# zzuiekongning/MGDT-YOLO

Measured on AMD Instinct MI355X. Metric: images/sec @640x640 bs=32 per GPU, detection forward + NMS (whole job: 1 GPU(s)), higher is better.
Workload: dtype bf16; 1 GPU; mspa_c2f_gd_yolov8-n (MSPA-C2f + GD neck + Detect, nc=80) 640x640 inference, batch 32/GPU: forward + decode + NMS(conf 0.25, iou 0.7), hipGraph replay, 4 batches in flight (one captured graph per resident batch, replayed round-robin on 4 streams); global_batch=32, parallelism=replicas x1 (batch-sharded, no data-path collective), rccl_ranks=1, input=bfloat16 NCHW images, 8 different batches resident in HBM (600 MiB) cycled, detections_last_step=9600, weights=seeded random init (no checkpoints offline), batches_in_flight=4

## Files before the change

include/mgdt.h:

```cpp
#ifndef MGDT_H
#define MGDT_H
#include <stddef.h>
#include <stdint.h>

#ifdef __cplusplus
extern "C" {
#endif

typedef void* mgdt_stream;

typedef enum { MGDT_OK = 0, MGDT_BAD_SHAPE = -1, MGDT_BAD_DTYPE = -2, MGDT_LAUNCH_FAIL = -3, MGDT_BAD_ARG = -4,
               MGDT_WORKSPACE = -5 } mgdt_status;
typedef enum { MGDT_F32 = 0, MGDT_BF16 = 1, MGDT_U8 = 2  } mgdt_dtype;
typedef enum { MGDT_ACT_NONE = 0, MGDT_ACT_SILU = 1, MGDT_ACT_RELU = 2, MGDT_ACT_GELU = 3 } mgdt_act;

typedef struct {
  void* p;
  int32_t n, h, w, c;
  int64_t sn, sh, sw, sc;
} mgdt_view;

const char* mgdt_last_error(void);
const char* mgdt_version(void);

size_t mgdt_conv_packed_bytes(int cin, int cout, int k, int dtype);
int mgdt_conv_pack(const float* w_oihw, const float* conv_bias, const float* bn_gamma, const float* bn_beta,
                   const float* bn_mean, const float* bn_var, float bn_eps, int cin, int cout, int k, int dtype,
                   void* packed_out, float* bias_out, mgdt_stream s);
int mgdt_conv_pack_dgrad(const float* w_oihw, int cin, int cout, int k, int phase, int dtype, void* packed_out, float* bias_out, mgdt_stream s);
typedef struct mgdt_pack_desc {
  const float* w; const float* conv_bias; const float* bn_gamma; const float* bn_beta; const float* bn_mean; const float* bn_var;
  float bn_eps; int32_t cin, cout, k, dtype, mode;
  void* packed; float* bias_out;
} mgdt_pack_desc;
int mgdt_conv_pack_batch(const mgdt_pack_desc* descs, int n, mgdt_stream s);

int mgdt_conv2d_fwd(const mgdt_view* x, const mgdt_view* x2, const float* in_scale, const float* in_shift,
                    const void* packed_w, const float* bias, int k, int stride, int act, const mgdt_view* r1,
                    const mgdt_view* r2, const mgdt_view* y, int dtype, mgdt_stream s);
size_t mgdt_conv_packed_bytes_fp8(int cin, int cout, int k);
int mgdt_conv_pack_fp8(const float* w_oihw, const float* conv_bias, const float* bn_gamma, const float* bn_beta, const float* bn_mean,
                       const float* bn_var, float bn_eps, int cin, int cout, int k, float x_qscale, void* packed_out, float* bias_out,
                       float* oscale_out, mgdt_stream s);
int mgdt_conv2d_fp8_fwd(const mgdt_view* x, const mgdt_view* x2, const float* in_scale, const float* in_shift, const void* packed_w,
                        const float* bias, const float* oscale, float x_qscale, int k, int stride, int act, const mgdt_view* r1,
                        const mgdt_view* r2, const mgdt_view* y, mgdt_stream s);
int mgdt_conv2d_phase_fwd(const mgdt_view* x, const void* packed_w, const float* bias, int phase, const mgdt_view* r1, const mgdt_view* r2,
                          const mgdt_view* y, int dtype, mgdt_stream s);

size_t mgdt_cnx_mlp_packed_bytes(int c, int dtype);
int mgdt_cnx_mlp_pack(const float* w1, const float* b1, const float* w2, const float* b2, int c, void* packed, int dtype, mgdt_stream s);
size_t mgdt_cnx_mlp_workspace_bytes(int n, int h, int w, int c);
int mgdt_cnx_mlp_fwd(const mgdt_view* t, const mgdt_view* res, const void* packed, const float* gamma, const float* beta, void* ws,
                     const mgdt_view* y, int dtype, mgdt_stream s);

int mgdt_cnx_block_supported(int n, int h, int w, int c, int dtype);
size_t mgdt_cnx_block_workspace_bytes(int n, int h, int w, int c);
int mgdt_cnx_block_fwd(const mgdt_view* x, const float* dw_w49c, const float* dw_b, const float* ln_w, const float* ln_b, float eps, const void* packed,
                       const float* gamma, const float* beta, const void* tail_w, const float* tail_b, int tail_act, void* ws, size_t ws_bytes,
                       const mgdt_view* y, int dtype, mgdt_stream s);

size_t mgdt_stem2_packed_bytes(void);
int mgdt_stem2_pack(const float* w_folded, void* packed, mgdt_stream s);
int mgdt_stem2_fwd(const mgdt_view* x, int x_dtype, const void* packed0, const float* bias0, const void* packed1, const float* bias1,
                   const mgdt_view* y, mgdt_stream s);

int mgdt_detect_tail_supported(int c2, int c3, int nc, int reg_max, int dtype);
int mgdt_detect_tail_fwd(const mgdt_view* tb, const mgdt_view* tc, const void* wb, const float* bb, const void* wc, const float* bc, int nc,
                         float stride, int a_off, int a_total, const mgdt_view* feat, float* y, unsigned long long* best_keys,
                         const void* wb3, const float* bb3, mgdt_stream s);
int mgdt_detect_tail_aug_fwd(const mgdt_view* tb, const mgdt_view* tc, const void* wb, const float* bb, const void* wc, const float* bc, int nc,
                             float stride, int a_off, int a_total, const mgdt_view* feat, float* y, unsigned long long* best_keys,
                             const void* wb3, const float* bb3, float aug_scale, int aug_flip, float aug_img_w, mgdt_stream s);

int mgdt_scale_img_fwd(const mgdt_view* x, int x_dtype, int flip, int hs, int ws, float pad, const mgdt_view* y, int y_dtype, mgdt_stream s);

int mgdt_csp_block_supported(int mode, int cin, int cout, int wd, int nbtl, int h, int w, int dtype);
int mgdt_csp_block_tiles(int mode, int n, int cin, int cout, int wd, int nbtl, int h, int w, int* geom8);
int mgdt_csp_block_fwd(int mode, const mgdt_view* x, const void* front, const float* front_bias, const void* const* mid,
                       const float* const* mid_bias, int nbtl, int shortcut, const void* back, const float* back_bias, int wd, int act,
                       const mgdt_view* y, float* pool, int dtype, mgdt_stream s);

size_t mgdt_pw_chain_packed_bytes(int wd, int dtype);
int mgdt_pw_chain_pack(int idx, const float* w_oi, const float* conv_bias, const float* bn_gamma, const float* bn_beta, const float* bn_mean,
                       const float* bn_var, float bn_eps, int wd, int dtype, void* packed, mgdt_stream s);
int mgdt_pw_chain3_fwd(const mgdt_view* x, const void* packed, int wd, int act, const mgdt_view* y, int dtype, mgdt_stream s);

int mgdt_conv1x1_inject_supported(int cin, int cout, int h, int w, int hg, int wg, int dtype);
int mgdt_conv1x1_inject_fwd(const mgdt_view* x, const void* packed_w, const float* bias, const mgdt_view* ga, const mgdt_view* gf,
                            const mgdt_view* y, int dtype, mgdt_stream s);

int mgdt_conv1x1_inject_conv_supported(int cin, int cmid, int cout2, int h, int w, int hg, int wg, int dtype);
int mgdt_conv1x1_inject_conv_fwd(const mgdt_view* x, const void* packed_w, const float* bias, const mgdt_view* ga, const mgdt_view* gf,
                                 const mgdt_view* gsrc, const void* packed_wg, const float* bias_g, int cmid,
                                 const void* packed_w2, const float* bias2, int act2, const mgdt_view* y2, int dtype, mgdt_stream s);

size_t mgdt_groupnorm_workspace_bytes(int n, int c);
int mgdt_groupnorm_fwd(const mgdt_view* x, const float* gamma, const float* beta, int groups, float eps, int act, void* ws, const mgdt_view* y,
                       int dtype, mgdt_stream s);
int mgdt_tood_layer_attn_fwd(const float* sums, int n, int c, int hw, const float* w1, const float* b1, const float* w2, const float* b2, int hid,
                             int stacked, float* scale, mgdt_stream s);
int mgdt_dcnv2_fwd(const mgdt_view* x, const mgdt_view* offset_mask, const float* w_gemm, const float* bias, const mgdt_view* y, int dtype,
                   mgdt_stream s);
int mgdt_dcnv2_mfma_fwd(const mgdt_view* x, const mgdt_view* offset_mask, const void* packed_w, const mgdt_view* y, int dtype, mgdt_stream s);
int mgdt_pixel_gate_fwd(const mgdt_view* x, const mgdt_view* gate, const mgdt_view* y, int dtype, mgdt_stream s);

int mgdt_conv_pack_direct(const float* w_oihw, const float* conv_bias, const float* bn_gamma, const float* bn_beta,
                          const float* bn_mean, const float* bn_var, float bn_eps, int cin_g, int cout, int k,
                          float* w_out, float* bias_out, mgdt_stream s);
int mgdt_conv2d_direct_fwd(const mgdt_view* x, int x_dtype, const float* w_gemm, const float* bias, int k, int stride,
                           int groups, int act, const mgdt_view* y, int dtype, mgdt_stream s);

#define MGDT_SPR_SPLITS 16
int mgdt_spr_pool_fwd(const mgdt_view* x, float* pooled, int dtype, mgdt_stream s);
int mgdt_spr_attn_fwd(const float* pooled, const float* fc1_w, const float* fc1_b, const float* fc2_w,
                      const float* fc2_b, int n, int c, int groups, int h, int w, int softmax, float* attn, mgdt_stream s);
int mgdt_scale_channels_fwd(const mgdt_view* x, const float* attn, const mgdt_view* y, int dtype, mgdt_stream s);
int mgdt_spr_attn_scale_fwd(const float* pooled, int nsplit, int tiles_x, int tiles_y, const float* fc1_w, const float* fc1_b, const float* fc2_w, const float* fc2_b, int groups,
                            const mgdt_view* x, const mgdt_view* y, const mgdt_view* pool_a, const mgdt_view* pool_b, int dtype, mgdt_stream s);

int mgdt_sppf_pool_fwd(const mgdt_view* x, const mgdt_view* y1, const mgdt_view* y2, const mgdt_view* y3, int dtype,
                       mgdt_stream s);

int mgdt_adaptive_avgpool_fwd(const mgdt_view* x, const mgdt_view* y, int dtype, mgdt_stream s);
int mgdt_bilinear_fwd(const mgdt_view* x, const mgdt_view* y, int dtype, mgdt_stream s);
int mgdt_nearest_fwd(const mgdt_view* x, const mgdt_view* y, int dtype, mgdt_stream s);
int mgdt_copy_fwd(const mgdt_view* x, int x_dtype, const mgdt_view* y, int y_dtype, mgdt_stream s);
int mgdt_image_pad4_fwd(const mgdt_view* x, int x_dtype, const mgdt_view* y, int y_dtype, mgdt_stream s);

#define MGDT_GRN_SPLITS 8
int mgdt_dwconv7_ln_fwd(const mgdt_view* x, const float* dw_w, const float* dw_b, const float* ln_w, const float* ln_b,
                        float eps, const mgdt_view* y, int dtype, mgdt_stream s);
int mgdt_grn_stats_fwd(const mgdt_view* t, const float* gamma, float* ws, float* scale, int dtype, mgdt_stream s);

int mgdt_inject_fwd(const mgdt_view* local, const mgdt_view* ga, const mgdt_view* gf, const mgdt_view* y, int dtype,
                    mgdt_stream s);

int mgdt_detect_decode_fwd(const mgdt_view* feat, int reg_max, int nc, float stride, int a_off, int a_total, float* y,
                           int dtype, mgdt_stream s);
int mgdt_detect_decode_aug_fwd(const mgdt_view* feat, int reg_max, int nc, float stride, int a_off, int a_total, float* y,
                               unsigned long long* best_keys, float aug_scale, int aug_flip, float aug_img_w, int dtype, mgdt_stream s);

size_t mgdt_nms_workspace_bytes(int n, int nc, int a, int multi_label, int max_nms);
int mgdt_nms_fwd(const float* pred, int n, int nc, int a, float conf_thres, float iou_thres, const int32_t* classes,
                 int n_classes, int agnostic, int multi_label, int max_det, int max_nms, float max_wh, float* out,
                 int32_t* kept_anchor, int32_t* counts, const unsigned long long* best_keys, void* ws, size_t ws_bytes, mgdt_stream s);

int mgdt_val_match_fwd(const float* det, const int32_t* ndet, int n, int max_det, const float* labels, const int32_t* nlab, int max_lab,
                       const float* iouv, int n_iou, uint8_t* correct, mgdt_stream s);

size_t mgdt_detect_loss_workspace_bytes(int b, int a_total, int n_gt);
int mgdt_detect_loss_fwd(const mgdt_view* const* feats, const float* strides, int n_levels, int reg_max, int nc,
                         const float* gt, int n_gt, int call_count, float gain_box, float gain_cls, float gain_dfl,
                         float* out5, unsigned char* fg_out, int32_t* gt_idx_out, float* tscore_out, void* ws,
                         size_t ws_bytes, int dtype, mgdt_stream s);
int mgdt_detect_loss_fwd_dev(const mgdt_view* const* feats, const float* strides, int n_levels, int reg_max, int nc,
                             const float* gt, int n_gt, const int32_t* call_count_dev, float gain_box, float gain_cls, float gain_dfl,
                             float* out5, unsigned char* fg_out, int32_t* gt_idx_out, float* tscore_out, void* ws,
                             size_t ws_bytes, int dtype, mgdt_stream s);
int mgdt_detect_loss_bwd(const mgdt_view* const* feats, const mgdt_view* const* grads, const float* strides, int n_levels,
                         int reg_max, int nc, const float* gt, int n_gt, float gain_box, float gain_cls, float gain_dfl,
                         float gscale, const float* out5, void* ws, size_t ws_bytes, int dtype, mgdt_stream s);

size_t mgdt_reduce_workspace_bytes(int c);
int mgdt_bn_stats_fwd(const mgdt_view* y, float eps, float momentum, float* mean, float* rstd, float* running_mean,
                      float* running_var, void* ws, int dtype, mgdt_stream s);
int mgdt_bn_act_fwd(const mgdt_view* y, const float* mean, const float* rstd, const float* gamma, const float* beta, int act,
                    const mgdt_view* r1, const mgdt_view* r2, const mgdt_view* z, int dtype, mgdt_stream s);
int mgdt_bn_act_bwd(const mgdt_view* gz, const mgdt_view* y, const float* mean, const float* rstd, const float* gamma,
                    const float* beta, int act, float* dgamma, float* dbeta, const mgdt_view* dy, void* ws, int dtype, mgdt_stream s);
int mgdt_conv_dgrad(const mgdt_view* dy, const float* w_oihw, int k, int stride, const mgdt_view* dx, int accumulate, int dtype,
                    mgdt_stream s);
int mgdt_gconv_dgrad(const mgdt_view* dy, const float* w, int k, int stride, int groups, const mgdt_view* dx, int accumulate, int dtype,
                     mgdt_stream s);
size_t mgdt_gconv_wgrad_workspace_bytes(int cin, int cout, int k, int groups);
int mgdt_gconv_wgrad(const mgdt_view* x, const mgdt_view* dy, int k, int stride, int groups, float* dw, int accumulate, void* ws, int dtype,
                     mgdt_stream s);
size_t mgdt_conv_wgrad_workspace_bytes(int cin, int cout, int k);
int mgdt_conv_wgrad(const mgdt_view* x, const mgdt_view* x2, const mgdt_view* dy, int k, int stride, float* dw_oihw, float* dbias,
                    int accumulate, void* ws, int dtype, mgdt_stream s);
int mgdt_conv_wgrad_splits(int cin, int cout, int k);
typedef struct mgdt_wgrad_final_desc { const float* partial; float* dw; long n; int32_t nsplit; int32_t accumulate; } mgdt_wgrad_final_desc;
int mgdt_wgrad_final_batch(const mgdt_wgrad_final_desc* descs, int n, mgdt_stream s);
int mgdt_add_fwd(const mgdt_view* a, const mgdt_view* b, const mgdt_view* o, int dtype, mgdt_stream s);
int mgdt_maxpool5_bwd(const mgdt_view* x, const mgdt_view* gy, float* gx_f32, int dtype, mgdt_stream s);
int mgdt_nearest_bwd(const mgdt_view* gy, const mgdt_view* gx, int dtype, mgdt_stream s);

int mgdt_ew_binary(const mgdt_view* a, const mgdt_view* b, const mgdt_view* o, int mode, int dtype, mgdt_stream s);
int mgdt_channel_affine(const mgdt_view* x, const float* scale, const float* shift, const mgdt_view* y, int dtype, mgdt_stream s);
size_t mgdt_nc_reduce_workspace_bytes(int n, int c);
int mgdt_nc_reduce(const mgdt_view* a, const mgdt_view* b, float* out, void* ws, int dtype, mgdt_stream s);
int mgdt_adaptive_avgpool_bwd(const mgdt_view* gy, const mgdt_view* gx, int accumulate, int dtype, mgdt_stream s);
int mgdt_bilinear_bwd(const mgdt_view* gy, const mgdt_view* gx, int accumulate, int dtype, mgdt_stream s);
size_t mgdt_spr_bwd_workspace_bytes(int n, int c, int groups);
int mgdt_spr_bwd(const mgdt_view* gy, const float* pooled_partial, int splits, const float* attn, const float* dattn,
                 const float* fc1_w, const float* fc1_b, const float* fc2_w, const float* fc2_b, int groups,
                 const mgdt_view* gx, float* param_grads, void* ws, int dtype, mgdt_stream s);
int mgdt_dwconv7_ln_train_fwd(const mgdt_view* x, const float* dw_w, const float* dw_b, const float* ln_w, const float* ln_b,
                              float eps, const mgdt_view* y, const mgdt_view* u_out, int dtype, mgdt_stream s);
size_t mgdt_dwconv7_ln_bwd_workspace_bytes(int c);
int mgdt_dwconv7_ln_bwd(const mgdt_view* x, const mgdt_view* u, const mgdt_view* gy, const float* dw_w49c, const float* ln_w, float eps,
                        const mgdt_view* du_tmp, const mgdt_view* dx, int accumulate_dx, float* d_dw_w, float* d_dw_b,
                        float* d_ln_w, float* d_ln_b, void* ws, int dtype, mgdt_stream s);
int mgdt_grn_bwd(const mgdt_view* g, const mgdt_view* t, const float* S, const float* A, const float* B, const float* gamma,
                 const mgdt_view* dt, float* dgamma, float* dbeta, void* ws, int dtype, mgdt_stream s);

size_t mgdt_grad_norm_workspace_bytes(void);
int mgdt_grad_clip_coef(const float* g, long n, float max_norm, float* out2, void* ws, mgdt_stream s);
int mgdt_sgd_step(float* p, const float* g, float* buf, const float* wd, long n, float lr, float lr_bias, float momentum, int nesterov,
                  int first, const float* clip2, mgdt_stream s);
int mgdt_ema_update(float* ema, const float* p, long n, float decay, mgdt_stream s);
int mgdt_sgd_ema_step_dev(float* p, const float* g, float* buf, const float* wd, long n_param, float* ema, long n_total, const float* hyper4,
                          int nesterov, int first, const float* clip2, mgdt_stream s);

int mgdt_box_convert(const float* in, float* out, long n, int row, int mode, mgdt_stream s);
int mgdt_box_iou(const float* b1, int n, const float* b2, int m, float eps, float* out, mgdt_stream s);
int mgdt_bbox_iou(const float* b1, int stride1, const float* b2, int stride2, long n, int xywh, int mode, float eps, float* out, mgdt_stream s);
int mgdt_scale_boxes(float* boxes, long n, int row, float gain, float padx, float pady, float h0, float w0, mgdt_stream s);
int mgdt_letterbox_fwd(const void* src_hwc_bgr, int sh, int sw, long src_pitch, void* dst_chw_rgb, int dh, int dw, int new_h, int new_w, int top,
                       int left, mgdt_stream s);
size_t mgdt_ap_workspace_bytes(int n_det, int n_cls);
int mgdt_ap_per_class(const void* tp, const float* conf, const int32_t* seg, const int32_t* nlab, int n_det, int n_cls, int T, const double* x101,
                      const double* px, double eps, void* ws, double* ap, double* pcur, double* rcur, mgdt_stream s);

int mgdt_gn_affine(const float* Sy, const float* Syy, int n, int c, int hw, const float* gamma, const float* beta, int groups, float eps,
                   float* mean_ng, float* rstd_ng, float* A, float* B, mgdt_stream s);
int mgdt_nc_affine_act_bwd(const mgdt_view* g, const mgdt_view* y, const float* A, const float* B, int act, const mgdt_view* gu, int dtype, mgdt_stream s);
size_t mgdt_gn_bwd_workspace_bytes(int n, int c);
int mgdt_gn_bwd_coef(const float* S1, const float* S2, const float* mean_ng, const float* rstd_ng, const float* gamma, int n, int c, int hw, int groups,
                     float* P, float* Q, float* R, float* dgamma, float* dbeta, int accumulate, void* ws, mgdt_stream s);
int mgdt_nc_axpby(const mgdt_view* a, const float* sa, const mgdt_view* b, const float* sb, const float* shift, const mgdt_view* out, int dtype,
                  mgdt_stream s);
int mgdt_pixel_gate_bwd(const mgdt_view* g, const mgdt_view* x, const mgdt_view* logit, const mgdt_view* gx, const mgdt_view* glogit, int dtype, mgdt_stream s);
size_t mgdt_tood_layer_attn_bwd_workspace_bytes(int n, int c, int hid, int stacked);
int mgdt_tood_layer_attn_bwd(const float* sums, const float* dscale, int n, int c, int hw, const float* w1, const float* b1, const float* w2,
                             const float* b2, int hid, int stacked, float* dsums, float* dw1, float* db1, float* dw2, float* db2, int accumulate,
                             void* ws, mgdt_stream s);
int mgdt_dcn_im2col(const mgdt_view* x, const mgdt_view* om, const mgdt_view* col, int dtype, mgdt_stream s);
int mgdt_dcn_col2im_bwd(const mgdt_view* gcol, const mgdt_view* x, const mgdt_view* om, float* gx_f32, const mgdt_view* gom, int dtype, mgdt_stream s);

#ifdef __cplusplus
}
#endif
#endif
```

mgdt_yolo_amd/_lib.py:

```python
import ctypes as C
import os

_HERE = os.path.dirname(os.path.abspath(__file__))
LIB_PATH = os.environ.get('MGDT_LIB') or os.path.join(_HERE, 'csrc', 'libmgdt_hip.so')

F32, BF16 = 0, 1
ACT_NONE, ACT_SILU, ACT_RELU, ACT_GELU = 0, 1, 2, 3
SPR_SPLITS = 16
GRN_SPLITS = 8


class View(C.Structure):
    _fields_ = [('p', C.c_void_p), ('n', C.c_int32), ('h', C.c_int32), ('w', C.c_int32), ('c', C.c_int32),
                ('sn', C.c_int64), ('sh', C.c_int64), ('sw', C.c_int64), ('sc', C.c_int64)]


VP = C.POINTER(View)
_vp, _i, _f, _sz = C.c_void_p, C.c_int, C.c_float, C.c_size_t

class PackDesc(C.Structure):
    _fields_ = [('w', C.c_void_p), ('conv_bias', C.c_void_p), ('bn_gamma', C.c_void_p), ('bn_beta', C.c_void_p), ('bn_mean', C.c_void_p), ('bn_var', C.c_void_p),
                ('bn_eps', C.c_float), ('cin', C.c_int32), ('cout', C.c_int32), ('k', C.c_int32), ('dtype', C.c_int32), ('mode', C.c_int32),
                ('packed', C.c_void_p), ('bias_out', C.c_void_p)]


class WgradFinalDesc(C.Structure):
    _fields_ = [('partial', C.c_void_p), ('dw', C.c_void_p), ('n', C.c_long), ('nsplit', C.c_int32), ('accumulate', C.c_int32)]


PROTOTYPES = {
    'mgdt_last_error': (C.c_char_p, []),
    'mgdt_version': (C.c_char_p, []),
    'mgdt_conv_packed_bytes': (_sz, [_i, _i, _i, _i]),
    'mgdt_conv_pack': (_i, [_vp, _vp, _vp, _vp, _vp, _vp, _f, _i, _i, _i, _i, _vp, _vp, _vp]),
    'mgdt_conv2d_fwd': (_i, [VP, VP, _vp, _vp, _vp, _vp, _i, _i, _i, VP, VP, VP, _i, _vp]),
    'mgdt_conv_packed_bytes_fp8': (_sz, [_i, _i, _i]),
    'mgdt_conv_pack_fp8': (_i, [_vp, _vp, _vp, _vp, _vp, _vp, _f, _i, _i, _i, _f, _vp, _vp, _vp, _vp]),
    'mgdt_conv2d_fp8_fwd': (_i, [VP, VP, _vp, _vp, _vp, _vp, _vp, _f, _i, _i, _i, VP, VP, VP, _vp]),
    'mgdt_conv_pack_batch': (_i, [_vp, _i, _vp]),
    'mgdt_conv2d_phase_fwd': (_i, [VP, _vp, _vp, _i, VP, VP, VP, _i, _vp]),
    'mgdt_conv_wgrad_splits': (_i, [_i, _i, _i]),
    'mgdt_wgrad_final_batch': (_i, [_vp, _i, _vp]),
    'mgdt_conv_pack_dgrad': (_i, [_vp, _i, _i, _i, _i, _i, _vp, _vp, _vp]),
    'mgdt_conv_pack_direct': (_i, [_vp, _vp, _vp, _vp, _vp, _vp, _f, _i, _i, _i, _vp, _vp, _vp]),
    'mgdt_conv2d_direct_fwd': (_i, [VP, _i, _vp, _vp, _i, _i, _i, _i, VP, _i, _vp]),
    'mgdt_spr_pool_fwd': (_i, [VP, _vp, _i, _vp]),
    'mgdt_spr_attn_fwd': (_i, [_vp, _vp, _vp, _vp, _vp, _i, _i, _i, _i, _i, _i, _vp, _vp]),
    'mgdt_scale_channels_fwd': (_i, [VP, _vp, VP, _i, _vp]),
    'mgdt_sppf_pool_fwd': (_i, [VP, VP, VP, VP, _i, _vp]),
    'mgdt_adaptive_avgpool_fwd': (_i, [VP, VP, _i, _vp]),
    'mgdt_bilinear_fwd': (_i, [VP, VP, _i, _vp]),
    'mgdt_nearest_fwd': (_i, [VP, VP, _i, _vp]),
    'mgdt_copy_fwd': (_i, [VP, _i, VP, _i, _vp]),
    'mgdt_image_pad4_fwd': (_i, [VP, _i, VP, _i, _vp]),
    'mgdt_dwconv7_ln_fwd': (_i, [VP, _vp, _vp, _vp, _vp, _f, VP, _i, _vp]),
    'mgdt_cnx_mlp_packed_bytes': (_sz, [_i, _i]),
    'mgdt_cnx_mlp_pack': (_i, [_vp, _vp, _vp, _vp, _i, _vp, _i, _vp]),
    'mgdt_cnx_mlp_workspace_bytes': (_sz, [_i, _i, _i, _i]),
    'mgdt_cnx_mlp_fwd': (_i, [VP, VP, _vp, _vp, _vp, _vp, VP, _i, _vp]),
    'mgdt_cnx_block_supported': (_i, [_i, _i, _i, _i, _i]),
    'mgdt_cnx_block_workspace_bytes': (_sz, [_i, _i, _i, _i]),
    'mgdt_cnx_block_fwd': (_i, [VP, _vp, _vp, _vp, _vp, _f, _vp, _vp, _vp, _vp, _vp, _i, _vp, _sz, VP, _i, _vp]),
    'mgdt_pw_chain_packed_bytes': (_sz, [_i, _i]),
    'mgdt_pw_chain_pack': (_i, [_i, _vp, _vp, _vp, _vp, _vp, _vp, _f, _i, _i, _vp, _vp]),
    'mgdt_pw_chain3_fwd': (_i, [VP, _vp, _i, _i, VP, _i, _vp]),
    'mgdt_conv1x1_inject_supported': (_i, [_i, _i, _i, _i, _i, _i, _i]),
    'mgdt_conv1x1_inject_fwd': (_i, [VP, _vp, _vp, VP, VP, VP, _i, _vp]),
    'mgdt_conv1x1_inject_conv_supported': (_i, [_i, _i, _i, _i, _i, _i, _i, _i]),
    'mgdt_conv1x1_inject_conv_fwd': (_i, [VP, _vp, _vp, VP, VP, VP, _vp, _vp, _i, _vp, _vp, _i, VP, _i, _vp]),
    'mgdt_spr_attn_scale_fwd': (_i, [_vp, _i, _i, _i, _vp, _vp, _vp, _vp, _i, VP, VP, VP, VP, _i, _vp]),
    'mgdt_stem2_packed_bytes': (_sz, []),
    'mgdt_stem2_pack': (_i, [_vp, _vp, _vp]),
    'mgdt_stem2_fwd': (_i, [VP, _i, _vp, _vp, _vp, _vp, VP, _vp]),
    'mgdt_detect_tail_supported': (_i, [_i, _i, _i, _i, _i]),
    'mgdt_detect_tail_fwd': (_i, [VP, VP, _vp, _vp, _vp, _vp, _i, _f, _i, _i, VP, _vp, _vp, _vp, _vp, _vp]),
    'mgdt_detect_tail_aug_fwd': (_i, [VP, VP, _vp, _vp, _vp, _vp, _i, _f, _i, _i, VP, _vp, _vp, _vp, _vp, _f, _i, _f, _vp]),
    'mgdt_scale_img_fwd': (_i, [VP, _i, _i, _i, _i, _f, VP, _i, _vp]),
    'mgdt_csp_block_supported': (_i, [_i, _i, _i, _i, _i, _i, _i, _i]),
    'mgdt_csp_block_tiles': (_i, [_i, _i, _i, _i, _i, _i, _i, _i, _vp]),
    'mgdt_csp_block_fwd': (_i, [_i, VP, _vp, _vp, _vp, _vp, _i, _i, _vp, _vp, _i, _i, VP, _vp, _i, _vp]),
    'mgdt_groupnorm_workspace_bytes': (_sz, [_i, _i]),
    'mgdt_groupnorm_fwd': (_i, [VP, _vp, _vp, _i, _f, _i, _vp, VP, _i, _vp]),
    'mgdt_tood_layer_attn_fwd': (_i, [_vp, _i, _i, _i, _vp, _vp, _vp, _vp, _i, _i, _vp, _vp]),
    'mgdt_dcnv2_fwd': (_i, [VP, VP, _vp, _vp, VP, _i, _vp]),
    'mgdt_dcnv2_mfma_fwd': (_i, [VP, VP, _vp, VP, _i, _vp]),
    'mgdt_pixel_gate_fwd': (_i, [VP, VP, VP, _i, _vp]),
    'mgdt_gn_affine': (_i, [_vp, _vp, _i, _i, _i, _vp, _vp, _i, _f, _vp, _vp, _vp, _vp, _vp]),
    'mgdt_nc_affine_act_bwd': (_i, [VP, VP, _vp, _vp, _i, VP, _i, _vp]),
    'mgdt_gn_bwd_workspace_bytes': (_sz, [_i, _i]),
    'mgdt_gn_bwd_coef': (_i, [_vp, _vp, _vp, _vp, _vp, _i, _i, _i, _i, _vp, _vp, _vp, _vp, _vp, _i, _vp, _vp]),
    'mgdt_nc_axpby': (_i, [VP, _vp, VP, _vp, _vp, VP, _i, _vp]),
    'mgdt_pixel_gate_bwd': (_i, [VP, VP, VP, VP, VP, _i, _vp]),
    'mgdt_tood_layer_attn_bwd_workspace_bytes': (_sz, [_i, _i, _i, _i]),
    'mgdt_tood_layer_attn_bwd': (_i, [_vp, _vp, _i, _i, _i, _vp, _vp, _vp, _vp, _i, _i, _vp, _vp, _vp, _vp, _vp, _i, _vp, _vp]),
    'mgdt_dcn_im2col': (_i, [VP, VP, VP, _i, _vp]),
    'mgdt_dcn_col2im_bwd': (_i, [VP, VP, VP, _vp, VP, _i, _vp]),
    'mgdt_val_match_fwd': (_i, [_vp, _vp, _i, _i, _vp, _vp, _i, _vp, _i, _vp, _vp]),
    'mgdt_grn_stats_fwd': (_i, [VP, _vp, _vp, _vp, _i, _vp]),
    'mgdt_inject_fwd': (_i, [VP, VP, VP, VP, _i, _vp]),
    'mgdt_detect_decode_fwd': (_i, [VP, _i, _i, _f, _i, _i, _vp, _i, _vp]),
    'mgdt_detect_decode_aug_fwd': (_i, [VP, _i, _i, _f, _i, _i, _vp, _vp, _f, _i, _f, _i, _vp]),
    'mgdt_detect_loss_workspace_bytes': (_sz, [_i, _i, _i]),
    'mgdt_detect_loss_fwd': (_i, [_vp, _vp, _i, _i, _i, _vp, _i, _i, _f, _f, _f, _vp, _vp, _vp, _vp, _vp, _sz, _i, _vp]),
    'mgdt_detect_loss_fwd_dev': (_i, [_vp, _vp, _i, _i, _i, _vp, _i, _vp, _f, _f, _f, _vp, _vp, _vp, _vp, _vp, _sz, _i, _vp]),
    'mgdt_detect_loss_bwd': (_i, [_vp, _vp, _vp, _i, _i, _i, _vp, _i, _f, _f, _f, _f, _vp, _vp, _sz, _i, _vp]),
    'mgdt_reduce_workspace_bytes': (_sz, [_i]),
    'mgdt_bn_stats_fwd': (_i, [VP, _f, _f, _vp, _vp, _vp, _vp, _vp, _i, _vp]),
    'mgdt_bn_act_fwd': (_i, [VP, _vp, _vp, _vp, _vp, _i, VP, VP, VP, _i, _vp]),
    'mgdt_bn_act_bwd': (_i, [VP, VP, _vp, _vp, _vp, _vp, _i, _vp, _vp, VP, _vp, _i, _vp]),
    'mgdt_conv_dgrad': (_i, [VP, _vp, _i, _i, VP, _i, _i, _vp]),
    'mgdt_gconv_dgrad': (_i, [VP, _vp, _i, _i, _i, VP, _i, _i, _vp]),
    'mgdt_gconv_wgrad_workspace_bytes': (_sz, [_i, _i, _i, _i]),
    'mgdt_gconv_wgrad': (_i, [VP, VP, _i, _i, _i, _vp, _i, _vp, _i, _vp]),
    'mgdt_conv_wgrad_workspace_bytes': (_sz, [_i, _i, _i]),
    'mgdt_conv_wgrad': (_i, [VP, VP, VP, _i, _i, _vp, _vp, _i, _vp, _i, _vp]),
    'mgdt_add_fwd': (_i, [VP, VP, VP, _i, _vp]),
    'mgdt_maxpool5_bwd': (_i, [VP, VP, _vp, _i, _vp]),
    'mgdt_nearest_bwd': (_i, [VP, VP, _i, _vp]),
    'mgdt_ew_binary': (_i, [VP, VP, VP, _i, _i, _vp]),
    'mgdt_channel_affine': (_i, [VP, _vp, _vp, VP, _i, _vp]),
    'mgdt_nc_reduce_workspace_bytes': (_sz, [_i, _i]),
    'mgdt_nc_reduce': (_i, [VP, VP, _vp, _vp, _i, _vp]),
    'mgdt_adaptive_avgpool_bwd': (_i, [VP, VP, _i, _i, _vp]),
    'mgdt_bilinear_bwd': (_i, [VP, VP, _i, _i, _vp]),
    'mgdt_spr_bwd_workspace_bytes': (_sz, [_i, _i, _i]),
    'mgdt_spr_bwd': (_i, [VP, _vp, _i, _vp, _vp, _vp, _vp, _vp, _vp, _i, VP, _vp, _vp, _i, _vp]),
    'mgdt_dwconv7_ln_train_fwd': (_i, [VP, _vp, _vp, _vp, _vp, _f, VP, VP, _i, _vp]),
    'mgdt_dwconv7_ln_bwd_workspace_bytes': (_sz, [_i]),
    'mgdt_dwconv7_ln_bwd': (_i, [VP, VP, VP, _vp, _vp, _f, VP, VP, _i, _vp, _vp, _vp, _vp, _vp, _i, _vp]),
    'mgdt_grn_bwd': (_i, [VP, VP, _vp, _vp, _vp, _vp, VP, _vp, _vp, _vp, _i, _vp]),
    'mgdt_grad_norm_workspace_bytes': (_sz, []),
    'mgdt_grad_clip_coef': (_i, [_vp, C.c_long, _f, _vp, _vp, _vp]),
    'mgdt_sgd_step': (_i, [_vp, _vp, _vp, _vp, C.c_long, _f, _f, _f, _i, _i, _vp, _vp]),
    'mgdt_ema_update': (_i, [_vp, _vp, C.c_long, _f, _vp]),
    'mgdt_sgd_ema_step_dev': (_i, [_vp, _vp, _vp, _vp, C.c_long, _vp, C.c_long, _vp, _i, _i, _vp, _vp]),
    'mgdt_box_convert': (_i, [_vp, _vp, C.c_long, _i, _i, _vp]),
    'mgdt_box_iou': (_i, [_vp, _i, _vp, _i, _f, _vp, _vp]),
    'mgdt_bbox_iou': (_i, [_vp, _i, _vp, _i, C.c_long, _i, _i, _f, _vp, _vp]),
    'mgdt_scale_boxes': (_i, [_vp, C.c_long, _i, _f, _f, _f, _f, _f, _vp]),
    'mgdt_letterbox_fwd': (_i, [_vp, _i, _i, C.c_long, _vp, _i, _i, _i, _i, _i, _i, _vp]),
    'mgdt_ap_workspace_bytes': (_sz, [_i, _i]),
    'mgdt_ap_per_class': (_i, [_vp, _vp, _vp, _vp, _i, _i, _i, _vp, _vp, C.c_double, _vp, _vp, _vp, _vp, _vp]),
    'mgdt_nms_workspace_bytes': (_sz, [_i, _i, _i, _i, _i]),
    'mgdt_nms_fwd': (_i, [_vp, _i, _i, _i, _f, _f, _vp, _i, _i, _i, _i, _i, _f, _vp, _vp, _vp, _vp, _vp, _sz, _vp]),
}

_lib = None


def lib():
    global _lib
    if _lib is None:
        if not os.path.exists(LIB_PATH):
            raise RuntimeError(f'{LIB_PATH} is missing: build it with `python -c "import __graft_entry__ as g; g.build()"` '
                               '(mgdt_yolo_amd has no CPU or PyTorch fallback)')
        import torch
        l = C.CDLL(LIB_PATH)
        for name, (res, args) in PROTOTYPES.items():
            fn = getattr(l, name)
            fn.restype, fn.argtypes = res, args
        _lib = l
    return _lib


def check(status, what=''):
    if status != 0:
        raise RuntimeError(f'{what or "mgdt"} failed ({status}): {lib().mgdt_last_error().decode()}')
```

mgdt_yolo_amd/csrc/conv3x3_lds.hip:

```cpp
#include <type_traits>
#include <vector>

#include "common.h"

#define C3_OOB ((int)0x80000000)
#define C3_TW 16
#define C3_RW 18
#define C3_MAXI 14

struct C3Args {
  const char* x; int xsn, xsh, xsw; uint32_t x_bytes;
  char* y; int ysn, ysh, ysw; uint32_t y_bytes;
  const char* wpk; const float* bias;
  int N, H, W, Ho, Wo, Cin, Cout, CP, nchunks, NTtot, ncg, tiles_x, tiles_per_img, ntiles, XP, act;
  FastDiv fd_tpi, fd_tx, fd_cp;
  const float* oscale; float xq;
  unsigned long long* dbg;
};

template <int ACT> __device__ __forceinline__ float c3_act(float v) {
  if (ACT == MGDT_ACT_SILU) return v * fast_sigmoid(v);
  if (ACT == MGDT_ACT_RELU) return fmaxf(v, 0.f);
  return v;
}

template <int NBW, int ACT, int NCH, int MT, bool Q8 = false, int S = 1, int WS = 1>
__global__ __launch_bounds__(256 * WS, 1) void conv3x3_lds_kernel(const C3Args a) {
  constexpr int NTHR = 256 * WS, NBH = (NBW + WS - 1) / WS;
  constexpr int RW = 15 * S + 3, TH = 4 * MT, RH = (TH - 1) * S + 3, RPX = RH * RW;
  constexpr int MAXI = ((S == 1 ? C3_MAXI : 18) + WS - 1) / WS;
  constexpr int WB = Q8 ? 512 : 1024, PB = Q8 ? 8 : 16;
  extern __shared__ __attribute__((aligned(16))) char c3_lds[];
  int* tab = (int*)c3_lds;
  char* wl = c3_lds + (((size_t)a.nchunks * 16 + 15) & ~(size_t)15);
  char* xs = wl + (size_t)a.nchunks * NBW * WB;
  const int tid = threadIdx.x, lane = tid & 63, r = lane & 15, g = lane >> 4;
  const int wave_all = __builtin_amdgcn_readfirstlane(tid >> 6);
  const int wave = wave_all & 3, wcol = wave_all >> 2;
  const int cg = blockIdx.x % a.ncg, w0 = blockIdx.x / a.ncg, wstep = gridDim.x / a.ncg;
  const int nb0 = cg * NBW;
  const __amdgpu_buffer_rsrc_t xrs = __builtin_amdgcn_make_buffer_rsrc((void*)a.x, 0, a.x_bytes, 0x00020000);
  const __amdgpu_buffer_rsrc_t yrs = __builtin_amdgcn_make_buffer_rsrc((void*)a.y, 0, a.y_bytes, 0x00020000);

  for (int p = tid; p < a.nchunks * 4; p += NTHR) {
    const int tap = (int)fdiv((uint32_t)p, a.fd_cp), cp = p - tap * a.CP;
    tab[p] = tap < 9 ? ((tap / 3) * RW + (tap % 3)) * a.XP + cp * PB : 0;
  }
  constexpr int WV = WB / 16;
  {
    const int total = a.nchunks * NBW * WV;
    for (int i0 = tid; i0 < total; i0 += 8 * NTHR) {
      uint4 t[8];
#pragma unroll
      for (int u = 0; u < 8; ++u) {
        const int i = min(i0 + u * NTHR, total - 1);
        const int kc = i / (NBW * WV), rem = i - kc * NBW * WV, bw = rem / WV, ln = rem % WV;
        const bool ok = nb0 + bw < a.NTtot;
        t[u] = ok ? *(const uint4*)(a.wpk + ((size_t)(kc * a.NTtot + nb0 + bw) * WV + ln) * 16) : make_uint4(0u, 0u, 0u, 0u);
      }
#pragma unroll
      for (int u = 0; u < 8; ++u)
        if (i0 + u * NTHR < total) *(uint4*)(wl + (size_t)(i0 + u * NTHR) * 16) = t[u];
    }
  }
  const int nbw0 = nb0 + wcol * NBH;
  f32x4 bias[NBH], osc[Q8 ? NBH : 1];
#pragma unroll
  for (int bw = 0; bw < NBH; ++bw) {
    bias[bw] = nbw0 + bw < a.NTtot ? *(const f32x4*)(a.bias + (nbw0 + bw) * 16 + 4 * g) : f32x4{0.f, 0.f, 0.f, 0.f};
    if constexpr (Q8) {
      osc[bw] = nbw0 + bw < a.NTtot ? *(const f32x4*)(a.oscale + (nbw0 + bw) * 16 + 4 * g) : f32x4{1.f, 1.f, 1.f, 1.f};
      bias[bw] = bias[bw] / osc[bw];
    }
  }

  const int nitems = RPX * a.CP;
  uint4 stage[MAXI];
  auto issue = [&](int t) {
    const int n = (int)fdiv((uint32_t)t, a.fd_tpi), rt = t - n * a.tiles_per_img;
    const int tyi = (int)fdiv((uint32_t)rt, a.fd_tx), txi = rt - tyi * a.tiles_x;
    const int iy0 = tyi * TH * S - 1, ix0 = txi * C3_TW * S - 1;
#pragma unroll
    for (int u = 0; u < MAXI; ++u) {
      const int it = tid + u * NTHR;
      const int pix = (int)fdiv((uint32_t)it, a.fd_cp), c8 = it - pix * a.CP;
      const int py = pix / RW, px = pix - py * RW;
      const int iy = iy0 + py, ix = ix0 + px;
      const bool ok = it < nitems && (unsigned)iy < (unsigned)a.H && (unsigned)ix < (unsigned)a.W;
      stage[u] = __builtin_bit_cast(uint4, __builtin_amdgcn_raw_buffer_load_b128(xrs, ok ? (uint32_t)(n * a.xsn + iy * a.xsh + ix * a.xsw + c8 * 16) : (uint32_t)C3_OOB, 0, 0));
    }
  };
  auto commit = [&]() {
#pragma unroll
    for (int u = 0; u < MAXI; ++u) {
      const int it = tid + u * NTHR;
      if (it < nitems) {
        const int pix = (int)fdiv((uint32_t)it, a.fd_cp), c8 = it - pix * a.CP;
        if constexpr (Q8) *(long*)(xs + pix * a.XP + c8 * 8) = quant8(__builtin_bit_cast(bf16x8, stage[u]), a.xq);
        else *(uint4*)(xs + pix * a.XP + c8 * 16) = stage[u];
      }
    }
  };

  const char* const wlane = wl + lane * PB;
  int bbase[MT];
#pragma unroll
  for (int m = 0; m < MT; ++m) bbase[m] = ((wave * MT + m) * S * RW + r * S) * a.XP;

  __builtin_amdgcn_s_waitcnt(0x0F70);
  unsigned long long T0 = 0, Tc = 0, Tm = 0, Te = 0, tl = 0, ntl = 0;
  if (a.dbg) { T0 = __builtin_amdgcn_s_memrealtime(); tl = T0; }
  int t = w0;
  if (t < a.ntiles) issue(t);
  while (t < a.ntiles) {
    __syncthreads();
    commit();
    __syncthreads();
    if (a.dbg) { const unsigned long long n_ = __builtin_amdgcn_s_memrealtime(); Tc += n_ - tl; tl = n_; }
    const int tn = t + wstep;
    if (tn < a.ntiles) issue(tn);

    f32x4 acc[NBH][MT];
#pragma unroll
    for (int bw = 0; bw < NBH; ++bw)
#pragma unroll
      for (int m = 0; m < MT; ++m) acc[bw][m] = bias[bw];
    typedef typename std::conditional<Q8, long, bf16x8>::type frag_t;
    frag_t A[2][NBH], B[2][MT];
    auto load_frags = [&](int kc, int buf) {
      const int off = tab[kc * 4 + g];
#pragma unroll
      for (int bw = 0; bw < NBH; ++bw) A[buf][bw] = *(const frag_t*)(wlane + (size_t)(kc * NBW + wcol * NBH + bw) * WB);
#pragma unroll
      for (int m = 0; m < MT; ++m) B[buf][m] = *(const frag_t*)(xs + bbase[m] + off);
    };
    auto mm = [&](frag_t w, frag_t p, f32x4 c) __attribute__((always_inline)) {
      if constexpr (Q8) return mma_q8(w, p, c);
      else return __builtin_amdgcn_mfma_f32_16x16x32_bf16(w, p, c, 0, 0, 0);
    };
    load_frags(0, 0);
    if (NCH > 0) {
#pragma unroll
      for (int kc = 0; kc < NCH; ++kc) {
        if (kc + 1 < NCH) load_frags(kc + 1, (kc + 1) & 1);
#pragma unroll
        for (int bw = 0; bw < NBH; ++bw)
#pragma unroll
          for (int m = 0; m < MT; ++m) acc[bw][m] = mm(A[kc & 1][bw], B[kc & 1][m], acc[bw][m]);
      }
    } else {
      for (int kc = 0; kc < a.nchunks; kc += 2) {
        if (kc + 1 < a.nchunks) load_frags(kc + 1, 1);
#pragma unroll
        for (int bw = 0; bw < NBH; ++bw)
#pragma unroll
          for (int m = 0; m < MT; ++m) acc[bw][m] = mm(A[0][bw], B[0][m], acc[bw][m]);
        if (kc + 1 < a.nchunks) {
          if (kc + 2 < a.nchunks) load_frags(kc + 2, 0);
#pragma unroll
          for (int bw = 0; bw < NBH; ++bw)
#pragma unroll
            for (int m = 0; m < MT; ++m) acc[bw][m] = mm(A[1][bw], B[1][m], acc[bw][m]);
        }
      }
    }

    if (a.dbg) { const unsigned long long n_ = __builtin_amdgcn_s_memrealtime(); Tm += n_ - tl; tl = n_; }
    {
      const int n = (int)fdiv((uint32_t)t, a.fd_tpi), rt = t - n * a.tiles_per_img;
      const int tyi = (int)fdiv((uint32_t)rt, a.fd_tx), txi = rt - tyi * a.tiles_x;
#pragma unroll
      for (int m = 0; m < MT; ++m) {
        const int oy = tyi * TH + wave * MT + m, ox = txi * C3_TW + r;
        const bool pin = oy < a.Ho && ox < a.Wo;
        const int po = n * a.ysn + oy * a.ysh + ox * a.ysw;
#pragma unroll
        for (int bw = 0; bw < NBH; ++bw) {
          const int co = (nbw0 + bw) * 16 + 4 * g;
          bf16x4 o;
#pragma unroll
          for (int j = 0; j < 4; ++j) o[j] = (bf16)c3_act<ACT>(Q8 ? acc[bw][m][j] * osc[Q8 ? bw : 0][j] : acc[bw][m][j]);
          __builtin_amdgcn_raw_buffer_store_b64(__builtin_bit_cast(__attribute__((__vector_size__(2 * sizeof(unsigned int)))) unsigned int, o), yrs,
                                                (pin && co < a.Cout) ? (uint32_t)(po + co * 2) : (uint32_t)C3_OOB, 0, 0);
        }
      }
    }
    if (a.dbg) { const unsigned long long n_ = __builtin_amdgcn_s_memrealtime(); Te += n_ - tl; tl = n_; ++ntl; }
    t = tn;
  }
  if (a.dbg && tid == 0) { unsigned long long* d = a.dbg + (size_t)blockIdx.x * 6; d[0] = T0; d[1] = tl; d[2] = Tc; d[3] = Tm; d[4] = Te; d[5] = ntl; }
}

bool mgdt_conv3x3_lds_launch(const mgdt_view* x, const mgdt_view* y, const void* packed_w, const float* bias, int act, int CP, int nchunks, int NTtot, hipStream_t st,
                             const float* q8_oscale, float q8_xq, int stride) {
  const bool q8 = q8_oscale != nullptr;
  static const int mode = getenv("MGDT_CONV3_LDS") ? atoi(getenv("MGDT_CONV3_LDS")) : 1;
  if (!mode) return false;
  static const bool ws2 = !(getenv("MGDT_C3_WAVES8") && atoi(getenv("MGDT_C3_WAVES8")) == 0);
  const bool wide = mode >= 3 || ws2;
  const int Cin = x->c, Cout = y->c;
  if (stride == 2 && (q8_oscale || Cin > 64 || NTtot % 4 || (nchunks != 9 && !(nchunks == 18 && wide)))) return false;
  if (Cin % 8 || Cin < 32 || Cin > 80 || Cout % 4 || Cout < 32 || (act != MGDT_ACT_SILU && act != MGDT_ACT_NONE && act != MGDT_ACT_RELU)) return false;
  const long M = (long)x->n * x->h * x->w;
  if (M < 16 * 1024 || x->h < 16 || x->w < 16) return false;
  const long extx = ((long)(x->n - 1) * x->sn + (long)(x->h - 1) * x->sh + (long)(x->w - 1) * x->sw + x->c) * 2;
  const long exty = ((long)(y->n - 1) * y->sn + (long)(y->h - 1) * y->sh + (long)(y->w - 1) * y->sw + y->c) * 2;
  if (extx >= 0x7fffffffL || exty >= 0x7fffffffL) return false;
  C3Args a;
  memset(&a, 0, sizeof(a));
  a.x = (const char*)x->p; a.xsn = (int)(x->sn * 2); a.xsh = (int)(x->sh * 2); a.xsw = (int)(x->sw * 2); a.x_bytes = (uint32_t)extx;
  a.y = (char*)y->p; a.ysn = (int)(y->sn * 2); a.ysh = (int)(y->sh * 2); a.ysw = (int)(y->sw * 2); a.y_bytes = (uint32_t)exty;
  a.wpk = (const char*)packed_w; a.bias = bias;
  a.N = x->n; a.H = x->h; a.W = x->w; a.Ho = y->h; a.Wo = y->w; a.Cin = Cin; a.Cout = Cout; a.CP = CP; a.nchunks = nchunks; a.NTtot = NTtot; a.act = act;
  a.XP = q8 ? Cin + 16 : Cin * 2 + 16;
  a.oscale = q8_oscale; a.xq = q8_xq;
  const int NBW = stride == 2 ? 4 : NTtot;
  if (NBW != 2 && NBW != 3 && NBW != 4 && NBW != 5 && NBW != 6) return false;
  a.ncg = NTtot / NBW;
  const size_t fixed = (((size_t)nchunks * 16 + 15) & ~(size_t)15) + (size_t)nchunks * NBW * (q8 ? 512 : 1024);
  auto region = [&](int mt) { return stride == 2 ? (size_t)(8 * mt + 1) * 33 * a.XP : (size_t)(4 * mt + 2) * C3_RW * a.XP; };
  int MT = stride == 2 ? 2 : 4;
  if (stride == 1 && fixed + region(MT) > 160 * 1024) MT = NBW == 5 && !q8 && wide && fixed + region(3) <= 160 * 1024 ? 3 : 2;
  const size_t lds = fixed + region(MT);
  if (lds > 160 * 1024) return false;
  if (NBW == 5 && !q8 && MT == 2 && mode < 2) return false;
  if (stride == 1 && (q8 ? MT != 4 : ((NBW == 5 && MT == 4) || (NBW != 5 && MT != 4)))) return false;
  const int TH = 4 * MT;
  a.tiles_x = cdiv(y->w, C3_TW);
  a.tiles_per_img = a.tiles_x * cdiv(y->h, TH);
  a.ntiles = x->n * a.tiles_per_img;
  if ((stride == 2 ? (2 * TH + 1) * 33 * CP > 256 * 18 : (TH + 2) * C3_RW * CP > 256 * C3_MAXI)) return false;
  a.fd_tpi = make_fastdiv((uint32_t)a.tiles_per_img); a.fd_tx = make_fastdiv((uint32_t)a.tiles_x); a.fd_cp = make_fastdiv((uint32_t)CP);
  int nwg = 256 / a.ncg * a.ncg;
  nwg = (int)std::min<long>(nwg, (long)a.ntiles * a.ncg);
  nwg = nwg / a.ncg * a.ncg;
  if (nwg < a.ncg) return false;
 #define C3_LAUNCH_Q8(NB, ACTV)                                                                                      \
  {                                                                                                                  \
    static std::atomic<bool> qattr{false}, qattr18{false}, qattr23{false};                                            \
    if (nchunks == 18) {                                                                                             \
      if (!qattr18) { (void)hipFuncSetAttribute((const void*)conv3x3_lds_kernel<NB, ACTV, 18, 4, true>, hipFuncAttributeMaxDynamicSharedMemorySize, 160 * 1024); qattr18 = true; } \
      conv3x3_lds_kernel<NB, ACTV, 18, 4, true><<<nwg, 256, lds, st>>>(a);                                           \
    } else if (nchunks == 23) {                                                                                      \
      if (!qattr23) { (void)hipFuncSetAttribute((const void*)conv3x3_lds_kernel<NB, ACTV, 23, 4, true>, hipFuncAttributeMaxDynamicSharedMemorySize, 160 * 1024); qattr23 = true; } \
      conv3x3_lds_kernel<NB, ACTV, 23, 4, true><<<nwg, 256, lds, st>>>(a);                                           \
    } else {                                                                                                         \
      if (!qattr) { (void)hipFuncSetAttribute((const void*)conv3x3_lds_kernel<NB, ACTV, 0, 4, true>, hipFuncAttributeMaxDynamicSharedMemorySize, 160 * 1024); qattr = true; } \
      conv3x3_lds_kernel<NB, ACTV, 0, 4, true><<<nwg, 256, lds, st>>>(a);                                            \
    }                                                                                                                \
  }
#define C3_ACT_Q8(NB) \
  if (act == MGDT_ACT_SILU) C3_LAUNCH_Q8(NB, MGDT_ACT_SILU) else if (act == MGDT_ACT_RELU) C3_LAUNCH_Q8(NB, MGDT_ACT_RELU) else C3_LAUNCH_Q8(NB, MGDT_ACT_NONE)
#define C3_LAUNCH(NB, ACTV, MTV, WSV)                                                                                     \
  {                                                                                                                  \
    static std::atomic<bool> attr{false}, attr18{false}, attr23{false};                                                                        \
    if (nchunks == 18) {                                                                                             \
      if (!attr18) { (void)hipFuncSetAttribute((const void*)conv3x3_lds_kernel<NB, ACTV, 18, MTV, false, 1, WSV>, hipFuncAttributeMaxDynamicSharedMemorySize, 160 * 1024); attr18 = true; } \
      conv3x3_lds_kernel<NB, ACTV, 18, MTV, false, 1, WSV><<<nwg, 256 * WSV, lds, st>>>(a);                                                    \
    } else if (nchunks == 23) {                                                                                      \
      if (!attr23) { (void)hipFuncSetAttribute((const void*)conv3x3_lds_kernel<NB, ACTV, 23, MTV, false, 1, WSV>, hipFuncAttributeMaxDynamicSharedMemorySize, 160 * 1024); attr23 = true; } \
      conv3x3_lds_kernel<NB, ACTV, 23, MTV, false, 1, WSV><<<nwg, 256 * WSV, lds, st>>>(a);                                               \
    } else {                                                                                                         \
      if (!attr) { (void)hipFuncSetAttribute((const void*)conv3x3_lds_kernel<NB, ACTV, 0, MTV, false, 1, WSV>, hipFuncAttributeMaxDynamicSharedMemorySize, 160 * 1024); attr = true; } \
      conv3x3_lds_kernel<NB, ACTV, 0, MTV, false, 1, WSV><<<nwg, 256 * WSV, lds, st>>>(a);                                                     \
    }                                                                                                                \
  }
#define C3_ACT(NB, MTV, WSV) \
  if (act == MGDT_ACT_SILU) C3_LAUNCH(NB, MGDT_ACT_SILU, MTV, WSV) else if (act == MGDT_ACT_RELU) C3_LAUNCH(NB, MGDT_ACT_RELU, MTV, WSV) else C3_LAUNCH(NB, MGDT_ACT_NONE, MTV, WSV)
  static unsigned long long* dbgbuf = nullptr;
  if (getenv("MGDT_C3_DBG") && !dbgbuf) (void)hipMalloc((void**)&dbgbuf, 256 * 6 * 8);
  a.dbg = dbgbuf;
#define C3_LAUNCH_S2(ACTV, NCHV)                                                                                      \
  {                                                                                                                  \
    static std::atomic<bool> sattr{false}, sattr8{false};                                                            \
    if (ws2) {                                                                                                       \
      if (!sattr8) { (void)hipFuncSetAttribute((const void*)conv3x3_lds_kernel<4, ACTV, NCHV, 2, false, 2, 2>, hipFuncAttributeMaxDynamicSharedMemorySize, 160 * 1024); sattr8 = true; } \
      conv3x3_lds_kernel<4, ACTV, NCHV, 2, false, 2, 2><<<nwg, 512, lds, st>>>(a);                                   \
    } else {                                                                                                         \
      if (!sattr) { (void)hipFuncSetAttribute((const void*)conv3x3_lds_kernel<4, ACTV, NCHV, 2, false, 2>, hipFuncAttributeMaxDynamicSharedMemorySize, 160 * 1024); sattr = true; } \
      conv3x3_lds_kernel<4, ACTV, NCHV, 2, false, 2><<<nwg, 256, lds, st>>>(a);                                      \
    }                                                                                                                \
  }
#define C3_ACT_S2(NCHV) \
  if (act == MGDT_ACT_SILU) C3_LAUNCH_S2(MGDT_ACT_SILU, NCHV) else if (act == MGDT_ACT_RELU) C3_LAUNCH_S2(MGDT_ACT_RELU, NCHV) else C3_LAUNCH_S2(MGDT_ACT_NONE, NCHV)
  if (stride == 2) {
    if (nchunks == 9) { C3_ACT_S2(9) } else { C3_ACT_S2(18) }
  } else if (q8) {
    if (NBW == 6) { C3_ACT_Q8(6) } else if (NBW == 5) { C3_ACT_Q8(5) } else if (NBW == 4) { C3_ACT_Q8(4) } else if (NBW == 3) { C3_ACT_Q8(3) } else { C3_ACT_Q8(2) }
  } else if (ws2 && (NBW == 6 || NBW == 4 || (NBW == 5 && MT == 3))) {
    if (NBW == 6) { C3_ACT(6, 4, 2) } else if (NBW == 4) { C3_ACT(4, 4, 2) } else { C3_ACT(5, 3, 2) }
  } else if (NBW == 6) { C3_ACT(6, 4, 1) } else if (NBW == 5 && MT == 3) { C3_ACT(5, 3, 1) } else if (NBW == 5) { C3_ACT(5, 2, 1) } else if (NBW == 4) { C3_ACT(4, 4, 1) } else if (NBW == 3) { C3_ACT(3, 4, 1) } else { C3_ACT(2, 4, 1) }
#undef C3_ACT
#undef C3_ACT_Q8
#undef C3_ACT_S2
#undef C3_LAUNCH_S2
#undef C3_LAUNCH_Q8
#undef C3_LAUNCH
  if (dbgbuf) {
    std::vector<unsigned long long> h(256 * 6);
    (void)hipStreamSynchronize(st);
    (void)hipMemcpy(h.data(), dbgbuf, h.size() * 8, hipMemcpyDeviceToHost);
    unsigned long long t0 = ~0ull, t1 = 0; double c = 0, m = 0, e = 0, nt = 0;
    for (int i = 0; i < nwg; ++i) { t0 = std::min(t0, h[i * 6]); t1 = std::max(t1, h[i * 6 + 1]); c += h[i * 6 + 2]; m += h[i * 6 + 3]; e += h[i * 6 + 4]; nt += h[i * 6 + 5]; }
    fprintf(stderr, "conv3x3_lds cin %d cout %d %dx%d: %d wgs, %d tiles, span %.1f us; per tile (us): wait+commit %.2f mfma %.2f epilogue %.2f\n", Cin, Cout, x->h, x->w, nwg,
            a.ntiles, (t1 - t0) * 0.01, c / nt * 0.01, m / nt * 0.01, e / nt * 0.01);
  }
  return true;
}
```

mgdt_yolo_amd/csrc/conv_igemm.hip:

```cpp
#include "conv_igemm_kernel.h"

struct FoldArgs { const float *cb, *g, *b, *mu, *var; float eps; int cout_real, cpad; float* bias_out; };
template <typename T>
__global__ void pack_kernel(const float* __restrict__ w, const float* __restrict__ scale, int Cin, int Cout, int KS,
                            int CP, int nchunks, int NTtot, T* __restrict__ out, int dgrad = 0, FoldArgs fa = FoldArgs{}) {
  constexpr int PE = Piece<T>::PE;
  long total = (long)nchunks * NTtot * 64 * PE;
  if (fa.bias_out && blockIdx.x == 0)
    for (int c = threadIdx.x; c < fa.cpad; c += blockDim.x) {
      float bo = 0.f;
      if (c < fa.cout_real) {
        if (fa.g) {
          const float s = fa.g[c] / sqrtf(fa.eps + fa.var[c]);
          bo = fa.b[c] - fa.g[c] * fa.mu[c] / sqrtf(fa.var[c] + fa.eps);
          if (fa.cb) bo += s * fa.cb[c];
        } else if (fa.cb) {
          bo = fa.cb[c];
        }
      }
      fa.bias_out[c] = bo;
    }
  for (long i = blockIdx.x * (long)blockDim.x + threadIdx.x; i < total; i += (long)gridDim.x * blockDim.x) {
    int j = (int)(i % PE);
    long t = i / PE;
// ... 130 lines not shown
      const float amax = red[0] * fabsf(fold);
      ws = amax > 0.f ? amax / 448.f : 1.f;
    }
    wscale[c] = ws;
    oscale[c] = ws / xq;
    fa.bias_out[c] = bo;
  }
}
__global__ void pack_q8_kernel(const float* __restrict__ w, FoldArgs fa, const float* __restrict__ wscale, int Cin, int Cout, int KS, int CP, int nchunks,
                               int NTtot, long* __restrict__ out) {
  typedef __attribute__((ext_vector_type(2))) int i32x2;
  const long total = (long)nchunks * NTtot * 64;
  for (long t = blockIdx.x * (long)blockDim.x + threadIdx.x; t < total; t += (long)gridDim.x * blockDim.x) {
    const int lane = (int)(t % 64);
    const int nb = (int)((t / 64) % NTtot), kc = (int)(t / 64 / NTtot);
    const int r = lane & 15, g = lane >> 4;
    const int p = kc * 4 + g, tap = p / CP, cp = p % CP, cout = nb * 16 + r;
    float v[8];
#pragma unroll
    for (int j = 0; j < 8; ++j) {
      const int cin = cp * 8 + j;
      float q = 0.f;
      if (tap < KS * KS && cin < Cin && cout < Cout) {
        q = w[(((long)cout * Cin + cin) * KS + tap / KS) * KS + tap % KS];
        if (fa.g) q *= fa.g[cout] / sqrtf(fa.eps + fa.var[cout]);
        q = __builtin_amdgcn_fmed3f(q / wscale[cout], -448.f, 448.f);
      }
      v[j] = q;
    }
    i32x2 o = {0, 0};
    o[0] = __builtin_amdgcn_cvt_pk_fp8_f32(v[0], v[1], o[0], false);
    o[0] = __builtin_amdgcn_cvt_pk_fp8_f32(v[2], v[3], o[0], true);
    o[1] = __builtin_amdgcn_cvt_pk_fp8_f32(v[4], v[5], o[1], false);
    o[1] = __builtin_amdgcn_cvt_pk_fp8_f32(v[6], v[7], o[1], true);
    out[t] = __builtin_bit_cast(long, o);
  }
}

extern "C" size_t mgdt_conv_packed_bytes_fp8(int cin, int cout, int k) {
  int CP, nchunks, NTtot;
  conv_geometry(cin, cout, k, MGDT_BF16, &CP, &nchunks, &NTtot);
  return (size_t)nchunks * NTtot * 512 + (size_t)NTtot * 16 * sizeof(float);
}

extern "C" int mgdt_conv_pack_fp8(const float* w, const float* cb, const float* g, const float* b, const float* mu, const float* var, float eps,
                                  int cin, int cout, int k, float x_qscale, void* packed, float* bias_out, float* oscale_out, mgdt_stream s) {
  if (!w || !packed || !bias_out || !oscale_out) MGDT_FAIL(MGDT_BAD_ARG, "conv_pack_fp8: null pointer");
  if ((g != nullptr) != (b != nullptr) || (g != nullptr) != (mu != nullptr) || (g != nullptr) != (var != nullptr))
    MGDT_FAIL(MGDT_BAD_ARG, "conv_pack_fp8: BN arguments must be all present or all NULL");
  if (!(x_qscale > 0.f) || !(x_qscale < 3.0e38f)) MGDT_FAIL(MGDT_BAD_ARG, "conv_pack_fp8: x_qscale must be a positive finite number");
  if (cin % 8 || cout % 4 || (k != 1 && k != 3)) MGDT_FAIL(MGDT_BAD_SHAPE, "conv_pack_fp8: cin=%d must be a multiple of 8, cout=%d of 4, k=%d 1 or 3", cin, cout, k);
  int CP, nchunks, NTtot;
  conv_geometry(cin, cout, k, MGDT_BF16, &CP, &nchunks, &NTtot);
  hipStream_t st = (hipStream_t)s;
  float* wscale = (float*)((char*)packed + (size_t)nchunks * NTtot * 512);
  const int cpad = NTtot * 16;
  const FoldArgs fa{cb, g, b, mu, var, eps, cout, cpad, bias_out};
  q8_wscale_kernel<<<cpad, 256, 0, st>>>(w, fa, cin * k * k, x_qscale, wscale, oscale_out);
  const long total = (long)nchunks * NTtot * 64;
  pack_q8_kernel<<<(int)std::min<long>((total + 255) / 256, 4096), 256, 0, st>>>(w, fa, wscale, cin, cout, k, CP, nchunks, NTtot, (long*)packed);
  MGDT_CHECK_LAUNCH("conv_pack_fp8");
  return MGDT_OK;
}

struct PackJob { const float* w; FoldArgs fa; int Cin, Cout, KS, CP, nchunks, NTtot, dgrad; void* out; };
#define PACK_BATCH 16
struct PackJobs { PackJob j[PACK_BATCH]; };
template <typename T>
__global__ void pack_batch_kernel(const PackJobs jobs) {
  const PackJob& J = jobs.j[blockIdx.y];
  constexpr int PE = Piece<T>::PE;
  const long total = (long)J.nchunks * J.NTtot * 64 * PE;
  const FoldArgs fa = J.fa;
  if (fa.bias_out && blockIdx.x == 0)
    for (int c = threadIdx.x; c < fa.cpad; c += blockDim.x) {
      float bo = 0.f;
      if (c < fa.cout_real) {
        if (fa.g) {
          const float s = fa.g[c] / sqrtf(fa.eps + fa.var[c]);
          bo = fa.b[c] - fa.g[c] * fa.mu[c] / sqrtf(fa.var[c] + fa.eps);
          if (fa.cb) bo += s * fa.cb[c];
        } else if (fa.cb) {
          bo = fa.cb[c];
        }
      }
      fa.bias_out[c] = bo;
    }
  const int Cin = J.Cin, Cout = J.Cout, KS = J.KS, CP = J.CP, NTtot = J.NTtot, dgrad = J.dgrad;
  const float* __restrict__ w = J.w;
  T* __restrict__ out = (T*)J.out;
  for (long i = blockIdx.x * (long)blockDim.x + threadIdx.x; i < total; i += (long)gridDim.x * blockDim.x) {
    int j = (int)(i % PE);
    long t = i / PE;
    int lane = (int)(t % 64);
    t /= 64;
    int nb = (int)(t % NTtot);
    int kc = (int)(t / NTtot);
    int r = lane & 15, g = lane >> 4;
    int p = kc * 4 + g;
    int tap = p / CP, cp = p % CP;
    if (dgrad >= 2) {
      const int nc_ = 1 + ((dgrad - 2) & 1), nr_ = 1 + ((dgrad - 2) >> 1);
      tap = tap < nr_ * nc_ ? (1 + tap / nc_) * 3 + (1 + tap % nc_) : 99;
    }
    int cin = cp * PE + j, cout = nb * 16 + r;
    float v = 0.f;
    if (tap < KS * KS && cin < Cin && cout < Cout) {
      if (dgrad == 1) v = w[(((long)cin * Cout + cout) * KS + (KS - 1 - tap / KS)) * KS + (KS - 1 - tap % KS)];
      else if (dgrad >= 2) {
        const int py = (dgrad - 2) >> 1, px = (dgrad - 2) & 1;
        const int ky = py + 1 - 2 * (tap / KS - 1), kx = px + 1 - 2 * (tap % KS - 1);
        v = ((unsigned)ky < 3u && (unsigned)kx < 3u) ? w[(((long)cin * Cout + cout) * 3 + ky) * 3 + kx] : 0.f;
      }
      else v = w[(((long)cout * Cin + cin) * KS + tap / KS) * KS + tap % KS];
      if (fa.g) v *= fa.g[cout] / sqrtf(fa.eps + fa.var[cout]);
    }
    out[i] = (T)v;
  }
}

extern "C" int mgdt_conv_pack_batch(const mgdt_pack_desc* d, int n, mgdt_stream s) {
  if (!d || n < 0) MGDT_FAIL(MGDT_BAD_ARG, "conv_pack_batch: null descriptor array");
  hipStream_t st = (hipStream_t)s;
  for (int dtype : {MGDT_F32, MGDT_BF16}) {
    PackJobs jobs;
    int m = 0;
    auto flush = [&]() {
      if (!m) return;
      for (int q = m; q < PACK_BATCH; ++q) { jobs.j[q] = jobs.j[0]; jobs.j[q].nchunks = 0; jobs.j[q].fa.bias_out = nullptr; }
      if (dtype == MGDT_F32) pack_batch_kernel<float><<<dim3(32, m), 256, 0, st>>>(jobs);
      else pack_batch_kernel<bf16><<<dim3(32, m), 256, 0, st>>>(jobs);
      m = 0;
    };
    for (int i = 0; i < n; ++i) {
      const mgdt_pack_desc& e = d[i];
      if (e.dtype != dtype) continue;
      if (!e.w || !e.packed || !e.bias_out) MGDT_FAIL(MGDT_BAD_ARG, "conv_pack_batch: descriptor %d has a null pointer", i);
      if (e.mode < 0 || e.mode > 5 || (e.mode >= 2 && e.k != 3)) MGDT_FAIL(MGDT_BAD_SHAPE, "conv_pack_batch: descriptor %d mode %d", i, e.mode);
      PackJob& J = jobs.j[m++];
      const int gi = e.mode == 0 ? e.cin : e.cout, go = e.mode == 0 ? e.cout : e.cin;
      conv_geometry(gi, go, e.k, dtype, &J.CP, &J.nchunks, &J.NTtot, e.mode >= 2 ? phase_ntaps(e.mode) : 0);
      J.w = e.w; J.Cin = gi; J.Cout = go; J.KS = e.k; J.dgrad = e.mode; J.out = e.packed;
      J.fa = e.mode == 0 ? FoldArgs{e.conv_bias, e.bn_gamma, e.bn_beta, e.bn_mean, e.bn_var, e.bn_eps, go, J.NTtot * 16, e.bias_out}
                         : FoldArgs{nullptr, nullptr, nullptr, nullptr, nullptr, 0.f, go, J.NTtot * 16, e.bias_out};
      if (m == PACK_BATCH) flush();
    }
    flush();
  }
  MGDT_CHECK_LAUNCH("conv_pack_batch");
  return MGDT_OK;
}

bool mgdt_conv3x3_lds_launch(const mgdt_view* x, const mgdt_view* y, const void* packed_w, const float* bias, int act, int CP, int nchunks, int NTtot, hipStream_t st,
                             const float* q8_oscale, float q8_xq, int stride);

template <typename T, int NT, int MT, bool Q8>
int launch_igemm(const ConvArgs& a, int gx, int gy, int threads, size_t lds, hipStream_t st);

template <typename T>
static int dispatch_igemm(const ConvArgs& a, int NT, int MT, int gx, int gy, int threads, size_t lds, hipStream_t st) {
#define CASE(nt, mt) \
  if (NT == nt && MT == mt) return launch_igemm<T, nt, mt, false>(a, gx, gy, threads, lds, st);
  CASE(1, 2) CASE(1, 4) CASE(2, 2) CASE(3, 2) CASE(4, 2) CASE(5, 2) CASE(6, 2) CASE(8, 2)
#undef CASE
  MGDT_FAIL(MGDT_BAD_SHAPE, "conv2d: no kernel for NT=%d MT=%d", NT, MT);
}

static int dispatch_igemm_q8(const ConvArgs& a, int NT, int gx, int gy, int threads, size_t lds, hipStream_t st) {
#define CASE(nt) \
  if (NT == nt) return launch_igemm<bf16, nt, 2, true>(a, gx, gy, threads, lds, st);
  CASE(1) CASE(2) CASE(3) CASE(4) CASE(5) CASE(6) CASE(8)
#undef CASE
  MGDT_FAIL(MGDT_BAD_SHAPE, "conv2d_fp8: no kernel for NT=%d", NT);
}

static int conv2d_fwd_impl(const mgdt_view* x, const mgdt_view* x2, const float* in_scale, const float* in_shift,
                           const void* packed_w, const float* bias, int k, int stride, int act, const mgdt_view* r1,
                           const mgdt_view* r2, const mgdt_view* y, int dtype, int tapmode, mgdt_stream s,
                           const float* q8_oscale = nullptr, float q8_xq = 1.f);
extern "C" int mgdt_conv2d_fwd(const mgdt_view* x, const mgdt_view* x2, const float* in_scale, const float* in_shift,
                               const void* packed_w, const float* bias, int k, int stride, int act, const mgdt_view* r1,
                               const mgdt_view* r2, const mgdt_view* y, int dtype, mgdt_stream s) {
  return conv2d_fwd_impl(x, x2, in_scale, in_shift, packed_w, bias, k, stride, act, r1, r2, y, dtype, 0, s);
}
extern "C" int mgdt_conv2d_phase_fwd(const mgdt_view* x, const void* packed_w, const float* bias, int phase, const mgdt_view* r1, const mgdt_view* r2,
                                     const mgdt_view* y, int dtype, mgdt_stream s) {
  if (phase < 0 || phase > 3) MGDT_FAIL(MGDT_BAD_ARG, "conv2d_phase: phase %d", phase);
  return conv2d_fwd_impl(x, nullptr, nullptr, nullptr, packed_w, bias, 3, 1, MGDT_ACT_NONE, r1, r2, y, dtype, 2 + phase, s);
}
extern "C" int mgdt_conv2d_fp8_fwd(const mgdt_view* x, const mgdt_view* x2, const float* in_scale, const float* in_shift,
                                   const void* packed_w, const float* bias, const float* oscale, float x_qscale, int k, int stride, int act,
                                   const mgdt_view* r1, const mgdt_view* r2, const mgdt_view* y, mgdt_stream s) {
  if (!oscale) MGDT_FAIL(MGDT_BAD_ARG, "conv2d_fp8: null oscale");
  if (!(x_qscale > 0.f) || !(x_qscale < 3.0e38f)) MGDT_FAIL(MGDT_BAD_ARG, "conv2d_fp8: x_qscale must be a positive finite number");
  return conv2d_fwd_impl(x, x2, in_scale, in_shift, packed_w, bias, k, stride, act, r1, r2, y, MGDT_BF16, 0, s, oscale, x_qscale);
}
static int conv2d_fwd_impl(const mgdt_view* x, const mgdt_view* x2, const float* in_scale, const float* in_shift,
                           const void* packed_w, const float* bias, int k, int stride, int act, const mgdt_view* r1,
                           const mgdt_view* r2, const mgdt_view* y, int dtype, int tapmode, mgdt_stream s,
                           const float* q8_oscale, float q8_xq) {
  const bool q8 = q8_oscale != nullptr;
  const int WB = q8 ? 512 : 1024;
  if (!view_ok(x) || !view_ok(y) || !packed_w || !bias) MGDT_FAIL(MGDT_BAD_ARG, "conv2d: null/empty view or weights");
  if (dtype != MGDT_F32 && dtype != MGDT_BF16) MGDT_FAIL(MGDT_BAD_DTYPE, "conv2d: dtype %d", dtype);
  if ((k != 1 && k != 3) || (stride != 1 && stride != 2)) MGDT_FAIL(MGDT_BAD_SHAPE, "conv2d: k=%d stride=%d unsupported", k, stride);
  const int pe = piece_elems(dtype);
  const int pad = k / 2;
  const int Ho = (x->h + 2 * pad - k) / stride + 1, Wo = (x->w + 2 * pad - k) / stride + 1;
  if (y->n != x->n || y->h != Ho || y->w != Wo) MGDT_FAIL(MGDT_BAD_SHAPE, "conv2d: y is %dx%dx%d, expected %dx%dx%d", y->n, y->h, y->w, x->n, Ho, Wo);
  if (x->c % pe || y->c % 4) MGDT_FAIL(MGDT_BAD_SHAPE, "conv2d: cin=%d must be a multiple of %d and cout=%d of 4", x->c, pe, y->c);
  auto aligned = [&](const mgdt_view* v, int q) {
    return v->sc == 1 && v->sw % q == 0 && v->sh % q == 0 && v->sn % q == 0 && ((uintptr_t)v->p % (q * dtype_size(dtype))) == 0;
  };
  if (!aligned(x, pe) || !aligned(y, 4)) MGDT_FAIL(MGDT_BAD_SHAPE, "conv2d: x/y must be NHWC views (sc==1) with 16-byte aligned pieces");
  if (x2 && x2->p && (x2->n != x->n || x2->h != x->h || x2->w != x->w || x2->c != x->c || !aligned(x2, pe)))
    MGDT_FAIL(MGDT_BAD_SHAPE, "conv2d: x2 must match x");
  for (const mgdt_view* rr : {r1, r2})
    if (rr && rr->p && (rr->n != y->n || rr->h != Ho || rr->w != Wo || rr->c != y->c || !aligned(rr, 4)))
      MGDT_FAIL(MGDT_BAD_SHAPE, "conv2d: residual must match y");

  ConvArgs a;
  memset(&a, 0, sizeof(a));
  const long sz = (long)dtype_size(dtype);
  auto extent = [&](const mgdt_view* v) { return ((long)(v->n - 1) * v->sn + (long)(v->h - 1) * v->sh + (long)(v->w - 1) * v->sw + v->c) * sz; };
  bool fits = true;
  auto bind = [&](const mgdt_view* v, const char** p, int* sn, int* sh, int* sw, uint32_t* bytes) {
    if (!v || !v->p) return;
    if (extent(v) >= 0x7fffffffL || v->sh * sz >= (1L << 23) || v->sw * sz >= (1L << 23)) { fits = false; return; }
    *p = (const char*)v->p; *sn = (int)(v->sn * sz); *sh = (int)(v->sh * sz); *sw = (int)(v->sw * sz); *bytes = (uint32_t)extent(v);
  };
  const char* yp = nullptr;
  bind(x, &a.x, &a.xsn, &a.xsh, &a.xsw, &a.x_bytes);
  bind(x2, &a.x2, &a.x2sn, &a.x2sh, &a.x2sw, &a.x2_bytes);
  bind(y, &yp, &a.ysn, &a.ysh, &a.ysw, &a.y_bytes);
  bind(r1, &a.r1, &a.r1sn, &a.r1sh, &a.r1sw, &a.r1_bytes);
  bind(r2, &a.r2, &a.r2sn, &a.r2sh, &a.r2sw, &a.r2_bytes);
  if (!fits) MGDT_FAIL(MGDT_BAD_SHAPE, "conv2d: a view spans >= 2 GiB or has a row stride >= 8 MiB");
  a.y = (char*)yp;
  a.in_scale = in_scale; a.in_shift = in_shift;
  a.wpk = (const char*)packed_w; a.bias = bias;
  a.oscale = q8_oscale; a.xq = q8_xq;
  a.N = x->n; a.H = x->h; a.W = x->w; a.Cin = x->c; a.Ho = Ho; a.Wo = Wo; a.Cout = y->c;
  a.KS = k; a.stride = stride; a.pad = pad; a.act = act;
  a.ntaps = tapmode >= 2 ? phase_ntaps(tapmode) : k * k;
  a.taplist = phase_taplist(tapmode, k);
  conv_geometry(a.Cin, a.Cout, k, dtype, &a.CP, &a.nchunks, &a.NTtot, tapmode >= 2 ? a.ntaps : 0);
  long M = (long)a.N * Ho * Wo;
  if (M > 0x7fffffffL - (1 << 20)) MGDT_FAIL(MGDT_BAD_SHAPE, "conv2d: problem too large");
  a.M = (int)M; a.HoWo = Ho * Wo;
  a.fd_howo = make_fastdiv((uint32_t)a.HoWo); a.fd_wo = make_fastdiv((uint32_t)Wo);
  if (tapmode == 0 && dtype == MGDT_BF16 && k == 3 && !(x2 && x2->p) && !in_scale && !in_shift && !(r1 && r1->p) && !(r2 && r2->p) &&
      mgdt_conv3x3_lds_launch(x, y, packed_w, bias, act, a.CP, a.nchunks, a.NTtot, (hipStream_t)s, q8_oscale, q8_xq, stride)) {
    MGDT_CHECK_LAUNCH("conv2d(3x3 lds)");
    return MGDT_OK;
  }

  int LDS_PANEL_KIB = 144;
  { const char* e = getenv("MGDT_CONV_PANEL_KIB"); if (e) LDS_PANEL_KIB = atoi(e); }
  int NT = 1;
  for (int c : {8, 6, 5, 4, 3, 2, 1})
    if (a.NTtot % c == 0 && (long)a.nchunks * c * WB <= LDS_PANEL_KIB * 1024L) { NT = c; break; }
  int MT = 2;
  if (!q8 && NT == 1 && a.NTtot == 1) { const char* e = getenv("MGDT_CONV_MT1"); MT = e && atoi(e) == 4 ? 4 : 2; }
  int waves = 8;
  auto wgs = [&](int nt, int wv) { return (long)cdiv(M, 16 * wv * MT) * (a.NTtot / nt); };
  {
    const char* e = getenv("MGDT_CONV_MINWG");
    const int minwg = e ? atoi(e) : 128;
    while (wgs(NT, waves) < minwg && NT > 1 && NT % 2 == 0) NT /= 2;
  }
  {
    static const bool tail_split = getenv("MGDT_CONV_TAIL_SPLIT") != nullptr;
    const long w0 = wgs(NT, waves);
    if (tail_split && w0 > 768 && w0 <= 960 && NT % 2 == 0) NT /= 2;
  }
  {
    const char* e;
    if ((e = getenv("MGDT_CONV_WAVES"))) waves = std::min(8, std::max(1, atoi(e)));
  }
  a.numTiles = cdiv(M, 16 * waves * MT);
  a.T8 = cdiv(a.numTiles, 8);
  a.tab_bytes = (a.nchunks + 3) / 4 * 4 * 4 * 16;
  size_t panel = (size_t)a.nchunks * NT * WB;
  if (panel <= (size_t)LDS_PANEL_KIB * 1024) { a.seg_chunks = a.nchunks; a.nseg = 1; }
  else { a.seg_chunks = 64; a.nseg = cdiv(a.nchunks, a.seg_chunks); }
  size_t lds = a.tab_bytes + (size_t)(q8 ? 2 : 1) * NT * 16 * sizeof(float) + (size_t)a.seg_chunks * NT * WB;
  int gcap = waves == 8 ? 256 : 1024;
  { const char* e = getenv("MGDT_CONV_GCAP"); if (e) gcap = atoi(e); }
  if (lds > 160 * 1024) MGDT_FAIL(MGDT_BAD_SHAPE, "conv2d: %zu bytes of LDS for NT=%d, %d chunks", lds, NT, a.seg_chunks);
  int gx = std::min(8 * a.T8, gcap), gy = a.NTtot / NT;
  hipStream_t st = (hipStream_t)s;
  if (q8) return dispatch_igemm_q8(a, NT, gx, gy, waves * 64, lds, st);
  if (dtype == MGDT_F32) return dispatch_igemm<float>(a, NT, MT, gx, gy, waves * 64, lds, st);
  return dispatch_igemm<bf16>(a, NT, MT, gx, gy, waves * 64, lds, st);
}
```

mgdt_yolo_amd/csrc/pointwise.hip:

```cpp
#include <algorithm>
#include <vector>

#include <type_traits>
#include "common.h"

#define SPR_SPLITS 16

static inline int grid_for(long work, int block = 256, int cap = 8192) { return (int)std::min<long>((work + block - 1) / block, cap); }

struct PixIdx { FastDiv fq, fw, fh; int Q, W, H; };
static inline PixIdx make_pixidx(int H, int W, int Q) { return PixIdx{make_fastdiv((uint32_t)Q), make_fastdiv((uint32_t)W), make_fastdiv((uint32_t)H), Q, W, H}; }
__device__ __forceinline__ void decode_idx(uint32_t i, const PixIdx& d, int& n, int& h, int& w, int& q) {
  uint32_t t = fdiv(i, d.fq);
  q = (int)(i - t * d.Q);
  uint32_t t2 = fdiv(t, d.fw);
  w = (int)(t - t2 * d.W);
  uint32_t t3 = fdiv(t2, d.fh);
  h = (int)(t2 - t3 * d.H);
  n = (int)t3;
}
template <typename T, int V> __device__ __forceinline__ void ldv(const T* p, float (&v)[V]) {
#pragma unroll
  for (int k = 0; k < V; k += 4) {
    f32x4 t = load4<T>(p + k);
// ... 261 lines not shown
  const int c0 = (int)((long)blockIdx.x * NC / gridDim.x), c1 = (int)((long)(blockIdx.x + 1) * NC / gridDim.x);
  for (int j = threadIdx.x; j < (c1 - c0) * Q; j += 256) {
    const int cl = j / Q, q = j - cl * Q, cell = c0 + cl, cy = cell / Wc, cx = cell - cy * Wc;
    float a[V];
#pragma unroll
    for (int k = 0; k < V; ++k) a[k] = att[q * V + k];
    float v[FM * FM][V];
#pragma unroll
    for (int e = 0; e < FM * FM; ++e) ldv<T, V>(x + n * xsn + (long)(cy * FM + e / FM) * xsh + (long)(cx * FM + e % FM) * xsw + q * V, v[e]);
    float accb[V], accs[4][V];
#pragma unroll
    for (int k = 0; k < V; ++k) { accb[k] = 0.f; accs[0][k] = accs[1][k] = accs[2][k] = accs[3][k] = 0.f; }
#pragma unroll
    for (int e = 0; e < FM * FM; ++e) {
      const int yy = e / FM, xx = e % FM;
#pragma unroll
      for (int k = 0; k < V; ++k) v[e][k] = (float)(T)(v[e][k] * a[k]);
      stv<T, V>(y + n * ysn + (long)(cy * FM + yy) * ysh + (long)(cx * FM + xx) * ysw + q * V, v[e]);
#pragma unroll
      for (int k = 0; k < V; ++k) {
        accb[k] += v[e][k];
        if (FM == 4) accs[(yy >> 1) * 2 + (xx >> 1)][k] += v[e][k];
      }
    }
    if (big.F) {
      const float inv = 1.f / (float)(FM * FM);
#pragma unroll
      for (int k = 0; k < V; ++k) accb[k] *= inv;
      stv<T, V>((T*)big.y + n * big.sn + cy * big.sh + cx * big.sw + q * V, accb);
    }
    if (FM == 4 && small.F) {
#pragma unroll
      for (int sc = 0; sc < 4; ++sc) {
#pragma unroll
        for (int k = 0; k < V; ++k) accs[sc][k] *= 0.25f;
        stv<T, V>((T*)small.y + n * small.sn + (long)(cy * 2 + (sc >> 1)) * small.sh + (long)(cx * 2 + (sc & 1)) * small.sw + q * V, accs[sc]);
      }
    }
  }
}

__device__ __forceinline__ void spr_prologue_fast(const float* __restrict__ partial, const float* __restrict__ w1, const float* __restrict__ b1,
                                                  const float* __restrict__ w2, const float* __restrict__ b2, int C, int G, int n, int nsplit, int tiles_x,
                                                  int tiles_y, FastDiv fd_gst, FastDiv fd_tx, FastDiv fd_l4, const float* cnt, float* sm, float* red, float* att, unsigned long long* TS, int& nt) {
#define SPR_STAMP() do { if (TS) TS[nt++] = __builtin_amdgcn_s_memrealtime(); } while (0)
  const int tid = threadIdx.x, cw = C / G, hid = cw / 4, L = 5 * cw, L4 = L / 4, r1 = L + 4, r2 = hid + 1;
  float* pvec = sm;
  float* hbuf = sm + C * 5;
  float* obuf = hbuf + G * hid;
  float* w1s = att + C + ((4 - ((C * 7 + G * hid) & 3)) & 3);
  float* w2s = w1s + hid * r1;
  float* b1s = w2s + cw * r2;
  float* b2s = b1s + hid;
  constexpr int PB = 16, WB = 6;
  const int ph = 256 / C, c = tid % C, sp0 = tid / C;
  const float* pc = partial + (long)n * nsplit * C + c;
  float pv[PB];
#pragma unroll
  for (int u = 0; u < PB; ++u) { const int sp = sp0 + u * ph; pv[u] = (sp0 < ph && sp < nsplit) ? pc[(long)sp * C] : 0.f; }
  const int nw4 = hid * L4;
  float4 wv[WB];
#pragma unroll
  for (int u = 0; u < WB; ++u) { const int i4 = tid + u * 256; wv[u] = i4 < nw4 ? ((const float4*)w1)[i4] : make_float4(0.f, 0.f, 0.f, 0.f); }
  const float w2v = tid < cw * hid ? w2[tid] : 0.f;
  const float b1v = tid < hid ? b1[tid] : 0.f, b2v = tid < cw ? b2[tid] : 0.f;
  SPR_STAMP();
#pragma unroll
  for (int u = 0; u < WB; ++u) {
    const int i4 = tid + u * 256;
    if (i4 < nw4) { const int row = (int)fdiv((uint32_t)i4, fd_l4); *(float4*)(w1s + row * r1 + (i4 - row * L4) * 4) = wv[u]; }
  }
  for (int i4 = tid + WB * 256; i4 < nw4; i4 += 256) { const int row = (int)fdiv((uint32_t)i4, fd_l4); *(float4*)(w1s + row * r1 + (i4 - row * L4) * 4) = ((const float4*)w1)[i4]; }
  if (tid < cw * hid) w2s[(tid / hid) * r2 + tid % hid] = w2v;
  for (int i = tid + 256; i < cw * hid; i += 256) w2s[(i / hid) * r2 + i % hid] = w2[i];
  if (tid < hid) b1s[tid] = b1v;
  if (tid < cw) b2s[tid] = b2v;
  for (int i = tid + 256; i < cw; i += 256) b2s[i] = b2[i];
  __builtin_amdgcn_s_waitcnt(0x0F70); SPR_STAMP();
  float acc[5] = {0.f, 0.f, 0.f, 0.f, 0.f};
  auto add = [&](float v, int sp) __attribute__((always_inline)) {
    const int tile = (int)fdiv((uint32_t)sp, fd_gst), ty = (int)fdiv((uint32_t)tile, fd_tx), tx = tile - ty * tiles_x;
    const int bin = (2 * ty >= tiles_y ? 2 : 0) + (2 * tx >= tiles_x ? 1 : 0);
    acc[0] += v;
    acc[1] += bin == 0 ? v : 0.f;
    acc[2] += bin == 1 ? v : 0.f;
    acc[3] += bin == 2 ? v : 0.f;
    acc[4] += bin == 3 ? v : 0.f;
  };
#pragma unroll
  for (int u = 0; u < PB; ++u) add(pv[u], sp0 + u * ph);
  if (sp0 < ph) {
    for (int sp = sp0 + PB * ph; sp < nsplit; sp += PB * ph) {
#pragma unroll
      for (int u = 0; u < PB; ++u) pv[u] = sp + u * ph < nsplit ? pc[(long)(sp + u * ph) * C] : 0.f;
#pragma unroll
      for (int u = 0; u < PB; ++u) add(pv[u], sp + u * ph);
    }
  }
#pragma unroll
  for (int k = 0; k < 5; ++k) red[k * 256 + tid] = acc[k];
  __syncthreads();
  for (int o = tid; o < C * 5; o += 256) {
    const int cc = o % C, k = o / C, gi = cc / cw, ci = cc - gi * cw;
    float sum = 0.f;
    for (int p = 0; p < ph; ++p) sum += red[k * 256 + p * C + cc];
    pvec[gi * L + (k == 0 ? ci : cw + 4 * ci + (k - 1))] = sum / cnt[k];
  }
  __syncthreads();
  SPR_STAMP();
  const int nout = G * hid;
  int tpo = 64;
  while (tpo > 1 && (256 / tpo < nout || tpo > L4)) tpo >>= 1;
  const int opp = 256 / tpo;
  for (int base = 0; base < nout; base += opp) {
    const int o = base + tid / tpo, p = tid % tpo;
    float a0 = 0.f, a1 = 0.f;
    if (o < nout) {
      const int gi = o / hid, hj = o - gi * hid;
      const float4* wr = (const float4*)(w1s + hj * r1);
      const float4* pg = (const float4*)(pvec + gi * L);
      int i = p;
      for (; i + tpo < L4; i += 2 * tpo) {
        const float4 wa = wr[i], xa = pg[i], wb = wr[i + tpo], xb = pg[i + tpo];
        a0 = fmaf(wa.w, xa.w, fmaf(wa.z, xa.z, fmaf(wa.y, xa.y, fmaf(wa.x, xa.x, a0))));
        a1 = fmaf(wb.w, xb.w, fmaf(wb.z, xb.z, fmaf(wb.y, xb.y, fmaf(wb.x, xb.x, a1))));
      }
      if (i < L4) { const float4 wa = wr[i], xa = pg[i]; a0 = fmaf(wa.w, xa.w, fmaf(wa.z, xa.z, fmaf(wa.y, xa.y, fmaf(wa.x, xa.x, a0)))); }
    }
    float s = a0 + a1;
    for (int m = tpo >> 1; m >= 1; m >>= 1) s += __shfl_xor(s, m, 64);
    if (o < nout && p == 0) hbuf[o] = fmaxf(s + b1s[o % hid], 0.f);
  }
  __syncthreads();
  SPR_STAMP();
  for (int o = tid; o < C; o += 256) {
    const int gi = o / cw, ci = o - gi * cw;
    float s = b2s[ci];
#pragma unroll 4
    for (int hj = 0; hj < hid; ++hj) s = fmaf(w2s[ci * r2 + hj], hbuf[gi * hid + hj], s);
    obuf[o] = 1.f / (1.f + expf(-s));
  }
  __syncthreads();
  SPR_STAMP();
  for (int ci = tid; ci < cw; ci += 256) {
    float mx = -INFINITY;
    for (int gi = 0; gi < G; ++gi) mx = fmaxf(mx, obuf[gi * cw + ci]);
    float den = 0.f;
    for (int gi = 0; gi < G; ++gi) { const float e = expf(obuf[gi * cw + ci] - mx); att[gi * cw + ci] = e; den += e; }
    for (int gi = 0; gi < G; ++gi) att[gi * cw + ci] /= den;
  }
  __syncthreads();
}

template <typename T, int V>
__global__ __launch_bounds__(256) void spr_attn_scale_kernel(const float* __restrict__ partial, const float* __restrict__ w1, const float* __restrict__ b1,
                                                             const float* __restrict__ w2, const float* __restrict__ b2, int C, int G, int H, int W,
                                                             const T* __restrict__ x, long xsn, long xsh, long xsw, T* __restrict__ y, long ysn, long ysh,
                                                             long ysw, FastDiv fd_q, FastDiv fd_w, int nsplit, int tiles_x, int tiles_y, SprPool pa, SprPool pb, FastDiv fd_gst,
                                                             FastDiv fd_tx, FastDiv fd_l4, int fast, unsigned long long* dbg) {
  extern __shared__ float sm[];
  unsigned long long TS[10]; int nt = 0;
  auto stamp = [&]() __attribute__((always_inline)) { if (dbg) TS[nt++] = __builtin_amdgcn_s_memrealtime(); };
  stamp();
  const int n = blockIdx.y, cw = C / G, hid = cw / 4;
  float* pooled = sm;
  float* hbuf = sm + C * 5;
  float* obuf = hbuf + G * hid;
  float* att = obuf + C;
  const int hs1 = bin_start(1, H, 2), he0 = bin_end(0, H, 2), ws1 = bin_start(1, W, 2), we0 = bin_end(0, W, 2);
  const float cnt[5] = {(float)H * W, (float)he0 * we0, (float)he0 * (W - ws1), (float)(H - hs1) * we0, (float)(H - hs1) * (W - ws1)};
  __shared__ float red[5 * 256];
  if (fast) {
    spr_prologue_fast(partial, w1, b1, w2, b2, C, G, n, nsplit, tiles_x, tiles_y, fd_gst, fd_tx, fd_l4, cnt, sm, red, att, dbg ? TS : nullptr, nt);
  } else {
    if (tiles_x > 0) {
      const int gst = nsplit / (tiles_x * tiles_y);
      for (int c0 = 0; c0 < C; c0 += 256) {
        const int lanes_c = min(C - c0, 256);
        const int ph = 256 / lanes_c;
        const int c = c0 + threadIdx.x % lanes_c, sp0 = threadIdx.x / lanes_c;
        float acc[5] = {0.f, 0.f, 0.f, 0.f, 0.f};
        if (sp0 < ph) {
          for (int sp = sp0; sp < nsplit; sp += ph) {
            const float v = partial[((long)n * nsplit + sp) * C + c];
            const int tile = sp / gst, ty = tile / tiles_x, tx = tile - ty * tiles_x;
            const int bin = (2 * ty >= tiles_y ? 2 : 0) + (2 * tx >= tiles_x ? 1 : 0);
            acc[0] += v;
            acc[1] += bin == 0 ? v : 0.f;
            acc[2] += bin == 1 ? v : 0.f;
            acc[3] += bin == 2 ? v : 0.f;
            acc[4] += bin == 3 ? v : 0.f;
          }
        }
#pragma unroll
        for (int k = 0; k < 5; ++k) red[k * 256 + threadIdx.x] = acc[k];
        __syncthreads();
        for (int o = threadIdx.x; o < lanes_c * 5; o += 256) {
          const int cc = o % lanes_c, k = o / lanes_c;
          float sum = 0.f;
          for (int p = 0; p < ph; ++p) sum += red[k * 256 + p * lanes_c + cc];
          pooled[(c0 + cc) * 5 + k] = sum / cnt[k];
        }
        __syncthreads();
      }
    } else {
      for (int i = threadIdx.x; i < C * 5; i += 256) {
        float sum = 0.f;
        for (int sp = 0; sp < nsplit; ++sp) sum += partial[((long)n * nsplit + sp) * C * 5 + i];
        pooled[i] = sum / cnt[i % 5];
      }
      __syncthreads();
    }
    for (int o = threadIdx.x; o < G * hid; o += 256) {
      int gi = o / hid, hj = o % hid;
      const float* wr = w1 + (long)hj * 5 * cw;
      float acc = b1[hj];
      for (int c = 0; c < cw; ++c) acc = fmaf(wr[c], pooled[(gi * cw + c) * 5 + 0], acc);
      for (int c = 0; c < cw; ++c)
        for (int bn = 0; bn < 4; ++bn) acc = fmaf(wr[cw + c * 4 + bn], pooled[(gi * cw + c) * 5 + 1 + bn], acc);
      hbuf[o] = fmaxf(acc, 0.f);
    }
    __syncthreads();
    for (int o = threadIdx.x; o < C; o += 256) {
      int gi = o / cw, c = o % cw;
      float acc = b2[c];
      for (int hj = 0; hj < hid; ++hj) acc = fmaf(w2[(long)c * hid + hj], hbuf[gi * hid + hj], acc);
      obuf[o] = 1.f / (1.f + expf(-acc));
    }
    __syncthreads();
    for (int c = threadIdx.x; c < cw; c += 256) {
      float mx = -INFINITY;
      for (int gi = 0; gi < G; ++gi) mx = fmaxf(mx, obuf[gi * cw + c]);
      float den = 0.f;
      for (int gi = 0; gi < G; ++gi) den += expf(obuf[gi * cw + c] - mx);
      for (int gi = 0; gi < G; ++gi) att[gi * cw + c] = expf(obuf[gi * cw + c] - mx) / den;
    }
    __syncthreads();
  }
  stamp();
  auto fin = [&]() __attribute__((always_inline)) { if (dbg) { __builtin_amdgcn_s_waitcnt(0); stamp(); if (threadIdx.x == 0) for (int k = 0; k < 8; ++k) dbg[((size_t)blockIdx.y * gridDim.x + blockIdx.x) * 8 + k] = TS[k]; } };
  {
    const int fa = pa.F, fb = pb.F, fm = max(fa, fb);
    const bool cells = fm > 0 && (fm == 2 || fm == 4) && (fa == 0 || fa == fm || (fm == 4 && fa == 2)) && (fb == 0 || fb == fm || (fm == 4 && fb == 2)) && !(fa == fb);
    if (cells) {
      const SprPool none = {nullptr, 0, 0, 0, 0};
      const SprPool big = fa == fm ? pa : (fb == fm ? pb : none), small = (fa && fa < fm) ? pa : ((fb && fb < fm) ? pb : none);
      if (fm == 4) spr_scale_cells<T, V, 4>(x, xsn, xsh, xsw, y, ysn, ysh, ysw, att, n, H, W, C, big, small);
      else spr_scale_cells<T, V, 2>(x, xsn, xsh, xsw, y, ysn, ysh, ysw, att, n, H, W, C, big, small);
      fin();
      return;
    }
  }
  const int Q = C / V, HW = H * W;
  const int p0 = (int)((long)blockIdx.x * HW / gridDim.x), p1 = (int)((long)(blockIdx.x + 1) * HW / gridDim.x);
  const uint32_t total = (uint32_t)(p1 - p0) * Q;
  auto one = [&](uint32_t i, long& xo, long& yo, int& qv) __attribute__((always_inline)) {
    const int pl = (int)fdiv(i, fd_q), q = (int)i - pl * Q;
    const int p = p0 + pl, h = (int)fdiv((uint32_t)p, fd_w), w = p - h * W;
    xo = n * xsn + h * xsh + w * xsw + q * V; yo = n * ysn + h * ysh + w * ysw + q * V; qv = q * V;
  };
  uint32_t i = threadIdx.x;
  for (; i + 3 * 256 < total; i += 4 * 256) {
    float v[4][V];
    long yo[4];
    int qv[4];
#pragma unroll
    for (int u = 0; u < 4; ++u) { long xo; one(i + u * 256, xo, yo[u], qv[u]); ldv<T, V>(x + xo, v[u]); }
#pragma unroll
    for (int u = 0; u < 4; ++u) {
#pragma unroll
      for (int k = 0; k < V; ++k) v[u][k] *= att[qv[u] + k];
      stv<T, V>(y + yo[u], v[u]);
    }
  }
  for (; i < total; i += 256) {
    long xo, yo; int qv; float v[V];
    one(i, xo, yo, qv);
    ldv<T, V>(x + xo, v);
#pragma unroll
    for (int k = 0; k < V; ++k) v[k] *= att[qv + k];
    stv<T, V>(y + yo, v);
  }
  const SprPool pools[2] = {pa, pb};
#pragma unroll
  for (int pi = 0; pi < 2; ++pi) {
    const SprPool P = pools[pi];
    if (P.F == 0) continue;
    const int F = P.F, Ho = H / F, Wo = W / F, HWo = Ho * Wo;
    const int q0 = (int)((long)blockIdx.x * HWo / gridDim.x), q1 = (int)((long)(blockIdx.x + 1) * HWo / gridDim.x);
    const float inv = 1.f / (float)(F * F);
    for (int j = threadIdx.x; j < (q1 - q0) * Q; j += 256) {
      const int pl = j / Q, q = j - pl * Q, po = q0 + pl, oy = po / Wo, ox = po - oy * Wo;
      float a[V], acc[V];
#pragma unroll
      for (int k = 0; k < V; ++k) { a[k] = att[q * V + k]; acc[k] = 0.f; }
      for (int yy = 0; yy < F; ++yy)
        for (int xx = 0; xx < F; ++xx) {
          float v[V];
          ldv<T, V>(x + n * xsn + (long)(oy * F + yy) * xsh + (long)(ox * F + xx) * xsw + q * V, v);
#pragma unroll
          for (int k = 0; k < V; ++k) acc[k] += (float)(T)(v[k] * a[k]);
        }
#pragma unroll
      for (int k = 0; k < V; ++k) acc[k] *= inv;
      stv<T, V>((T*)P.y + n * P.sn + oy * P.sh + ox * P.sw + q * V, acc);
    }
  }
  fin();
}

extern "C" int mgdt_spr_attn_scale_fwd(const float* pooled, int nsplit, int tiles_x, int tiles_y, const float* fc1_w, const float* fc1_b, const float* fc2_w, const float* fc2_b, int groups,
                                       const mgdt_view* x, const mgdt_view* y, const mgdt_view* pool_a, const mgdt_view* pool_b, int dtype, mgdt_stream s) {
  if (nsplit <= 0) nsplit = SPR_SPLITS;
  if (tiles_x > 0 && (tiles_y <= 0 || nsplit % (tiles_x * tiles_y) || tiles_x % 2 || tiles_y % 2 || x->h % 2 || x->w % 2))
    MGDT_FAIL(MGDT_BAD_SHAPE, "spr_attn_scale: per-tile sums need an even tile grid over an even map (nsplit=%d tiles %dx%d)", nsplit, tiles_y, tiles_x);
  if (!pooled || !fc1_w || !fc1_b || !fc2_w || !fc2_b || !view_ok(x) || !view_ok(y)) MGDT_FAIL(MGDT_BAD_ARG, "spr_attn_scale: null/empty argument");
  const int c = x->c;
  if (groups < 1 || c % groups || (c / groups) % 4 || c > 4096) MGDT_FAIL(MGDT_BAD_SHAPE, "spr_attn_scale: c=%d groups=%d", c, groups);
  if (!vec4_ok(x, dtype) || !vec4_ok(y, dtype) || x->n != y->n || x->h != y->h || x->w != y->w || y->c != c)
    MGDT_FAIL(MGDT_BAD_SHAPE, "spr_attn_scale: views must be matching NHWC, c%%4==0");
  const int cw = c / groups, hid = cw / 4;
  size_t lds = (size_t)(c * 5 + groups * hid + 2 * c) * sizeof(float);
  const size_t wbytes = ((size_t)hid * (5 * cw + 4) + (size_t)cw * (hid + 1) + hid + cw + 4) * sizeof(float);
  const int fast = tiles_x > 0 && c <= 256 && lds + wbytes <= 48 * 1024 && ((uintptr_t)fc1_w & 15) == 0;
  if (fast) lds += wbytes;
  SprPool pl[2] = {{nullptr, 0, 0, 0, 0}, {nullptr, 0, 0, 0, 0}};
  bool pool8 = true;
  const mgdt_view* pv[2] = {pool_a, pool_b};
  for (int i = 0; i < 2; ++i) {
    const mgdt_view* p = pv[i];
    if (!p || !p->p) continue;
    if (!view_ok(p) || !vec4_ok(p, dtype) || p->n != x->n || p->c != c || p->h < 1 || x->h % p->h || x->w % p->w || x->h / p->h != x->w / p->w)
      MGDT_FAIL(MGDT_BAD_SHAPE, "spr_attn_scale: a pooled output must be an NHWC view of the same n, c whose size divides the map by one factor");
    pl[i].y = p->p; pl[i].sn = p->sn; pl[i].sh = p->sh; pl[i].sw = p->sw; pl[i].F = x->h / p->h;
    pool8 = pool8 && vecN_ok(p, dtype, 8);
  }
  static unsigned long long* dbgbuf = nullptr;
  if (getenv("MGDT_SPR_DBG") && !dbgbuf) (void)hipMalloc((void**)&dbgbuf, 4096 * 8 * 8);
  int gK = 0;
  MGDT_DISPATCH_TV(dtype, vecN_ok(x, dtype, 8) && vecN_ok(y, dtype, 8) && pool8, {
    const long vecs = (long)x->h * x->w * (c / V);
    static const long per_wg = getenv("MGDT_SPR_VECS") ? atol(getenv("MGDT_SPR_VECS")) : 2048;
    static const long kmax = getenv("MGDT_SPR_KMAX") ? atol(getenv("MGDT_SPR_KMAX")) : 12;
    const int K = (int)std::max<long>(1, std::min<long>(kmax, vecs / per_wg));
    spr_attn_scale_kernel<T, V><<<dim3(K, x->n), 256, lds, (hipStream_t)s>>>(pooled, fc1_w, fc1_b, fc2_w, fc2_b, c, groups, x->h, x->w, (const T*)x->p, x->sn,
                                                                              x->sh, x->sw, (T*)y->p, y->sn, y->sh, y->sw, make_fastdiv((uint32_t)(c / V)),
                                                                              make_fastdiv((uint32_t)x->w), nsplit, tiles_x, tiles_y, pl[0], pl[1],
                                                                              make_fastdiv((uint32_t)(tiles_x > 0 ? nsplit / (tiles_x * tiles_y) : 1)),
                                                                              make_fastdiv((uint32_t)std::max(tiles_x, 1)), make_fastdiv((uint32_t)(5 * cw / 4)), fast, dbgbuf);
    gK = K;
  });
  MGDT_CHECK_LAUNCH("spr_attn_scale_fwd");
  if (dbgbuf && gK * x->n <= 4096) {
    (void)hipStreamSynchronize((hipStream_t)s);
    std::vector<unsigned long long> h((size_t)gK * x->n * 8);
    (void)hipMemcpy(h.data(), dbgbuf, h.size() * 8, hipMemcpyDeviceToHost);
    unsigned long long t0 = ~0ull, t1 = 0; double ph[7] = {0, 0, 0, 0, 0, 0, 0};
    const int ns = fast ? 8 : 3;
    for (int i = 0; i < gK * x->n; ++i) { t0 = std::min(t0, h[i * 8]); t1 = std::max(t1, h[i * 8 + ns - 1]); for (int k = 0; k + 1 < ns; ++k) ph[k] += (double)(h[i * 8 + k + 1] - h[i * 8 + k]); }
    fprintf(stderr, "spr_attn_scale c %d %dx%d: %d wgs, span %.1f us; mean per wg (us):", c, x->h, x->w, gK * x->n, (t1 - t0) * 0.01);
    for (int k = 0; k + 1 < ns; ++k) fprintf(stderr, " %.2f", ph[k] * 0.01 / (gK * x->n));
    fprintf(stderr, fast ? "  (issue | loads land | sums | fc1 | fc2 | softmax | scale)\n" : "  (prologue | scale)\n");
  }
  return MGDT_OK;
}

template <typename T, int V>
__global__ void scale_channels_kernel(const T* __restrict__ x, long xsn, long xsh, long xsw, const float* __restrict__ attn,
                                      T* __restrict__ y, long ysn, long ysh, long ysw, uint32_t total, int C, PixIdx d) {
  for (uint32_t i = blockIdx.x * blockDim.x + threadIdx.x; i < total; i += gridDim.x * blockDim.x) {
    int n, h, w, q;
    decode_idx(i, d, n, h, w, q);
    float v[V], a[V];
    ldv<T, V>(x + n * xsn + h * xsh + w * xsw + q * V, v);
    ldv<float, V>(attn + (long)n * C + q * V, a);
#pragma unroll
    for (int k = 0; k < V; ++k) v[k] *= a[k];
    stv<T, V>(y + n * ysn + h * ysh + w * ysw + q * V, v);
  }
}

extern "C" int mgdt_scale_channels_fwd(const mgdt_view* x, const float* attn, const mgdt_view* y, int dtype, mgdt_stream s) {
  if (!view_ok(x) || !view_ok(y) || !attn) MGDT_FAIL(MGDT_BAD_ARG, "scale_channels: null/empty argument");
  if (!vec4_ok(x, dtype) || !vec4_ok(y, dtype) || x->n != y->n || x->h != y->h || x->w != y->w || x->c != y->c)
    MGDT_FAIL(MGDT_BAD_SHAPE, "scale_channels: views must be matching NHWC, c%%4==0");
  long tot = (long)x->n * x->h * x->w * x->c;
  if (tot >= 0x7fffffffL) MGDT_FAIL(MGDT_BAD_SHAPE, "scale_channels: too large");
  MGDT_DISPATCH_TV(dtype, vecN_ok(x, dtype, 8) && vecN_ok(y, dtype, 8), {
    PixIdx d = make_pixidx(x->h, x->w, x->c / V);
    uint32_t total = (uint32_t)(tot / V);
    scale_channels_kernel<T, V><<<grid_for(total), 256, 0, (hipStream_t)s>>>((const T*)x->p, x->sn, x->sh, x->sw, attn, (T*)y->p, y->sn, y->sh, y->sw, total, x->c, d);
  });
  MGDT_CHECK_LAUNCH("scale_channels_fwd");
  return MGDT_OK;
}

__device__ __forceinline__ float pool_max(float a, float b) { return __builtin_elementwise_maximum(a, b); }

template <typename T, int SPPF_CG>
__global__ __launch_bounds__(256) void sppf_pool_kernel(const T* __restrict__ x, long xsn, long xsh, long xsw, T* __restrict__ y1, long s1n,
                                                        long s1h, long s1w, T* __restrict__ y2, long s2n, long s2h, long s2w,
                                                        T* __restrict__ y3, long s3n, long s3h, long s3w, int H, int W) {
  extern __shared__ float sm[];
  const int n = blockIdx.x, c0 = blockIdx.y * SPPF_CG, HW = H * W, WP = W + 4, PP = (H + 4) * WP;
  float* A = sm;
  float* Bf = sm + PP * SPPF_CG;
  constexpr int QN = SPPF_CG / 4;
  const f32x4 ninf = {-INFINITY, -INFINITY, -INFINITY, -INFINITY};
  for (int i = threadIdx.x; i < PP * QN; i += 256) {
    const int pp = i / QN, qq = (i % QN) * 4;
    const int hh = pp / WP - 2, ww = pp % WP - 2;
    const bool in = (unsigned)hh < (unsigned)H && (unsigned)ww < (unsigned)W;
    *(f32x4*)(A + pp * SPPF_CG + qq) = in ? load4<T>(x + n * xsn + hh * xsh + ww * xsw + c0 + qq) : ninf;
    *(f32x4*)(Bf + pp * SPPF_CG + qq) = ninf;
  }
  __syncthreads();
  T* outs[3] = {y1, y2, y3};
  const long on[3] = {s1n, s2n, s3n}, oh[3] = {s1h, s2h, s3h}, ow[3] = {s1w, s2w, s3w};
  for (int pass = 0; pass < 3; ++pass) {
    for (int i = threadIdx.x; i < HW * SPPF_CG; i += 256) {
      const int c = i % SPPF_CG, p = i / SPPF_CG, h = p / W, w = p - h * W;
      const int o = ((h + 2) * WP + w + 2) * SPPF_CG + c;
      const float a0 = A[o - 2 * SPPF_CG], a1 = A[o - SPPF_CG], a2 = A[o], a3 = A[o + SPPF_CG], a4 = A[o + 2 * SPPF_CG];
      Bf[o] = pool_max(pool_max(pool_max(a0, a1), pool_max(a2, a3)), a4);
    }
    __syncthreads();
    for (int i = threadIdx.x; i < HW * SPPF_CG; i += 256) {
      const int c = i % SPPF_CG, p = i / SPPF_CG, h = p / W, w = p - h * W;
      const int o = ((h + 2) * WP + w + 2) * SPPF_CG + c, rs = WP * SPPF_CG;
      const float b0 = Bf[o - 2 * rs], b1 = Bf[o - rs], b2 = Bf[o], b3 = Bf[o + rs], b4 = Bf[o + 2 * rs];
      A[o] = pool_max(pool_max(pool_max(b0, b1), pool_max(b2, b3)), b4);
    }
    __syncthreads();
    for (int i = threadIdx.x; i < HW * QN; i += 256) {
      const int p = i / QN, qq = (i % QN) * 4, h = p / W, w = p - h * W;
      store4<T>(outs[pass] + n * on[pass] + h * oh[pass] + w * ow[pass] + c0 + qq, *(const f32x4*)(A + ((h + 2) * WP + w + 2) * SPPF_CG + qq));
    }
  }
}

template <typename T, int V>
__global__ __launch_bounds__(256) void sppf_pool3_kernel(const T* __restrict__ x, long xsn, long xsh, long xsw, T* __restrict__ y1, long s1n, long s1h, long s1w,
                                                         T* __restrict__ y2, long s2n, long s2h, long s2w, T* __restrict__ y3, long s3n, long s3h, long s3w, int H, int W) {
  extern __shared__ __attribute__((aligned(16))) char sm3[];
  const int n = blockIdx.x, c0 = blockIdx.y * V, WP = W + 12, HP = H + 12;
  T* X = (T*)sm3;
  T* R = X + (size_t)H * WP * V;
  float ninf[V];
#pragma unroll
  for (int k = 0; k < V; ++k) ninf[k] = -INFINITY;
  for (int i = threadIdx.x; i < H * WP; i += 256) {
    const int h = i / WP, wp = i - h * WP, w = wp - 6;
    float v[V];
    if ((unsigned)w < (unsigned)W) ldv<T, V>(x + n * xsn + h * xsh + w * xsw + c0, v);
    else {
#pragma unroll
      for (int k = 0; k < V; ++k) v[k] = -INFINITY;
    }
    stv<T, V>(X + (size_t)i * V, v);
  }
  for (int i = threadIdx.x; i < 3 * 12 * W; i += 256) {
    const int pl = i / (12 * W), rem = i - pl * 12 * W, hr = rem / W, w = rem - hr * W;
    const int hp = hr < 6 ? hr : H + hr;
    stv<T, V>(R + ((size_t)(pl * HP + hp) * W + w) * V, ninf);
  }
  __syncthreads();
  for (int i = threadIdx.x; i < H * W; i += 256) {
    const int h = i / W, w = i - h * W;
    const T* row = X + ((size_t)h * WP + w) * V;
    float t[13][V];
#pragma unroll
    for (int j = 0; j < 13; ++j) ldv<T, V>(row + (size_t)j * V, t[j]);
    float m5[V], m9[V], m13[V];
#pragma unroll
    for (int k = 0; k < V; ++k) {
      m5[k] = pool_max(pool_max(pool_max(t[4][k], t[5][k]), pool_max(t[6][k], t[7][k])), t[8][k]);
      m9[k] = pool_max(pool_max(m5[k], pool_max(t[2][k], t[3][k])), pool_max(t[9][k], t[10][k]));
      m13[k] = pool_max(pool_max(m9[k], pool_max(t[0][k], t[1][k])), pool_max(t[11][k], t[12][k]));
    }
    stv<T, V>(R + ((size_t)(0 * HP + h + 6) * W + w) * V, m5);
    stv<T, V>(R + ((size_t)(1 * HP + h + 6) * W + w) * V, m9);
    stv<T, V>(R + ((size_t)(2 * HP + h + 6) * W + w) * V, m13);
  }
  __syncthreads();
  for (int i = threadIdx.x; i < H * W; i += 256) {
    const int h = i / W, w = i - h * W;
    float o[V], t[V];
#pragma unroll
    for (int k = 0; k < V; ++k) o[k] = -INFINITY;
#pragma unroll
    for (int j = 4; j <= 8; ++j) {
      ldv<T, V>(R + ((size_t)(0 * HP + h + j) * W + w) * V, t);
#pragma unroll
      for (int k = 0; k < V; ++k) o[k] = pool_max(o[k], t[k]);
    }
    stv<T, V>(y1 + n * s1n + h * s1h + w * s1w + c0, o);
#pragma unroll
    for (int k = 0; k < V; ++k) o[k] = -INFINITY;
#pragma unroll
    for (int j = 2; j <= 10; ++j) {
      ldv<T, V>(R + ((size_t)(1 * HP + h + j) * W + w) * V, t);
#pragma unroll
      for (int k = 0; k < V; ++k) o[k] = pool_max(o[k], t[k]);
    }
    stv<T, V>(y2 + n * s2n + h * s2h + w * s2w + c0, o);
#pragma unroll
    for (int k = 0; k < V; ++k) o[k] = -INFINITY;
#pragma unroll
    for (int j = 0; j <= 12; ++j) {
      ldv<T, V>(R + ((size_t)(2 * HP + h + j) * W + w) * V, t);
#pragma unroll
      for (int k = 0; k < V; ++k) o[k] = pool_max(o[k], t[k]);
    }
    stv<T, V>(y3 + n * s3n + h * s3h + w * s3w + c0, o);
  }
}
// ... 762 lines not shown
```

mgdt_yolo_amd/nn/modules/block.py:

```python
import torch
import torch.nn as nn

from ... import ops
from .conv import Conv, HipModule, act_code
from .convnextv2 import ConvNeXtV2_Block
from .spr_module import SPRModule

__all__ = ('DFL', 'SPPF', 'C2f', 'MSPA_C2f', 'Bottleneck', 'SimFusion_4in', 'SimFusion_3in', 'IFM', 'h_sigmoid',
           'InjectionMultiSum_Auto_pool', 'Upsample')


def _plain_block(first, last, bottlenecks):
    def conv_ok(c, k):
        return (isinstance(c, Conv) and c.plain_affine() and c.conv.kernel_size == (k, k) and c.conv.stride == (1, 1) and c.conv.groups == 1
                and act_code(c.act) == a0)
    try:
        a0 = act_code(first.act)
    except RuntimeError:
        return False
    if a0 != ops.ACT_SILU:
        return False
    if not (conv_ok(first, 1) and conv_ok(last, 1)) or len(bottlenecks) == 0:
        return False
    return all(isinstance(m, Bottleneck) and conv_ok(m.cv1, 3) and conv_ok(m.cv2, 3) and m.add == bottlenecks[0].add
               and m.cv1.conv.in_channels == m.cv1.conv.out_channels == m.cv2.conv.out_channels for m in bottlenecks)


class DFL(nn.Module):

    def __init__(self, c1=16):
        super().__init__()
        self.conv = nn.Conv2d(c1, 1, 1, bias=False).requires_grad_(False)
        self.conv.weight.data[:] = torch.arange(c1, dtype=torch.float).view(1, c1, 1, 1)
        self.c1 = c1


class Bottleneck(HipModule):

    def __init__(self, c1, c2, shortcut=True, g=1, k=(3, 3), e=0.5):
        super().__init__()
        c_ = int(c2 * e)
        k0 = k[0][0] if isinstance(k[0], (tuple, list)) else k[0]
        k1 = k[1][0] if isinstance(k[1], (tuple, list)) else k[1]
        self.cv1 = Conv(c1, c_, k0, 1)
        self.cv2 = Conv(c_, c2, k1, 1, g=g)
        self.add = shortcut and c1 == c2

    def run(self, x, out=None, x2=None):
        if self.training and hasattr(self.cv1, 'bn'):
            t = self.cv1.train_fwd(x, x2=x2)
            return self.cv2.train_fwd(t, out=out, r1=x if self.add else None, r2=x2 if self.add else None)
        t = self.cv1.run(x, x2=x2)
        return self.cv2.run(t, out=out, r1=x if self.add else None, r2=x2 if self.add else None)

    def backward(self, gz, acc_into=None):
        gmid = self.cv2.backward(gz)
        return self.cv1.backward(gmid, dx_out=acc_into, acc=acc_into is not None, r2=gz if self.add else None)

    def forward(self, x):
        return self.run(x)


class C2f(HipModule):

    def __init__(self, c1, c2, n=1, shortcut=False, g=1, e=0.5):
        super().__init__()
        self.c = int(c2 * e)
        self.cv1 = Conv(c1, 2 * self.c, 1, 1)
        self.cv2 = Conv((2 + n) * self.c, c2, 1)
        self.m = nn.ModuleList(Bottleneck(self.c, self.c, shortcut, g, k=((3, 3), (3, 3)), e=1.0) for _ in range(n))

    def forward(self, x, head=None):
        if head is not None:
            x_l = head[1][0]
            dt0 = self.cv1.out_dtype(x_l)
            ok = (not (self.training and hasattr(self.cv1, 'bn')) and _plain_block(self.cv1, self.cv2, self.m) and ops.csp_block_supported(
                ops.CSP_C2F, ops.new_act(x_l.shape[0], 2 * self.c, x_l.shape[2], x_l.shape[3], dt0, x_l.device), self.cv2.conv.out_channels, self.c, len(self.m), dt0))
            y01 = head[0].forward_into_conv(head[1], self.cv1) if ok else None
            if y01 is None:
                x = head[0](head[1])
            else:
                mids = [pk for m in self.m for pk in (m.cv1.packed(y01.dtype, False), m.cv2.packed(y01.dtype, False))]
                return ops.csp_block(ops.CSP_C2F, y01, None, None, mids, self.m[0].add, self.cv2.packed(y01.dtype, False), self.c, act_code(self.cv1.act),
                                     self.cv2.conv.out_channels, False)[0]
        b, _, h, w = x.shape
        c, n = self.c, len(self.m)
        train = self.training and hasattr(self.cv1, 'bn')
        dt = self.cv1.out_dtype(x)
        if not train and x.dtype == dt and _plain_block(self.cv1, self.cv2, self.m):
            y01 = ops.new_act(b, 2 * c, h, w, dt, x.device)
            if ops.csp_block_supported(ops.CSP_C2F, y01, self.cv2.conv.out_channels, c, n, dt):
                self.cv1.run(x, out=y01)
                mids = [pk for m in self.m for pk in (m.cv1.packed(dt, False), m.cv2.packed(dt, False))]
                return ops.csp_block(ops.CSP_C2F, y01, None, None, mids, self.m[0].add, self.cv2.packed(dt, False), c, act_code(self.cv1.act),
                                     self.cv2.conv.out_channels, False)[0]
        cat = ops.new_act(b, (2 + n) * c, h, w, dt, x.device)
        (self.cv1.train_fwd if train else self.cv1.run)(x, out=cat[:, :2 * c])
        for j, m in enumerate(self.m):
            m.run(cat[:, (1 + j) * c:(2 + j) * c], out=cat[:, (2 + j) * c:(3 + j) * c])
        return (self.cv2.train_fwd if train else self.cv2.run)(cat)

    forward_split = forward

    def backward(self, g):
        c, n = self.c, len(self.m)
        gcat = self.cv2.backward(g)
        for j in reversed(range(n)):
            self.m[j].backward(gcat[:, (2 + j) * c:(3 + j) * c], acc_into=gcat[:, (1 + j) * c:(2 + j) * c])
        return self.cv1.backward(gcat[:, :2 * c])


class MSPA_C2f(HipModule):

    def __init__(self, inplanes, outplanes, n=1, shortcut=False, g=1, e=0.5, scale=4, stride=1, stype='normal'):
        super().__init__()
        self.nums = scale
        self.inwidth = inplanes // self.nums
        self.outwidth = outplanes // self.nums
        self.stride = stride
        assert stype in ['stage', 'normal'], 'One of these is suppported (stage or normal)'
        self.stype = stype
        self.convs = nn.ModuleList([])
        self.btnk_nums = n
        for i in range(self.nums):
            if self.stride == 1 and i != self.nums - 1:
                self.convs.append(Conv(self.inwidth, self.inwidth, 1, 1))
            else:
                self.convs.append(Conv(inplanes + self.outwidth * (n - 1), outplanes, 1, 1))
        self.bottleneck = nn.ModuleList(Bottleneck(self.inwidth, self.inwidth, shortcut, g, k=((3, 3), (3, 3)), e=1.0) for _ in range(n))
        self.attention = SPRModule(self.outwidth)
        self.softmax = nn.Softmax(dim=1)

    def forward(self, x, deliver=None):
        if self.stride != 1:
            raise RuntimeError('MSPA_C2f: only stride=1 is wired by parse_model and built here')
        d_out = deliver.get('out') if deliver else None
        d_pools = deliver.get('pools', ()) if deliver else ()
        b, _, h, w = x.shape
        wd, s, n = self.inwidth, self.nums, self.btnk_nums
        train = self.training and hasattr(self.convs[0], 'bn')
        run = (lambda m: m.train_fwd) if train else (lambda m: m.run)
        dt = self.convs[0].out_dtype(x)
        at = self.attention
        if (not train and s == 4 and self.inwidth == self.outwidth and self._chain_ok() and _plain_block(self.convs[0], self.convs[3], self.bottleneck)
                and ops.csp_block_supported(ops.CSP_MSPA, x, self.convs[3].conv.out_channels, wd, n, dt)):
            mids = [pk for m in self.bottleneck for pk in (m.cv1.packed(dt, False), m.cv2.packed(dt, False))]
            out, pool, slots, tiles = ops.csp_block(ops.CSP_MSPA, x, self._packed_chain(dt).blob, None, mids, self.bottleneck[0].add,
                                                    self.convs[3].packed(dt, False), wd, act_code(self.convs[0].act), self.convs[3].conv.out_channels, True)
            return ops.spr_attention_scale(out, at.fc1.weight, at.fc1.bias, at.fc2.weight, at.fc2.bias, s, out=d_out, part=pool, nsplit=slots, tiles=tiles, pools=d_pools)
        cat = ops.new_act(b, (s - 1 + n) * wd, h, w, dt, x.device)
        if not train and s == 4 and ops.pw_chain_supported(wd, cat.dtype) and x.dtype == cat.dtype and self._chain_ok():
            ops.pw_chain3(x[:, :3 * wd], self._packed_chain(cat.dtype), act_code(self.convs[0].act), cat[:, :3 * wd])
        else:
            run(self.convs[0])(x[:, :wd], out=cat[:, :wd])
            for i in range(1, s - 1):
                run(self.convs[i])(cat[:, (i - 1) * wd:i * wd], x2=x[:, i * wd:(i + 1) * wd], out=cat[:, i * wd:(i + 1) * wd])
        src, pending = cat[:, (s - 2) * wd:(s - 1) * wd], x[:, (s - 1) * wd:s * wd]
        for j, m in enumerate(self.bottleneck):
            dst = cat[:, (s - 1 + j) * wd:(s + j) * wd]
            m.run(src, out=dst, x2=pending)
            src, pending = dst, None
        out = run(self.convs[s - 1])(cat)
        if train:
            attn, part = ops.spr_attention_train(out, at.fc1.weight, at.fc1.bias, at.fc2.weight, at.fc2.bias, s)
            self._save_ctx((out, attn, part, x.shape))
        else:
            return ops.spr_attention_scale(out, at.fc1.weight, at.fc1.bias, at.fc2.weight, at.fc2.bias, s, out=d_out, pools=d_pools)
        return ops.scale_channels(out, attn)

    def _chain_ok(self):
        cs = list(self.convs)[:3]
        return all(c.plain_affine() and c.conv.kernel_size == (1, 1) and c.conv.groups == 1 and c.conv.in_channels == self.inwidth
                   and c.conv.out_channels == self.inwidth and act_code(c.act) == act_code(cs[0].act) for c in cs)

    def _packed_chain(self, dtype):
        cs = list(self.convs)[:3]
        tens = [t for c in cs for t in c.affine_tensors()]
        return self._cached(('chain', dtype), tens, lambda: ops.PackedPwChain([(c.conv.weight, c.conv.bias, c.bn_tuple()) for c in cs], dtype))

    def backward(self, g):
        out, attn, part, xshape = self._ctx.pop()
        wd, s, n = self.inwidth, self.nums, self.btnk_nums
        at = self.attention
        dattn = ops.nc_reduce(g, out)
        prms = (at.fc1.weight, at.fc1.bias, at.fc2.weight, at.fc2.bias)
        gb = [ops.grad_buf(p) for p in prms]
        chained = all(t.is_contiguous() and t.dtype == torch.float32 for t in gb) and all(
            a.untyped_storage().data_ptr() == b.untyped_storage().data_ptr() and a.storage_offset() + a.numel() == b.storage_offset() for a, b in zip(gb, gb[1:]))
        pg_out = gb[0].new_empty(0).set_(gb[0].untyped_storage(), gb[0].storage_offset(), (sum(t.numel() for t in gb),)) if chained else None
        gout, pg = ops.spr_bwd(g, part, attn, dattn, at.fc1.weight, at.fc1.bias, at.fc2.weight, at.fc2.bias, s, out=pg_out)
        if not chained:
            o = 0
            for prm, t in zip(prms, gb):
                t.copy_(pg[o:o + t.numel()].view_as(prm))
                o += t.numel()
        gcat = self.convs[s - 1].backward(gout)
        gx = ops.new_act(xshape[0], xshape[1], xshape[2], xshape[3], g.dtype, g.device)
        sl = lambda t, i: t[:, i * wd:(i + 1) * wd]
        for j in reversed(range(n)):
            if j > 0:
                self.bottleneck[j].backward(sl(gcat, s - 1 + j), acc_into=sl(gcat, s - 2 + j))
                continue
            gin = self.bottleneck[j].backward(sl(gcat, s - 1 + j))
            dst = sl(gcat, s - 2 + j)
            ops.add(dst, gin, out=dst)
            ops.copy(gin, sl(gx, s - 1))
        for i in reversed(range(1, s - 1)):
            gi = self.convs[i].backward(sl(gcat, i), dx_out=sl(gx, i))
            dst = sl(gcat, i - 1)
            ops.add(dst, gi, out=dst)
        self.convs[0].backward(sl(gcat, 0), dx_out=sl(gx, 0))
        return gx


class SPPF(HipModule):

    def __init__(self, c1, c2, k=5):
        super().__init__()
        if k != 5:
            raise RuntimeError('SPPF: k=5 is what the YAMLs use and what the fused pooling kernel implements')
        c_ = c1 // 2
        self.cv1 = Conv(c1, c_, 1, 1)
        self.cv2 = Conv(c_ * 4, c2, 1, 1)
        self.m = nn.MaxPool2d(kernel_size=k, stride=1, padding=k // 2)

    def forward(self, x):
        b, _, h, w = x.shape
        c_ = self.cv1.conv.out_channels
        train = self.training and hasattr(self.cv1, 'bn')
        cat = ops.new_act(b, 4 * c_, h, w, self.cv1.out_dtype(x), x.device)
        (self.cv1.train_fwd if train else self.cv1.run)(x, out=cat[:, :c_])
        ops.sppf_pools(cat[:, :c_], cat[:, c_:2 * c_], cat[:, 2 * c_:3 * c_], cat[:, 3 * c_:])
        if train:
            self._cat = cat if ops.ctx_enabled() else None
        return (self.cv2.train_fwd if train else self.cv2.run)(cat)

    def backward(self, g):
        c_ = self.cv1.conv.out_channels
        cat, self._cat = self._cat, None
        gcat = self.cv2.backward(g)
        sl = lambda t, i: t[:, i * c_:(i + 1) * c_]
        g2 = ops.add(sl(gcat, 2), ops.maxpool5_bwd(sl(cat, 2), sl(gcat, 3)))
        g1 = ops.add(sl(gcat, 1), ops.maxpool5_bwd(sl(cat, 1), g2))
        g0 = ops.add(sl(gcat, 0), ops.maxpool5_bwd(sl(cat, 0), g1))
        return self.cv1.backward(g0)


class Upsample(nn.Module):

    def __init__(self, size=None, scale_factor=None, mode='nearest'):
        super().__init__()
        if mode != 'nearest' or size is not None:
            raise RuntimeError("Upsample: only (None, scale_factor, 'nearest') is on the detection path")
        self.scale_factor, self.mode, self.size = scale_factor, mode, size

    def forward(self, x):
        b, c, h, w = x.shape
        out = ops.new_act(b, c, int(h * self.scale_factor), int(w * self.scale_factor), x.dtype, x.device)
        return ops.nearest(x, out)

    def backward(self, g):
        b, c, h, w = g.shape
        return ops.nearest_bwd(g, ops.new_act(b, c, int(h / self.scale_factor), int(w / self.scale_factor), g.dtype, g.device))


class SimFusion_4in(nn.Module):

    def forward(self, x, pre=None):
        x_l, x_m, x_s, x_n = x
        b, c, h, w = x_s.shape
        cs = [x_l.shape[1], x_m.shape[1], c, x_n.shape[1]]
        self._shapes = [t.shape for t in x]
        out, done = None, ()
        if pre is not None and pre.get('out') is not None and tuple(pre['out'].shape) == (b, sum(cs), h, w) and pre['out'].dtype == x_s.dtype:
            out, done = pre['out'], pre['done']
        if out is None:
            out = ops.new_act(b, sum(cs), h, w, x_s.dtype, x_s.device)
        o = 0
        if 0 not in done:
            ops.adaptive_avgpool(x_l, out[:, o:o + cs[0]])
        o += cs[0]
        if 1 not in done:
            ops.adaptive_avgpool(x_m, out[:, o:o + cs[1]])
        o += cs[1]
        if not (2 in done and x_s.data_ptr() == out[:, o:o + cs[2]].data_ptr()):
            ops.copy(x_s, out[:, o:o + cs[2]])
        o += cs[2]
        ops.bilinear(x_n, out[:, o:o + cs[3]])
        return out

    def backward(self, g):
        sh = self._shapes
        mk = lambda i: ops.new_act(sh[i][0], sh[i][1], sh[i][2], sh[i][3], g.dtype, g.device)
        c0, c1, c2 = sh[0][1], sh[0][1] + sh[1][1], sh[0][1] + sh[1][1] + sh[2][1]
        return [ops.adaptive_avgpool_bwd(g[:, :c0], mk(0)), ops.adaptive_avgpool_bwd(g[:, c0:c1], mk(1)), g[:, c1:c2],
                ops.bilinear_bwd(g[:, c2:], mk(3))]


class SimFusion_3in(HipModule):

    def __init__(self, in_channel_list, out_channels):
        super().__init__()
        self.cv1 = Conv(in_channel_list[0], out_channels, act=nn.ReLU()) if in_channel_list[0] != out_channels else nn.Identity()
        self.cv2 = Conv(in_channel_list[1], out_channels, act=nn.ReLU()) if in_channel_list[1] != out_channels else nn.Identity()
        self.cv3 = Conv(in_channel_list[2], out_channels, act=nn.ReLU()) if in_channel_list[2] != out_channels else nn.Identity()
        self.cv_fuse = Conv(out_channels * 3, out_channels, act=nn.ReLU())

    def forward(self, x, pre=None):
        b, _, h, w = x[1].shape
        oc = self.cv_fuse.conv.out_channels
        dt, dev = x[1].dtype, x[1].device
        self._shapes = [t.shape for t in x]
        cat, done, pooled0 = None, (), None
        if pre is not None and pre.get('out') is not None and tuple(pre['out'].shape) == (b, 3 * oc, h, w) and pre['out'].dtype == dt:
            cat, done, pooled0 = pre['out'], pre['done'], pre.get('pooled0')
        if cat is None:
            cat = ops.new_act(b, 3 * oc, h, w, dt, dev)
        if isinstance(self.cv1, nn.Identity):
            if 0 not in done:
                ops.adaptive_avgpool(x[0], cat[:, :oc])
        else:
            if pooled0 is None or tuple(pooled0.shape) != (b, x[0].shape[1], h, w):
                pooled0 = ops.adaptive_avgpool(x[0], ops.new_act(b, x[0].shape[1], h, w, dt, dev))
            (self.cv1.train_fwd if (self.training and hasattr(self.cv1, 'bn')) else self.cv1.run)(pooled0, out=cat[:, :oc])
        if isinstance(self.cv2, nn.Identity):
            if not (1 in done and x[1].data_ptr() == cat[:, oc:2 * oc].data_ptr()):
                ops.copy(x[1], cat[:, oc:2 * oc])
        else:
            (self.cv2.train_fwd if (self.training and hasattr(self.cv2, 'bn')) else self.cv2.run)(x[1], out=cat[:, oc:2 * oc])
        if isinstance(self.cv3, nn.Identity):
            ops.bilinear(x[2], cat[:, 2 * oc:])
        else:
            (self.cv3.train_fwd if (self.training and hasattr(self.cv3, 'bn')) else self.cv3.run)(
                ops.bilinear(x[2], ops.new_act(b, x[2].shape[1], h, w, dt, dev)), out=cat[:, 2 * oc:])
        return self.cv_fuse(cat)

    def backward(self, g):
        oc = self.cv_fuse.conv.out_channels
        sh = self._shapes
        mk = lambda i: ops.new_act(sh[i][0], sh[i][1], sh[i][2], sh[i][3], g.dtype, g.device)
        gcat = self.cv_fuse.backward(g)
        g0 = gcat[:, :oc] if isinstance(self.cv1, nn.Identity) else self.cv1.backward(gcat[:, :oc])
        g1 = gcat[:, oc:2 * oc] if isinstance(self.cv2, nn.Identity) else self.cv2.backward(gcat[:, oc:2 * oc])
        g2 = gcat[:, 2 * oc:] if isinstance(self.cv3, nn.Identity) else self.cv3.backward(gcat[:, 2 * oc:])
        return [ops.adaptive_avgpool_bwd(g0, mk(0)), g1, ops.bilinear_bwd(g2, mk(2))]


class IFM(nn.Module):

    def __init__(self, inc, ouc, embed_dim_p=96, fuse_block_num=3) -> None:
        super().__init__()
        self.conv = nn.Sequential(Conv(inc, embed_dim_p), *[ConvNeXtV2_Block(embed_dim_p) for _ in range(fuse_block_num)],
                                  Conv(embed_dim_p, sum(ouc)))

    def forward(self, x):
        mods = list(self.conv)
        if (not self.training and len(mods) >= 2 and isinstance(mods[-2], ConvNeXtV2_Block) and not mods[-2]._forward_hooks and not self.conv._forward_hooks):
            for m in mods[:-2]:
                x = m(x)
            r = mods[-2](x, tail=mods[-1])
            return r[0] if isinstance(r, tuple) else mods[-1](r)
        return self.conv(x)

    def backward(self, g):
        for m in reversed(list(self.conv)):
            g = m.backward(g)
        return g


class h_sigmoid(nn.Module):

    def __init__(self, inplace=True):
        super().__init__()
        self.relu = nn.ReLU6(inplace=inplace)


class InjectionMultiSum_Auto_pool(HipModule):

    def __init__(self, inp: int, oup: int, global_inp: list, flag: int) -> None:
        super().__init__()
        self.global_inp = global_inp
        self.flag = flag
        self.local_embedding = Conv(inp, oup, 1, act=False)
        self.global_embedding = Conv(global_inp[self.flag], oup, 1, act=False)
        self.global_act = Conv(global_inp[self.flag], oup, 1, act=False)
        self.act = h_sigmoid()

    def _merged_global(self, g, xq=None):
        a, b = self.global_act, self.global_embedding
        ok = all(m.plain_affine() and act_code(m.act) == ops.ACT_NONE and m.conv.kernel_size == (1, 1) and m.conv.groups == 1 for m in (a, b))
        dt = a.out_dtype(g)
        fused = not hasattr(a, 'bn')
        if (not ok or fused != (not hasattr(b, 'bn')) or (not fused and a.bn.eps != b.bn.eps) or a.conv.out_channels % 8
                or not ops.conv_can_mfma(g, a.conv.in_channels, a.conv.out_channels + b.conv.out_channels, 1, 1, 1, dt)):
            return None
        tens = [t for m in (a, b) for t in m.affine_tensors()]
        cat = lambda fn: torch.cat([fn(a).detach().float(), fn(b).detach().float()])
        zb = lambda m: m.conv.bias if m.conv.bias is not None else torch.zeros(m.conv.out_channels, device=m.conv.weight.device)
        bn = lambda: None if fused else (cat(lambda m: m.bn.weight), cat(lambda m: m.bn.bias), cat(lambda m: m.bn.running_mean), cat(lambda m: m.bn.running_var), a.bn.eps)
        cb = lambda: cat(zb) if fused else None
        if xq is not None:
            return self._cached(('gaf', 'fp8', float(xq)), tens, lambda: ops.PackedConvFp8(cat(lambda m: m.conv.weight), cb(), bn(), 1, xq))
        return self._cached(('gaf', dt), tens, lambda: ops.PackedConv(cat(lambda m: m.conv.weight), cb(), bn(), 1, dt))

    def forward_into_conv(self, x, conv):
        x_l, x_g = x
        le = self.local_embedding
        if self.training or not isinstance(conv, Conv) or not conv.plain_affine() or not le.plain_affine():
            return None
        if ops.Q8_CALIB is not None or self.__dict__.get('_q8') or conv.__dict__.get('_q8') or le.__dict__.get('_q8'):
            return None
        dt = le.out_dtype(x_l)
        c0 = sum(self.global_inp[:self.flag])
        g = x_g[:, c0:c0 + self.global_inp[self.flag]]
        pk2g = self._merged_global(g)
        if (pk2g is None or dt != torch.bfloat16 or act_code(le.act) != ops.ACT_NONE or le.conv.kernel_size != (1, 1)
                or le.conv.groups != 1 or conv.conv.kernel_size != (1, 1) or conv.conv.stride != (1, 1) or conv.conv.groups != 1
                or conv.conv.in_channels != le.conv.out_channels):
            return None
        oc = self.global_act.conv.out_channels
        b, _, h, w = x_l.shape
        gh, gw = g.shape[2], g.shape[3]
        probe = ops.new_act(1, oc, gh, gw, dt, x_l.device)
        if not ops.conv1x1_inject_conv_supported(x_l, oc, conv.conv.out_channels, probe, dt):
            return None
        in_launch = g.shape[1] == 32 and oc == 256 and ops.FUSED_INJECT_GCONV
        if not in_launch:
            gaf = ops.conv2d(g, pk2g, 1, ops.ACT_NONE)
            ga, gf = gaf[:, :oc], gaf[:, oc:]
            if ga.stride() != gf.stride():
                return None
        pk2 = conv._cached(('acc_order', dt), conv.affine_tensors(), lambda: ops.PackedConv(
            conv.conv.weight.detach()[:, ops.acc_order_index(conv.conv.in_channels, conv.conv.weight.device)], conv.conv.bias, conv.bn_tuple(), 1, dt))
        out = ops.new_act(b, conv.conv.out_channels, h, w, dt, x_l.device)
        if in_launch:
            return ops.conv1x1_inject_conv(x_l, le.packed(dt, direct=False), None, None, pk2, act_code(conv.act), out, gsrc=g, pkg=pk2g)
        return ops.conv1x1_inject_conv(x_l, le.packed(dt, direct=False), ga, gf, pk2, act_code(conv.act), out)

    def forward(self, x):
        x_l, x_g = x
        c0 = sum(self.global_inp[:self.flag])
        g = x_g[:, c0:c0 + self.global_inp[self.flag]]
        train = self.training and hasattr(self.local_embedding, 'bn')
        f = (lambda m: m.train_fwd) if train else (lambda m: m.run)
        pk2 = None if train else self._merged_global(g)
        if pk2 is not None:
            xq = self.q8_site(('gaf',), g) if pk2.dtype == torch.bfloat16 else None
            gaf = ops.conv2d(g, pk2, 1, ops.ACT_NONE) if xq is None else ops.conv2d_fp8(g, self._merged_global(g, xq), 1, ops.ACT_NONE)
            oc = self.global_act.conv.out_channels
            ga, gf = gaf[:, :oc], gaf[:, oc:]
        else:
            ga = f(self.global_act)(g)
            gf = f(self.global_embedding)(g)
        le = self.local_embedding
        dt = le.out_dtype(x_l)
        if (not train and le.plain_affine() and act_code(le.act) == ops.ACT_NONE and le.conv.kernel_size == (1, 1) and le.conv.groups == 1
                and ops.conv1x1_inject_supported(x_l, le.conv.out_channels, ga, dt) and ga.stride() == gf.stride()):
            return ops.conv1x1_inject(x_l, le.packed(dt, direct=False), ga, gf)
        local = f(le)(x_l)
        if train:
            self._save_ctx((local, ga, x_g.shape, c0))
        return ops.inject(local, ga, gf)

    def backward(self, g):
        local, ga, gshape, c0 = self._ctx.pop()
        b, c, h, w = local.shape
        use_pool = h < ga.shape[2]
        small = lambda: ops.new_act(ga.shape[0], ga.shape[1], ga.shape[2], ga.shape[3], g.dtype, g.device)
# ... 19 lines not shown
```

mgdt_yolo_amd/nn/tasks.py:

```python
import ast
import contextlib
import math
import re
from copy import deepcopy
from pathlib import Path

import torch
import torch.nn as nn

from .. import ops
from ..yolo.utils.torch_utils import fuse_conv_and_bn, initialize_weights, intersect_dicts, make_divisible
from .modules import (C2f, IFM, MSPA_C2f, SPPF, Bottleneck, Concat, Conv, Detect, DWConv, InjectionMultiSum_Auto_pool,
                      SimFusion_3in, SimFusion_4in, TOODHead, Upsample)

REGISTRY = {c.__name__: c for c in (Conv, DWConv, Concat, Bottleneck, C2f, MSPA_C2f, SPPF, SimFusion_4in, SimFusion_3in, IFM,
                                    InjectionMultiSum_Auto_pool, Detect, TOODHead)}
REGISTRY['nn.Upsample'] = Upsample


class _TrainForwardFn(torch.autograd.Function):

    @staticmethod
    def forward(ctx, model, x, anchor):
        with ops.force_ctx():
            feats = model._predict_once(x)
        ctx.model = model
        ctx.n = len(feats)
        return tuple(feats)

    @staticmethod
    def backward(ctx, *gfeats):
        model = ctx.model
        gfeats = [g if g.is_contiguous(memory_format=torch.channels_last) else g.contiguous(memory_format=torch.channels_last) for g in gfeats]
        acc = model._accumulate_snapshot() if getattr(model, 'grad_accumulate', False) else None
        model.backward(gfeats)
        if acc is not None:
            model._accumulate_restore(acc)
        return None, None, None


class BaseModel(nn.Module):

    def forward(self, x, *args, **kwargs):
        if isinstance(x, dict):
            return self.loss(x, *args, **kwargs)
        return self.predict(x, *args, **kwargs)

    def predict(self, x, profile=False, visualize=False, augment=False):
        if profile or visualize:
            raise RuntimeError('profile / visualize are host-side tooling outside the hot path')
        if augment:
            if self.training or not hasattr(self, '_predict_augment'):
                raise RuntimeError('augment=True is an inference call form: put the detection model in eval() (augmented training is not built)')
            return self._predict_augment(x)
        if self.training and torch.is_grad_enabled() and any(p.requires_grad for p in self.model[0].parameters()):
            if not hasattr(self, '_anchor'):
                self._anchor = torch.zeros((), device=x.device, requires_grad=True)
            return list(_TrainForwardFn.apply(self, x, self._anchor))
        return self._predict_once(x)

    def _predict_once(self, x, profile=False, visualize=False):
        if not x.is_cuda:
            raise RuntimeError('mgdt_yolo_amd runs on MI355X (HIP) only: move the model and the input to cuda (no CPU fallback)')
        if self.training:
            for m in self.modules():
                m.__dict__.pop('_ctx', None)
        y = []
        layers = self.model
        if not self.training and self._stem_fusable(x):
            m0, m1 = self.model[0], self.model[1]
            pk0 = m0._cached(('stem2',), m0.affine_tensors(), lambda: ops.PackedStem2(m0.conv.weight, m0.folded_bn_like()))
            x = ops.stem2(x, pk0, m1.packed(torch.bfloat16, direct=False))
            y = [None, x if 1 in self.save else None]
            layers = list(self.model)[2:]
        plan = self._neck_plan(x) if not self.training else None
        bufs = {}
        head = None
        side = self._side_branch() if not self.training else None
        first = layers[0].i
        y += [None] * (len(self.model) - len(y))
        prev = {first - 1: x}

        def run(m):
            nonlocal head
            src = lambda j: prev[m.i - 1] if j == -1 else y[m.i + j if j < 0 else j]
            xin = src(m.f) if isinstance(m.f, int) else [src(j) for j in m.f]
            if head is not None:
                out, head = m(None, head=head), None
            elif self._injection_feeds_next(m):
                head, out = (m, xin), None
            elif plan is not None and m.i in plan['producers']:
                out = m(xin, deliver=self._neck_deliveries(plan, m, xin, bufs))
            elif plan is not None and m.i in plan['consumers']:
                out = m(xin, pre=bufs.get(m.i))
            else:
                out = m(xin)
            prev.pop(m.i - 1, None)
            prev[m.i] = out
            y[m.i] = out if m.i in self.save else None

        if side is None or side[2] < first:
            for m in layers:
                run(m)
            return prev[len(self.model) - 1]
        s0, s1, dep = side
        main, other = torch.cuda.current_stream(), ops.side_stream(x.device)
        for m in layers:
            if s0 <= m.i <= s1:
                continue
            if m.i == s1 + 1:
                main.wait_stream(other)
            run(m)
            if m.i == dep:
                other.wait_stream(main)
                with torch.cuda.stream(other):
                    for k in range(s0, s1 + 1):
                        run(self.model[k])
        if s1 + 1 >= len(self.model):
            main.wait_stream(other)
        return prev[len(self.model) - 1]

    def _side_branch(self):
        if not ops.SIDE_STREAM:
            return None
        if '_side_branch_cache' not in self.__dict__:
            absf = lambda m: [m.i + f if f < 0 else f for f in ([m.f] if isinstance(m.f, int) else m.f)]
            best = None
            n = len(self.model)
            for s0 in range(2, n - 1):
                deps, s1 = set(), s0 - 1
                for k in range(s0, n - 1):
                    ext = {j for j in absf(self.model[k]) if j < s0}
                    if ext and max(ext) >= s0 - 1:
                        break
                    deps |= ext
                    s1 = k
                if s1 < s0 or not deps:
                    continue
                dep = max(deps)
                if best is None or (s0 - 1 - dep, s1 - s0) > (best[0] - 1 - best[2], best[1] - best[0]):
                    best = (s0, s1, dep)
            self.__dict__['_side_branch_cache'] = best
        best = self.__dict__['_side_branch_cache']
        if best is None or any(self.model[k]._forward_hooks for k in range(best[2] + 1, best[1] + 1)):
            return None
        return best

    def _injection_feeds_next(self, m):
        if (self.training or not ops.FUSED_INJECT_CONV or getattr(self, 'compute_dtype', None) != torch.bfloat16 or not isinstance(m, InjectionMultiSum_Auto_pool)
                or m.i in self.save or m.i + 1 >= len(self.model)):
            return False
        nxt = self.model[m.i + 1]
        return isinstance(nxt, C2f) and nxt.f == -1 and not m._forward_hooks and not nxt._forward_hooks and len(nxt.m) >= 1

    def _neck_plan(self, x):
        if not ops.FUSED_NECK or getattr(self, 'compute_dtype', None) != torch.bfloat16 or not hasattr(self, '_reductions'):
            return None
        plan = self.__dict__.get('_neck_plan_cache')
        if plan is None:
            prod, cons = {}, set()
            absf = lambda m: [m.i + f if f < 0 else f for f in ([m.f] if isinstance(m.f, int) else m.f)]
            for m in self.model:
                if isinstance(m, SimFusion_4in):
                    src = absf(m)
                    kinds = ('pool', 'pool', 'main')
                elif isinstance(m, SimFusion_3in):
                    src = absf(m)
                    kinds = ('pool', 'main' if isinstance(m.cv2, nn.Identity) else None)
                else:
                    continue
                for slot, kind in enumerate(kinds):
                    j = src[slot]
                    if kind is None or not isinstance(self.model[j], MSPA_C2f):
                        continue
                    if kind == 'main' and any(k == 'main' for k, _, _ in prod.get(j, [])):
                        continue
                    prod.setdefault(j, []).append((kind, m.i, slot))
                    cons.add(m.i)
            plan = self.__dict__['_neck_plan_cache'] = {'producers': prod, 'consumers': cons} if prod else False
        if not plan:
            return None
        if any(self.model[i]._forward_hooks for i in list(plan['producers']) + list(plan['consumers'])):
            return None
        return plan

    def _neck_deliveries(self, plan, m, x, bufs):
        b, c, h, w = x.shape
        out, pools = None, []
        red = self._reductions
        absf = lambda mm: [mm.i + f if f < 0 else f for f in ([mm.f] if isinstance(mm.f, int) else mm.f)]
        for kind, ci, slot in plan['producers'][m.i]:
            cm = self.model[ci]
            src = absf(cm)
            tgt = src[2] if isinstance(cm, SimFusion_4in) else src[1]
            if red[tgt] % red[m.i]:
                continue
            F = int(red[tgt] // red[m.i])
            if F < 1 or h % F or w % F or (kind == 'main' and F != 1) or (kind == 'pool' and F == 1):
                continue
            th, tw = h // F, w // F
            if isinstance(cm, SimFusion_4in):
                cs = [self.model[j].c2 for j in src]
                total, off = sum(cs), sum(cs[:slot])
            else:
                oc = cm.cv_fuse.conv.out_channels
                total, off = 3 * oc, slot * oc
            st = bufs.setdefault(ci, {'out': None, 'done': set()})
            if st['out'] is None:
                st['out'] = ops.new_act(b, total, th, tw, x.dtype, x.device)
            if tuple(st['out'].shape) != (b, total, th, tw):
                continue
            if isinstance(cm, SimFusion_3in) and slot == 0 and not isinstance(cm.cv1, nn.Identity):
                st['pooled0'] = ops.new_act(b, c, th, tw, x.dtype, x.device)
                pools.append(st['pooled0'])
                continue
            view = st['out'][:, off:off + c]
            if kind == 'pool':
                pools.append(view)
            else:
                out = view
            st['done'].add(slot)
        return {'out': out, 'pools': pools[:2]} if (out is not None or pools) else None

    def _stem_fusable(self, x):
        if not ops.FUSED_STEM or getattr(self, 'compute_dtype', None) != torch.bfloat16 or len(self.model) < 3 or 0 in self.save:
            return False
        if x.dtype not in (torch.bfloat16, torch.float32, torch.uint8) or x.dim() != 4 or x.shape[1] != 3:
            return False
        m0, m1 = self.model[0], self.model[1]
        for m, (ci, co) in ((m0, (3, 16)), (m1, (16, 32))):
            if not (isinstance(m, Conv) and not isinstance(m, DWConv) and m.plain_affine() and isinstance(m.act, nn.SiLU) and m.f == -1 and not m._forward_hooks
                    and m.conv.kernel_size == (3, 3) and m.conv.stride == (2, 2) and m.conv.padding == (1, 1) and m.conv.groups == 1
                    and m.conv.in_channels == ci and m.conv.out_channels == co):
                return False
        return True

    def backward(self, head_grads, layer_done=None):
        with ops.defer_wgrad():
            self._backward_layers(head_grads, layer_done)

    def _backward_layers(self, head_grads, layer_done):
        n = len(self.model)
        pend = {n - 1: head_grads}
        for m in reversed(list(self.model)):
            g = pend.pop(m.i, None)
            if g is None:
                if layer_done is not None:
                    layer_done(m.i)
                continue
            if not hasattr(m, 'backward'):
                raise NotImplementedError(f'{type(m).__name__}.backward is not built yet (training path of this module: next)')
            first = m.i == 0
            gin = m.backward(g, need_dx=False) if (first and isinstance(m, Conv)) else m.backward(g)
            srcs = [m.f] if isinstance(m.f, int) else list(m.f)
            gins = [gin] if isinstance(m.f, int) else list(gin)
            for f, gi in zip(srcs, gins):
                if gi is None:
                    continue
                j = m.i - 1 if f == -1 else (f if f >= 0 else m.i + f)
                if j < 0:
                    continue
                if j in pend:
                    dst = pend[j] if (pend[j].is_contiguous(memory_format=torch.channels_last) and pend[j].shape == gi.shape) else None
                    pend[j] = ops.add(pend[j], gi, out=dst) if dst is not None else ops.add(pend[j], gi)
                else:
                    pend[j] = gi
            if layer_done is not None:
                layer_done(m.i)

    def _accumulate_snapshot(self):
        fs = getattr(self, '_flat_state', None)
        if fs is not None:
            return fs.grad.clone()
        return [(p, p.grad.clone()) for p in self.parameters() if p.requires_grad and p.grad is not None]

    def _accumulate_restore(self, snap):
        if torch.is_tensor(snap):
            self._flat_state.grad.add_(snap)
            return
        for p, g in snap:
            p.grad.add_(g)

    def fuse(self, verbose=True):
        if not self.is_fused():
            for m in self.model.modules():
                if isinstance(m, (Conv, DWConv)) and hasattr(m, 'bn'):
                    m.conv = fuse_conv_and_bn(m.conv, m.bn)
                    delattr(m, 'bn')
                    m.forward = m.forward_fuse
                    m.__dict__.pop('_pk', None)
        return self

    def is_fused(self, thresh=10):
        bn = tuple(v for k, v in nn.__dict__.items() if 'Norm' in k)
        return sum(isinstance(v, bn) for v in self.modules()) < thresh

    def info(self, detailed=False, verbose=True, imgsz=640):
        n_p = sum(x.numel() for x in self.parameters())
        n_l = len(list(self.modules()))
        if verbose:
            print(f'{Path(self.yaml.get("yaml_file", "model")).stem} summary: {n_l} layers, {n_p} parameters')
        return n_l, n_p

    def _apply(self, fn):
        self = super()._apply(fn)
        m = self.model[-1]
        if isinstance(m, Detect):
            m.stride = fn(m.stride)
            m.anchors = fn(m.anchors)
            m.strides = fn(m.strides)
        return self

    def load(self, weights, verbose=True):
        model = weights['model'] if isinstance(weights, dict) and 'model' in weights else weights
        csd = {k: v.float() for k, v in (model.state_dict() if isinstance(model, nn.Module) else model).items()}
        csd = intersect_dicts(csd, self.state_dict())
        self.load_state_dict(csd, strict=False)
        if verbose:
            print(f'Transferred {len(csd)}/{len(self.model.state_dict())} items from pretrained weights')

    def loss(self, batch, preds=None):
        if not hasattr(self, 'criterion'):
            self.criterion = self.init_criterion()
        preds = self.forward(batch['img']) if preds is None else preds
        return self.criterion(preds, batch)

    def init_criterion(self):
        raise NotImplementedError('compute_loss() needs to be implemented by task heads')

    def half(self):
        return self.set_compute_dtype(torch.bfloat16)

    def float(self):
        return self.set_compute_dtype(torch.float32)

    def quantize_fp8(self, calib, headroom=2.0, exclude=(), percentile=None):
        import math
        self.set_compute_dtype(torch.bfloat16)
        was_training = self.training
        self.eval()
        self.dequantize_fp8()
        stats = {}
        ops.Q8_CALIB, ops.Q8_CALIB_PCT = stats, percentile
        try:
            with torch.no_grad():
                for xb in (calib if isinstance(calib, (list, tuple)) else [calib]):
                    self._predict_once(xb)
        finally:
            ops.Q8_CALIB, ops.Q8_CALIB_PCT = None, None
            self.train(was_training)
        names = {m: n for n, m in self.named_modules()}
        table = {}
        for (m, key), amax in stats.items():
            if any(e in names.get(m, '?') + '.' for e in exclude):
                continue
            q = 1.0 if not (amax > 0.0 and math.isfinite(amax)) else 2.0 ** math.floor(math.log2(448.0 / (headroom * amax)))
            m.__dict__.setdefault('_q8', {})[key] = q
            table[names.get(m, '?') + ('' if key is None else ':' + '/'.join(str(k) for k in key))] = q
        self.fp8_table = table
        return table

    def dequantize_fp8(self):
        for m in self.modules():
            m.__dict__.pop('_q8', None)
        self.fp8_table = {}
        return self

    def set_compute_dtype(self, dtype):
        ops.dtype_code(dtype)
        for m in self.modules():
            if hasattr(m, 'out_dtype'):
                m._cdtype = dtype
        self.compute_dtype = dtype
        return self

# ... 283 lines not shown
```

mgdt_yolo_amd/ops.py:

```python
import ctypes as C
import os

import torch

from . import _lib as L
from ._lib import ACT_GELU, ACT_NONE, ACT_RELU, ACT_SILU, BF16, F32, View

U8 = 2
_DT = {torch.float32: F32, torch.bfloat16: BF16}


def dtype_code(dt):
    try:
        return _DT[dt]
    except KeyError:
        raise RuntimeError(f'mgdt_yolo_amd computes in float32 or bfloat16, not {dt}') from None


def _need_gpu(t):
    if not t.is_cuda:
        raise RuntimeError('mgdt_yolo_amd runs on MI355X (HIP) only: got a CPU tensor and there is no CPU/PyTorch fallback')


_PROF = None
# ... 127 lines not shown
            nbytes = lib.mgdt_conv_packed_bytes(cin_g, cout, k, code)
            self.w = torch.empty(nbytes, dtype=torch.uint8, device=dev)
            self.bias = torch.empty((cout + 15) // 16 * 16, dtype=torch.float32, device=dev)
            _launch('conv_pack', 'mgdt_conv_pack', ptr(weight), ptr(cb), ptr(g), ptr(b), ptr(mu), ptr(var), eps, cin_g, cout, k, code,
                                       ptr(self.w), ptr(self.bias), stream())
            if groups == 1:
                _register_pack(self, (weight, cb, g, b, mu, var, float(eps), cin_g, cout, k, code, 0))


class PackedConvFp8:
    __slots__ = ('w', 'bias', 'oscale', 'xq', 'k', 'cin', 'cout', 'dtype', 'direct', 'groups', '__weakref__')

    def __init__(self, weight, conv_bias, bn, k, xq):
        lib = L.lib()
        weight = weight.detach().float().contiguous()
        _need_gpu(weight)
        cout, cin = weight.shape[0], weight.shape[1]
        dev = weight.device
        g, b, mu, var, eps = (None, None, None, None, 0.0) if bn is None else bn
        f = lambda t: None if t is None else t.detach().float().contiguous()
        g, b, mu, var, cb = f(g), f(b), f(mu), f(var), f(conv_bias)
        self.k, self.cin, self.cout, self.dtype, self.direct, self.groups, self.xq = k, cin, cout, torch.bfloat16, False, 1, float(xq)
        self.w = torch.empty(lib.mgdt_conv_packed_bytes_fp8(cin, cout, k), dtype=torch.uint8, device=dev)
        cpad = (cout + 15) // 16 * 16
        self.bias = torch.empty(cpad, dtype=torch.float32, device=dev)
        self.oscale = torch.empty(cpad, dtype=torch.float32, device=dev)
        _launch('conv_pack_fp8', 'mgdt_conv_pack_fp8', ptr(weight), ptr(cb), ptr(g), ptr(b), ptr(mu), ptr(var), eps, cin, cout, k, self.xq,
                ptr(self.w), ptr(self.bias), ptr(self.oscale), stream())


Q8_CALIB = None
Q8_CALIB_PCT = None


def conv2d_fp8(x, pk, stride, act, out=None, x2=None, r1=None, r2=None, in_scale=None, in_shift=None):
    _need_gpu(x)
    b, _, h, w = x.shape
    ho, wo = conv_out_hw(h, w, pk.k, stride)
    if out is None:
        out = new_act(b, pk.cout, ho, wo, torch.bfloat16, x.device)
    _same(x, x2, r1, r2, out)
    if x.dtype != torch.bfloat16:
        raise RuntimeError(f'conv2d_fp8: activations are bf16 in HBM, the input is {x.dtype}')
    if _PROF is not None:
        _META['conv2d_fp8_fwd'] = dict(shape=(b, pk.cin, h, w, pk.cout, pk.k, stride), flops=2.0 * b * ho * wo * pk.cout * pk.cin * pk.k * pk.k,
                                       bytes=float(b * h * w * pk.cin * 2 + b * ho * wo * pk.cout * 2 + pk.cout * pk.cin * pk.k * pk.k))
    _launch('conv2d_fp8_fwd', 'mgdt_conv2d_fp8_fwd', vp(x), vp(x2), ptr(in_scale), ptr(in_shift), ptr(pk.w), ptr(pk.bias), ptr(pk.oscale), pk.xq,
            pk.k, stride, act, vp(r1), vp(r2), vp(out), stream())
    return out


_PACK_REGISTRY = None
LIVE_STORAGES = set()


def _register_pack(obj, src):
    global _PACK_REGISTRY
    import weakref
    if not all(t is None or t.untyped_storage().data_ptr() in LIVE_STORAGES for t in src[:6]):
        return
    if _PACK_REGISTRY is None:
        _PACK_REGISTRY = weakref.WeakSet()
    obj.src, obj.epoch = src, PARAM_EPOCH[0]
    _PACK_REGISTRY.add(obj)


def repack_all():
    if not _PACK_REGISTRY:
        return []
    live = [o for o in _PACK_REGISTRY if getattr(o, 'epoch', -2) == PARAM_EPOCH[0] - 1]
    if not live:
        return []
    arr = (L.PackDesc * len(live))()
    for d, o in zip(arr, live):
        w, cb, g, b, mu, var, eps, cin, cout, k, code, mode = o.src
        d.w, d.conv_bias, d.bn_gamma, d.bn_beta, d.bn_mean, d.bn_var = ptr(w), ptr(cb), ptr(g), ptr(b), ptr(mu), ptr(var)
        d.bn_eps, d.cin, d.cout, d.k, d.dtype, d.mode = eps, cin, cout, k, code, mode
        d.packed, d.bias_out = ptr(o.w), ptr(o.bias)
    _launch('conv_pack_batch', 'mgdt_conv_pack_batch', arr, len(live), stream())
    for o in live:
        o.epoch = PARAM_EPOCH[0]
    return live


def pack_is_current(obj):
    return getattr(obj, 'epoch', None) == PARAM_EPOCH[0]


def conv_can_mfma(x, cin, cout, k, s, groups, dtype):
    pe = 8 if dtype == torch.bfloat16 else 4
    return (groups == 1 and k in (1, 3) and s in (1, 2) and cin % pe == 0 and cout % 4 == 0 and x.dtype == dtype
            and is_nhwc(x) and x.stride(3) % pe == 0 and x.stride(2) % pe == 0 and x.stride(0) % pe == 0
            and x.data_ptr() % 16 == 0)


def conv_out_hw(h, w, k, s):
    p = k // 2
    return (h + 2 * p - k) // s + 1, (w + 2 * p - k) // s + 1


def conv2d(x, pk, stride, act, out=None, x2=None, r1=None, r2=None, in_scale=None, in_shift=None):
    _need_gpu(x)
    b, _, h, w = x.shape
    ho, wo = conv_out_hw(h, w, pk.k, stride)
    if out is None:
        out = new_act(b, pk.cout, ho, wo, pk.dtype, x.device)
    if _PROF is not None:
        es = out.element_size()
        _META['conv2d_direct_fwd' if pk.direct else 'conv2d_fwd'] = dict(
            shape=(b, pk.cin, h, w, pk.cout, pk.k, stride), flops=2.0 * b * ho * wo * pk.cout * pk.cin // pk.groups * pk.k * pk.k,
            bytes=float(b * h * w * pk.cin * x.element_size() + b * ho * wo * pk.cout * es + pk.w.numel() * pk.w.element_size()))
    if pk.direct:
        if x2 is not None or r1 is not None or r2 is not None or in_scale is not None or in_shift is not None:
            raise RuntimeError('direct convolution path has no fused extras')
        _launch('conv2d_direct_fwd', 'mgdt_conv2d_direct_fwd', vp(x), U8 if x.dtype == torch.uint8 else dtype_code(x.dtype), ptr(pk.w), ptr(pk.bias), pk.k, stride, pk.groups, act,
                                           vp(out), dtype_code(out.dtype), stream())
    else:
        _same(x, x2, r1, r2, out)
        if x.dtype != pk.dtype:
            raise RuntimeError(f'conv2d: the weights are packed for {pk.dtype}, the input is {x.dtype}')
        _launch('conv2d_fwd', 'mgdt_conv2d_fwd', vp(x), vp(x2), ptr(in_scale), ptr(in_shift), ptr(pk.w), ptr(pk.bias), pk.k, stride, act,
                                    vp(r1), vp(r2), vp(out), dtype_code(pk.dtype), stream())
    return out


def spr_attention(x, fc1_w, fc1_b, fc2_w, fc2_b, groups, softmax=True):
    b, c, h, w = x.shape
    lib = L.lib()
    part = torch.empty(b * L.SPR_SPLITS * c * 5, dtype=torch.float32, device=x.device)
    _launch('spr_pool_fwd', 'mgdt_spr_pool_fwd', vp(x), ptr(part), dtype_code(x.dtype), stream())
    attn = torch.empty(b, c, dtype=torch.float32, device=x.device)
    _launch('spr_attn_fwd', 'mgdt_spr_attn_fwd', ptr(part), ptr(fc1_w), ptr(fc1_b), ptr(fc2_w), ptr(fc2_b), b, c, groups, h, w, int(bool(softmax)),
            ptr(attn), stream())
    return attn


def spr_attention_scale(x, fc1_w, fc1_b, fc2_w, fc2_b, groups, out=None, part=None, nsplit=0, tiles=(0, 0), pools=()):
    b, c, h, w = x.shape
    if part is None:
        part = torch.empty(b * L.SPR_SPLITS * c * 5, dtype=torch.float32, device=x.device)
        _launch('spr_pool_fwd', 'mgdt_spr_pool_fwd', vp(x), ptr(part), dtype_code(x.dtype), stream())
        nsplit, tiles = L.SPR_SPLITS, (0, 0)
    out = like(x) if out is None else out
    pools = list(pools)
    if len(pools) > 2:
        raise RuntimeError('spr_attention_scale: at most two pooled outputs')
    _same(x, out, *pools)
    pa, pb = (pools + [None, None])[:2]
    _launch('spr_attn_scale_fwd', 'mgdt_spr_attn_scale_fwd', ptr(part), int(nsplit), int(tiles[0]), int(tiles[1]), ptr(fc1_w), ptr(fc1_b), ptr(fc2_w), ptr(fc2_b), groups, vp(x), vp(out),
            vp(pa), vp(pb), dtype_code(x.dtype), stream())
    return out


FUSED_NECK = True


FUSED_STEM = True


class PackedStem2:

    def __init__(self, weight, bn):
        g, b, mu, var, eps = bn
        scale = (g.detach().float() / torch.sqrt(eps + var.detach().float()))
        wf = (weight.detach().float() * scale.view(-1, 1, 1, 1)).contiguous()
        self.bias = (b.detach().float() - g.detach().float() * mu.detach().float() / torch.sqrt(var.detach().float() + eps)).contiguous()
        self.blob = torch.empty(L.lib().mgdt_stem2_packed_bytes(), dtype=torch.uint8, device=weight.device)
        L.check(L.lib().mgdt_stem2_pack(ptr(wf), ptr(self.blob), stream()), 'stem2_pack')


def stem2(x, pk0, pk1):
    _need_gpu(x)
    b, _, h, w = x.shape
    h0, w0 = (h - 1) // 2 + 1, (w - 1) // 2 + 1
    h1, w1 = (h0 - 1) // 2 + 1, (w0 - 1) // 2 + 1
    y = new_act(b, 32, h1, w1, torch.bfloat16, x.device)
    if _PROF is not None:
        _META['stem2_fwd'] = dict(shape=(b, 3, h, w, 32, 3, 4), flops=2.0 * b * (h0 * w0 * 16 * 27 + h1 * w1 * 32 * 144),
                                  bytes=float(x.numel() * x.element_size() + y.numel() * 2))
    _launch('stem2_fwd', 'mgdt_stem2_fwd', vp(x), U8 if x.dtype == torch.uint8 else dtype_code(x.dtype), ptr(pk0.blob), ptr(pk0.bias), ptr(pk1.w), ptr(pk1.bias),
            vp(y), stream())
    return y


FUSED_CSP_BLOCK = True
CSP_MSPA, CSP_C2F = 0, 1


def csp_block_supported(mode, x, cout, wd, nbtl, dtype):
    if not (FUSED_CSP_BLOCK and dtype == torch.bfloat16 and x.dtype == dtype and is_nhwc(x)):
        return False
    lib = L.lib()
    if not lib.mgdt_csp_block_supported(mode, x.shape[1], int(cout), int(wd), int(nbtl), x.shape[2], x.shape[3], dtype_code(dtype)):
        return False
    return lib.mgdt_csp_block_tiles(mode, x.shape[0], x.shape[1], int(cout), int(wd), int(nbtl), x.shape[2], x.shape[3], None) > 0


def csp_block(mode, x, front, front_bias, mids, shortcut, back, wd, act, cout, want_pool):
    lib = L.lib()
    b, cin, h, w = x.shape
    nb = len(mids) // 2
    geom = (C.c_int * 8)()
    slots = lib.mgdt_csp_block_tiles(mode, b, cin, cout, wd, nb, h, w, geom)
    if slots <= 0:
        raise RuntimeError('csp_block: configuration not covered')
    y = new_act(b, cout, h, w, x.dtype, x.device)
    pool = torch.empty(b * slots * cout, dtype=torch.float32, device=x.device) if want_pool else None
    marr = (C.c_void_p * len(mids))(*[m.w.data_ptr() for m in mids])
    barr = (C.c_void_p * len(mids))(*[m.bias.data_ptr() for m in mids])
    if _PROF is not None:
        es = x.element_size()
        catc = (3 if mode == CSP_MSPA else 2) * wd + nb * wd
        fl = 2.0 * b * h * w * ((3 * wd * wd if mode == CSP_MSPA else 0) + 2 * nb * 9 * wd * wd + catc * cout)
        _META['csp_block_fwd'] = dict(shape=(b, cin, h, w, cout, wd, nb), flops=fl, bytes=float(b * h * w * (cin + cout) * es))
    _launch('csp_block_fwd', 'mgdt_csp_block_fwd', mode, vp(x), ptr(front), ptr(front_bias), marr, barr, nb, int(bool(shortcut)), ptr(back.w), ptr(back.bias),
            int(wd), act, vp(y), ptr(pool), dtype_code(x.dtype), stream())
    return y, pool, slots, (geom[6], geom[7])


def scale_channels(x, attn, out=None):
    out = like(x) if out is None else out
    _same(x, out)
    _launch('scale_channels_fwd', 'mgdt_scale_channels_fwd', vp(x), ptr(attn), vp(out), dtype_code(x.dtype), stream())
    return out


def sppf_pools(x, y1, y2, y3):
    _launch('sppf_pool_fwd', 'mgdt_sppf_pool_fwd', vp(x), vp(y1), vp(y2), vp(y3), dtype_code(x.dtype), stream())


def adaptive_avgpool(x, out):
    _same(x, out)
    _launch('adaptive_avgpool_fwd', 'mgdt_adaptive_avgpool_fwd', vp(x), vp(out), dtype_code(x.dtype), stream())
    return out


def bilinear(x, out):
    _same(x, out)
    _launch('bilinear_fwd', 'mgdt_bilinear_fwd', vp(x), vp(out), dtype_code(x.dtype), stream())
    return out


def nearest(x, out):
    _same(x, out)
    _launch('nearest_fwd', 'mgdt_nearest_fwd', vp(x), vp(out), dtype_code(x.dtype), stream())
    return out


def copy(x, out):
    _launch('copy_fwd', 'mgdt_copy_fwd', vp(x), U8 if x.dtype == torch.uint8 else dtype_code(x.dtype), vp(out), dtype_code(out.dtype), stream())
    return out


def dwconv7_ln(x, dw_w49c, dw_b, ln_w, ln_b, eps, out=None):
    out = like(x) if out is None else out
    _launch('dwconv7_ln_fwd', 'mgdt_dwconv7_ln_fwd', vp(x), ptr(dw_w49c), ptr(dw_b), ptr(ln_w), ptr(ln_b), eps, vp(out), dtype_code(x.dtype),
                                        stream())
    return out


def grn_scale(t, gamma):
    b, c = t.shape[:2]
    ws = torch.empty(b * L.GRN_SPLITS * c, dtype=torch.float32, device=t.device)
    sc = torch.empty(b, c, dtype=torch.float32, device=t.device)
    _launch('grn_stats_fwd', 'mgdt_grn_stats_fwd', vp(t), ptr(gamma), ptr(ws), ptr(sc), dtype_code(t.dtype), stream())
    return sc


FUSED_PW_CHAIN = True


def pw_chain_supported(wd, dtype):
    return FUSED_PW_CHAIN and L.lib().mgdt_pw_chain_packed_bytes(int(wd), dtype_code(dtype)) > 0


class PackedPwChain:

    def __init__(self, convs, dtype):
        wd = convs[0][0].shape[0]
        self.wd, self.dtype = wd, dtype
        self.blob = torch.empty(L.lib().mgdt_pw_chain_packed_bytes(wd, dtype_code(dtype)), dtype=torch.uint8, device=convs[0][0].device)
        f = lambda t: None if t is None else t.detach().float().contiguous()
        for i, (w, cb, bn) in enumerate(convs):
            g, b, mu, var, eps = (None, None, None, None, 0.0) if bn is None else bn
            w, cb, g, b, mu, var = f(w), f(cb), f(g), f(b), f(mu), f(var)
            L.check(L.lib().mgdt_pw_chain_pack(i, ptr(w), ptr(cb), ptr(g), ptr(b), ptr(mu), ptr(var), eps, wd, dtype_code(dtype), ptr(self.blob), stream()),
                    'pw_chain_pack')


def pw_chain3(x, pk, act, out):
    if _PROF is not None:
        b, c, h, w = x.shape
        _META['pw_chain3_fwd'] = dict(shape=(b, pk.wd, h, w, pk.wd, 1, 1), flops=2.0 * b * h * w * pk.wd * pk.wd * 3, bytes=float(2 * b * h * w * c * x.element_size()))
    _launch('pw_chain3_fwd', 'mgdt_pw_chain3_fwd', vp(x), ptr(pk.blob), pk.wd, act, vp(out), dtype_code(x.dtype), stream())
    return out


FUSED_CNX_MLP = True


def cnx_mlp_supported(c, dtype):
    return FUSED_CNX_MLP and L.lib().mgdt_cnx_mlp_packed_bytes(int(c), dtype_code(dtype)) > 0


class PackedCnxMlp:

# ... 672 lines not shown
```

Baseline: 39640 images/sec.

## Defer SPR channel scaling into following stride-2 3x3 conv with fused pooling

Instead of materializing the SPR-attention-scaled tensor, the attention factors are computed separately, and the next stride-2 3x3 LDS conv applies the per-channel scale while staging its input. The same kernel also emits the 2x and 4x average-pooled copies needed by the GD neck. This avoids a full read/write pass over the activation in the scale kernel. In exchange it adds scaling ALU work and pooling work inside the conv's staging loop, plus a new kernel variant and more complex routing logic in the model.

Result: no change. 39790 images/sec (median of 6 runs) (+0.4%).

```diff
diff --git a/include/mgdt.h b/include/mgdt.h
--- a/include/mgdt.h
+++ b/include/mgdt.h
@@ -38,6 +38,9 @@
 int mgdt_conv2d_fwd(const mgdt_view* x, const mgdt_view* x2, const float* in_scale, const float* in_shift,
                     const void* packed_w, const float* bias, int k, int stride, int act, const mgdt_view* r1,
                     const mgdt_view* r2, const mgdt_view* y, int dtype, mgdt_stream s);
+int mgdt_conv3x3_s2_scaled_supported(int n, int h, int w, int cin, int cout, int act);
+int mgdt_conv3x3_s2_scaled_fwd(const mgdt_view* x, const float* in_scale, const void* packed_w, const float* bias, int act, const mgdt_view* y,
+                               const mgdt_view* pool_a, const mgdt_view* pool_b, mgdt_stream s);
 size_t mgdt_conv_packed_bytes_fp8(int cin, int cout, int k);
 int mgdt_conv_pack_fp8(const float* w_oihw, const float* conv_bias, const float* bn_gamma, const float* bn_beta, const float* bn_mean,
                        const float* bn_var, float bn_eps, int cin, int cout, int k, float x_qscale, void* packed_out, float* bias_out,
@@ -118,6 +121,9 @@
 int mgdt_scale_channels_fwd(const mgdt_view* x, const float* attn, const mgdt_view* y, int dtype, mgdt_stream s);
 int mgdt_spr_attn_scale_fwd(const float* pooled, int nsplit, int tiles_x, int tiles_y, const float* fc1_w, const float* fc1_b, const float* fc2_w, const float* fc2_b, int groups,
                             const mgdt_view* x, const mgdt_view* y, const mgdt_view* pool_a, const mgdt_view* pool_b, int dtype, mgdt_stream s);
+
+int mgdt_spr_attn_tiles_fwd(const float* pooled, int nsplit, int tiles_x, int tiles_y, const float* fc1_w, const float* fc1_b, const float* fc2_w, const float* fc2_b, int groups,
+                            int n, int c, int h, int w, float* attn, mgdt_stream s);
 
 int mgdt_sppf_pool_fwd(const mgdt_view* x, const mgdt_view* y1, const mgdt_view* y2, const mgdt_view* y3, int dtype,
                        mgdt_stream s);
diff --git a/mgdt_yolo_amd/_lib.py b/mgdt_yolo_amd/_lib.py
--- a/mgdt_yolo_amd/_lib.py
+++ b/mgdt_yolo_amd/_lib.py
@@ -69,6 +69,9 @@
     'mgdt_conv1x1_inject_conv_supported': (_i, [_i, _i, _i, _i, _i, _i, _i, _i]),
     'mgdt_conv1x1_inject_conv_fwd': (_i, [VP, _vp, _vp, VP, VP, VP, _vp, _vp, _i, _vp, _vp, _i, VP, _i, _vp]),
     'mgdt_spr_attn_scale_fwd': (_i, [_vp, _i, _i, _i, _vp, _vp, _vp, _vp, _i, VP, VP, VP, VP, _i, _vp]),
+    'mgdt_spr_attn_tiles_fwd': (_i, [_vp, _i, _i, _i, _vp, _vp, _vp, _vp, _i, _i, _i, _i, _i, _vp, _vp]),
+    'mgdt_conv3x3_s2_scaled_supported': (_i, [_i, _i, _i, _i, _i, _i]),
+    'mgdt_conv3x3_s2_scaled_fwd': (_i, [VP, _vp, _vp, _vp, _i, VP, VP, VP, _vp]),
     'mgdt_stem2_packed_bytes': (_sz, []),
     'mgdt_stem2_pack': (_i, [_vp, _vp, _vp]),
     'mgdt_stem2_fwd': (_i, [VP, _i, _vp, _vp, _vp, _vp, VP, _vp]),
diff --git a/mgdt_yolo_amd/csrc/conv3x3_lds.hip b/mgdt_yolo_amd/csrc/conv3x3_lds.hip
--- a/mgdt_yolo_amd/csrc/conv3x3_lds.hip
+++ b/mgdt_yolo_amd/csrc/conv3x3_lds.hip
@@ -8,6 +8,7 @@
 #define C3_RW 18
 #define C3_MAXI 14
 
+struct C3Pool { char* y; int sn, sh, sw; };
 struct C3Args {
   const char* x; int xsn, xsh, xsw; uint32_t x_bytes;
   char* y; int ysn, ysh, ysw; uint32_t y_bytes;
@@ -15,6 +16,7 @@
   int N, H, W, Ho, Wo, Cin, Cout, CP, nchunks, NTtot, ncg, tiles_x, tiles_per_img, ntiles, XP, act;
   FastDiv fd_tpi, fd_tx, fd_cp;
   const float* oscale; float xq;
+  const float* in_scale; C3Pool p2, p4;
   unsigned long long* dbg;
 };
 
@@ -24,7 +26,7 @@
   return v;
 }
 
-template <int NBW, int ACT, int NCH, int MT, bool Q8 = false, int S = 1, int WS = 1>
+template <int NBW, int ACT, int NCH, int MT, bool Q8 = false, int S = 1, int WS = 1, bool SC = false>
 __global__ __launch_bounds__(256 * WS, 1) void conv3x3_lds_kernel(const C3Args a) {
   constexpr int NTHR = 256 * WS, NBH = (NBW + WS - 1) / WS;
   constexpr int RW = 15 * S + 3, TH = 4 * MT, RH = (TH - 1) * S + 3, RPX = RH * RW;
@@ -76,8 +78,13 @@
 
   const int nitems = RPX * a.CP;
   uint4 stage[MAXI];
+  f32x4 sc[2];
+  const bool scaled = SC && a.in_scale != nullptr;
+  const int c8t = SC ? tid - (int)fdiv((uint32_t)tid, a.fd_cp) * a.CP : 0;
   auto issue = [&](int t) {
     const int n = (int)fdiv((uint32_t)t, a.fd_tpi), rt = t - n * a.tiles_per_img;
+    if constexpr (SC)
+      if (scaled) { const f32x4* sp = (const f32x4*)(a.in_scale + (size_t)n * a.Cin + c8t * 8); sc[0] = sp[0]; sc[1] = sp[1]; }
     const int tyi = (int)fdiv((uint32_t)rt, a.fd_tx), txi = rt - tyi * a.tiles_x;
     const int iy0 = tyi * TH * S - 1, ix0 = txi * C3_TW * S - 1;
 #pragma unroll
@@ -96,6 +103,13 @@
       const int it = tid + u * NTHR;
       if (it < nitems) {
         const int pix = (int)fdiv((uint32_t)it, a.fd_cp), c8 = it - pix * a.CP;
+        if constexpr (SC)
+          if (scaled) {
+            bf16x8 v = __builtin_bit_cast(bf16x8, stage[u]);
+#pragma unroll
+            for (int k = 0; k < 8; ++k) v[k] = (bf16)((float)v[k] * sc[k >> 2][k & 3]);
+            stage[u] = __builtin_bit_cast(uint4, v);
+          }
         if constexpr (Q8) *(long*)(xs + pix * a.XP + c8 * 8) = quant8(__builtin_bit_cast(bf16x8, stage[u]), a.xq);
         else *(uint4*)(xs + pix * a.XP + c8 * 16) = stage[u];
       }
@@ -119,6 +133,34 @@
     if (a.dbg) { const unsigned long long n_ = __builtin_amdgcn_s_memrealtime(); Tc += n_ - tl; tl = n_; }
     const int tn = t + wstep;
     if (tn < a.ntiles) issue(tn);
+    if constexpr (SC) {
+      if (cg == 0 && (a.p2.y || a.p4.y)) {
+        const int n = (int)fdiv((uint32_t)t, a.fd_tpi), rt = t - n * a.tiles_per_img;
+        const int tyi = (int)fdiv((uint32_t)rt, a.fd_tx), txi = rt - tyi * a.tiles_x;
+        auto pool = [&](const C3Pool& P, const int F) __attribute__((always_inline)) {
+          const int cw = 32 / F, ch = 2 * TH / F, Hp = a.H / F, Wp = a.W / F;
+          for (int it = tid; it < ch * cw * a.CP; it += NTHR) {
+            const int cell = (int)fdiv((uint32_t)it, a.fd_cp), c8 = it - cell * a.CP;
+            const int cy = cell / cw, cx = cell - cy * cw, gy = tyi * ch + cy, gx = txi * cw + cx;
+            if (gy >= Hp || gx >= Wp) continue;
+            float acc[8] = {0.f, 0.f, 0.f, 0.f, 0.f, 0.f, 0.f, 0.f};
+            for (int yy = 0; yy < F; ++yy)
+              for (int xx = 0; xx < F; ++xx) {
+                const bf16x8 v = *(const bf16x8*)(xs + ((1 + cy * F + yy) * RW + 1 + cx * F + xx) * a.XP + c8 * 16);
+#pragma unroll
+                for (int k = 0; k < 8; ++k) acc[k] += (float)v[k];
+              }
+            const float inv = 1.f / (float)(F * F);
+            bf16x8 o;
+#pragma unroll
+            for (int k = 0; k < 8; ++k) o[k] = (bf16)(acc[k] * inv);
+            *(bf16x8*)(P.y + (size_t)n * P.sn + (size_t)gy * P.sh + (size_t)gx * P.sw + c8 * 16) = o;
+          }
+        };
+        if (a.p2.y) pool(a.p2, 2);
+        if (a.p4.y) pool(a.p4, 4);
+      }
+    }
 
     f32x4 acc[NBH][MT];
 #pragma unroll
@@ -192,13 +234,15 @@
 }
 
 bool mgdt_conv3x3_lds_launch(const mgdt_view* x, const mgdt_view* y, const void* packed_w, const float* bias, int act, int CP, int nchunks, int NTtot, hipStream_t st,
-                             const float* q8_oscale, float q8_xq, int stride) {
+                             const float* q8_oscale, float q8_xq, int stride, const float* in_scale, const mgdt_view* pool2, const mgdt_view* pool4, bool dry) {
   const bool q8 = q8_oscale != nullptr;
   static const int mode = getenv("MGDT_CONV3_LDS") ? atoi(getenv("MGDT_CONV3_LDS")) : 1;
   if (!mode) return false;
   static const bool ws2 = !(getenv("MGDT_C3_WAVES8") && atoi(getenv("MGDT_C3_WAVES8")) == 0);
   const bool wide = mode >= 3 || ws2;
   const int Cin = x->c, Cout = y->c;
+  if ((in_scale || pool2 || pool4) && (stride != 2 || q8 || !ws2 || (CP != 4 && CP != 8) || ((uintptr_t)in_scale & 15))) return false;
+  if ((pool2 && (x->h % 2 || x->w % 2)) || (pool4 && (x->h % 4 || x->w % 4))) return false;
   if (stride == 2 && (q8_oscale || Cin > 64 || NTtot % 4 || (nchunks != 9 && !(nchunks == 18 && wide)))) return false;
   if (Cin % 8 || Cin < 32 || Cin > 80 || Cout % 4 || Cout < 32 || (act != MGDT_ACT_SILU && act != MGDT_ACT_NONE && act != MGDT_ACT_RELU)) return false;
   const long M = (long)x->n * x->h * x->w;
@@ -235,6 +279,10 @@
   nwg = (int)std::min<long>(nwg, (long)a.ntiles * a.ncg);
   nwg = nwg / a.ncg * a.ncg;
   if (nwg < a.ncg) return false;
+  if (dry) return true;
+  a.in_scale = in_scale;
+  if (pool2) a.p2 = C3Pool{(char*)pool2->p, (int)(pool2->sn * 2), (int)(pool2->sh * 2), (int)(pool2->sw * 2)};
+  if (pool4) a.p4 = C3Pool{(char*)pool4->p, (int)(pool4->sn * 2), (int)(pool4->sh * 2), (int)(pool4->sw * 2)};
  #define C3_LAUNCH_Q8(NB, ACTV)                                                                                      \
   {                                                                                                                  \
     static std::atomic<bool> qattr{false}, qattr18{false}, qattr23{false};                                            \
@@ -272,8 +320,11 @@
   a.dbg = dbgbuf;
 #define C3_LAUNCH_S2(ACTV, NCHV)                                                                                      \
   {                                                                                                                  \
-    static std::atomic<bool> sattr{false}, sattr8{false};                                                            \
-    if (ws2) {                                                                                                       \
+    static std::atomic<bool> sattr{false}, sattr8{false}, sattrc{false};                                             \
+    if (in_scale || pool2 || pool4) {                                                                                \
+      if (!sattrc) { (void)hipFuncSetAttribute((const void*)conv3x3_lds_kernel<4, ACTV, NCHV, 2, false, 2, 2, true>, hipFuncAttributeMaxDynamicSharedMemorySize, 160 * 1024); sattrc = true; } \
+      conv3x3_lds_kernel<4, ACTV, NCHV, 2, false, 2, 2, true><<<nwg, 512, lds, st>>>(a);                             \
+    } else if (ws2) {                                                                                                       \
       if (!sattr8) { (void)hipFuncSetAttribute((const void*)conv3x3_lds_kernel<4, ACTV, NCHV, 2, false, 2, 2>, hipFuncAttributeMaxDynamicSharedMemorySize, 160 * 1024); sattr8 = true; } \
       conv3x3_lds_kernel<4, ACTV, NCHV, 2, false, 2, 2><<<nwg, 512, lds, st>>>(a);                                   \
     } else {                                                                                                         \
diff --git a/mgdt_yolo_amd/csrc/conv_igemm.hip b/mgdt_yolo_amd/csrc/conv_igemm.hip
--- a/mgdt_yolo_amd/csrc/conv_igemm.hip
+++ b/mgdt_yolo_amd/csrc/conv_igemm.hip
@@ -306,7 +306,7 @@
 }
 
 bool mgdt_conv3x3_lds_launch(const mgdt_view* x, const mgdt_view* y, const void* packed_w, const float* bias, int act, int CP, int nchunks, int NTtot, hipStream_t st,
-                             const float* q8_oscale, float q8_xq, int stride);
+                             const float* q8_oscale, float q8_xq, int stride, const float* in_scale, const mgdt_view* pool2, const mgdt_view* pool4, bool dry);
 
 template <typename T, int NT, int MT, bool Q8>
 int launch_igemm(const ConvArgs& a, int gx, int gy, int threads, size_t lds, hipStream_t st);
@@ -336,6 +336,42 @@
                                const void* packed_w, const float* bias, int k, int stride, int act, const mgdt_view* r1,
                                const mgdt_view* r2, const mgdt_view* y, int dtype, mgdt_stream s) {
   return conv2d_fwd_impl(x, x2, in_scale, in_shift, packed_w, bias, k, stride, act, r1, r2, y, dtype, 0, s);
+}
+static bool c3s2_route(const mgdt_view* x, const mgdt_view* y, const void* packed_w, const float* bias, int act, const float* in_scale, const mgdt_view* p2,
+                       const mgdt_view* p4, bool dry, mgdt_stream s) {
+  int CP, nchunks, NTtot;
+  conv_geometry(x->c, y->c, 3, MGDT_BF16, &CP, &nchunks, &NTtot, 0);
+  return mgdt_conv3x3_lds_launch(x, y, packed_w, bias, act, CP, nchunks, NTtot, (hipStream_t)s, nullptr, 1.f, 2, in_scale, p2, p4, dry);
+}
+extern "C" int mgdt_conv3x3_s2_scaled_supported(int n, int h, int w, int cin, int cout, int act) {
+  if (n < 1 || h < 4 || w < 4 || h % 4 || w % 4 || cin < 8 || cin % 8 || cout < 4 || cout % 4) return 0;
+  mgdt_view x = {nullptr, n, h, w, cin, (long)h * w * cin, (long)w * cin, cin, 1};
+  mgdt_view y = {nullptr, n, h / 2, w / 2, cout, (long)(h / 2) * (w / 2) * cout, (long)(w / 2) * cout, cout, 1};
+  mgdt_view p2 = {nullptr, n, h / 2, w / 2, cin, (long)(h / 2) * (w / 2) * cin, (long)(w / 2) * cin, cin, 1};
+  mgdt_view p4 = {nullptr, n, h / 4, w / 4, cin, (long)(h / 4) * (w / 4) * cin, (long)(w / 4) * cin, cin, 1};
+  return c3s2_route(&x, &y, nullptr, nullptr, act, nullptr, &p2, &p4, true, nullptr) ? 1 : 0;
+}
+extern "C" int mgdt_conv3x3_s2_scaled_fwd(const mgdt_view* x, const float* in_scale, const void* packed_w, const float* bias, int act, const mgdt_view* y,
+                                          const mgdt_view* pool_a, const mgdt_view* pool_b, mgdt_stream s) {
+  if (!view_ok(x) || !view_ok(y) || !packed_w || !bias || !in_scale) MGDT_FAIL(MGDT_BAD_ARG, "conv3x3_s2_scaled: null/empty view, weights or factor");
+  auto nhwc16 = [](const mgdt_view* v) {
+    return v->sc == 1 && v->c % 8 == 0 && v->sw % 8 == 0 && v->sh % 8 == 0 && v->sn % 8 == 0 && ((uintptr_t)v->p & 15) == 0 && v->sn >= 0 && v->sh >= 0 && v->sw >= 0 &&
+           ((long)(v->n - 1) * v->sn + (long)(v->h - 1) * v->sh + (long)(v->w - 1) * v->sw + v->c) * 2 < 0x7fffffffL;
+  };
+  if (x->h % 2 || x->w % 2 || y->n != x->n || y->h != x->h / 2 || y->w != x->w / 2 || !nhwc16(x) || y->sc != 1 || y->c % 4 || y->sw % 4 || y->sh % 4 || y->sn % 4 || ((uintptr_t)y->p & 7))
+    MGDT_FAIL(MGDT_BAD_SHAPE, "conv3x3_s2_scaled: x must be an even-sized NHWC bf16 view with 16-byte pieces, y its stride-2 output");
+  const mgdt_view* p2 = nullptr; const mgdt_view* p4 = nullptr;
+  for (const mgdt_view* p : {pool_a, pool_b}) {
+    if (!p || !p->p) continue;
+    const int F = p->h > 0 ? x->h / p->h : 0;
+    if (!view_ok(p) || !nhwc16(p) || p->n != x->n || p->c != x->c || (F != 2 && F != 4) || p->h * F != x->h || p->w * F != x->w || (F == 2 ? p2 : p4))
+      MGDT_FAIL(MGDT_BAD_SHAPE, "conv3x3_s2_scaled: a pooled output must be an NHWC view of x's n, c and 1/2 or 1/4 of its size (one of each at most)");
+    (F == 2 ? p2 : p4) = p;
+  }
+  if (!c3s2_route(x, y, packed_w, bias, act, in_scale, p2, p4, false, s))
+    MGDT_FAIL(MGDT_BAD_SHAPE, "conv3x3_s2_scaled: %dx%dx%d -> %d is outside the LDS-staged stride-2 kernel (see mgdt_conv3x3_s2_scaled_supported)", x->h, x->w, x->c, y->c);
+  MGDT_CHECK_LAUNCH("conv3x3_s2_scaled_fwd");
+  return MGDT_OK;
 }
 extern "C" int mgdt_conv2d_phase_fwd(const mgdt_view* x, const void* packed_w, const float* bias, int phase, const mgdt_view* r1, const mgdt_view* r2,
                                      const mgdt_view* y, int dtype, mgdt_stream s) {
@@ -403,8 +439,8 @@
   if (M > 0x7fffffffL - (1 << 20)) MGDT_FAIL(MGDT_BAD_SHAPE, "conv2d: problem too large");
   a.M = (int)M; a.HoWo = Ho * Wo;
   a.fd_howo = make_fastdiv((uint32_t)a.HoWo); a.fd_wo = make_fastdiv((uint32_t)Wo);
-  if (tapmode == 0 && dtype == MGDT_BF16 && k == 3 && !(x2 && x2->p) && !in_scale && !in_shift && !(r1 && r1->p) && !(r2 && r2->p) &&
-      mgdt_conv3x3_lds_launch(x, y, packed_w, bias, act, a.CP, a.nchunks, a.NTtot, (hipStream_t)s, q8_oscale, q8_xq, stride)) {
+  if (tapmode == 0 && dtype == MGDT_BF16 && k == 3 && !(x2 && x2->p) && !in_shift && !(r1 && r1->p) && !(r2 && r2->p) &&
+      mgdt_conv3x3_lds_launch(x, y, packed_w, bias, act, a.CP, a.nchunks, a.NTtot, (hipStream_t)s, q8_oscale, q8_xq, stride, in_scale, nullptr, nullptr, false)) {
     MGDT_CHECK_LAUNCH("conv2d(3x3 lds)");
     return MGDT_OK;
   }
diff --git a/mgdt_yolo_amd/csrc/pointwise.hip b/mgdt_yolo_amd/csrc/pointwise.hip
--- a/mgdt_yolo_amd/csrc/pointwise.hip
+++ b/mgdt_yolo_amd/csrc/pointwise.hip
@@ -437,17 +437,11 @@
   __syncthreads();
 }
 
-template <typename T, int V>
-__global__ __launch_bounds__(256) void spr_attn_scale_kernel(const float* __restrict__ partial, const float* __restrict__ w1, const float* __restrict__ b1,
-                                                             const float* __restrict__ w2, const float* __restrict__ b2, int C, int G, int H, int W,
-                                                             const T* __restrict__ x, long xsn, long xsh, long xsw, T* __restrict__ y, long ysn, long ysh,
-                                                             long ysw, FastDiv fd_q, FastDiv fd_w, int nsplit, int tiles_x, int tiles_y, SprPool pa, SprPool pb, FastDiv fd_gst,
-                                                             FastDiv fd_tx, FastDiv fd_l4, int fast, unsigned long long* dbg) {
-  extern __shared__ float sm[];
-  unsigned long long TS[10]; int nt = 0;
-  auto stamp = [&]() __attribute__((always_inline)) { if (dbg) TS[nt++] = __builtin_amdgcn_s_memrealtime(); };
-  stamp();
-  const int n = blockIdx.y, cw = C / G, hid = cw / 4;
+__device__ __forceinline__ void spr_attention_lds(const float* __restrict__ partial, const float* __restrict__ w1, const float* __restrict__ b1,
+                                                  const float* __restrict__ w2, const float* __restrict__ b2, int C, int G, int H, int W, int n, int nsplit,
+                                                  int tiles_x, int tiles_y, FastDiv fd_gst, FastDiv fd_tx, FastDiv fd_l4, int fast, float* sm,
+                                                  unsigned long long* TS, int& nt) {
+  const int cw = C / G, hid = cw / 4;
   float* pooled = sm;
   float* hbuf = sm + C * 5;
   float* obuf = hbuf + G * hid;
@@ -456,7 +450,7 @@
   const float cnt[5] = {(float)H * W, (float)he0 * we0, (float)he0 * (W - ws1), (float)(H - hs1) * we0, (float)(H - hs1) * (W - ws1)};
   __shared__ float red[5 * 256];
   if (fast) {
-    spr_prologue_fast(partial, w1, b1, w2, b2, C, G, n, nsplit, tiles_x, tiles_y, fd_gst, fd_tx, fd_l4, cnt, sm, red, att, dbg ? TS : nullptr, nt);
+    spr_prologue_fast(partial, w1, b1, w2, b2, C, G, n, nsplit, tiles_x, tiles_y, fd_gst, fd_tx, fd_l4, cnt, sm, red, att, TS, nt);
   } else {
     if (tiles_x > 0) {
       const int gst = nsplit / (tiles_x * tiles_y);
@@ -522,6 +516,21 @@
     }
     __syncthreads();
   }
+}
+
+template <typename T, int V>
+__global__ __launch_bounds__(256) void spr_attn_scale_kernel(const float* __restrict__ partial, const float* __restrict__ w1, const float* __restrict__ b1,
+                                                             const float* __restrict__ w2, const float* __restrict__ b2, int C, int G, int H, int W,
+                                                             const T* __restrict__ x, long xsn, long xsh, long xsw, T* __restrict__ y, long ysn, long ysh,
+                                                             long ysw, FastDiv fd_q, FastDiv fd_w, int nsplit, int tiles_x, int tiles_y, SprPool pa, SprPool pb, FastDiv fd_gst,
+                                                             FastDiv fd_tx, FastDiv fd_l4, int fast, unsigned long long* dbg) {
+  extern __shared__ float sm[];
+  unsigned long long TS[10]; int nt = 0;
+  auto stamp = [&]() __attribute__((always_inline)) { if (dbg) TS[nt++] = __builtin_amdgcn_s_memrealtime(); };
+  stamp();
+  const int n = blockIdx.y;
+  const float* att = sm + C * 5 + G * (C / G / 4) + C;
+  spr_attention_lds(partial, w1, b1, w2, b2, C, G, H, W, n, nsplit, tiles_x, tiles_y, fd_gst, fd_tx, fd_l4, fast, sm, dbg ? TS : nullptr, nt);
   stamp();
   auto fin = [&]() __attribute__((always_inline)) { if (dbg) { __builtin_amdgcn_s_waitcnt(0); stamp(); if (threadIdx.x == 0) for (int k = 0; k < 8; ++k) dbg[((size_t)blockIdx.y * gridDim.x + blockIdx.x) * 8 + k] = TS[k]; } };
   {
@@ -594,6 +603,15 @@
   fin();
 }
 
+static size_t spr_prologue_lds(int c, int groups, int tiles_x, const float* fc1_w, int* fast) {
+  const int cw = c / groups, hid = cw / 4;
+  size_t lds = (size_t)(c * 5 + groups * hid + 2 * c) * sizeof(float);
+  const size_t wbytes = ((size_t)hid * (5 * cw + 4) + (size_t)cw * (hid + 1) + hid + cw + 4) * sizeof(float);
+  *fast = tiles_x > 0 && c <= 256 && lds + wbytes <= 48 * 1024 && ((uintptr_t)fc1_w & 15) == 0;
+  if (*fast) lds += wbytes;
+  return lds;
+}
+
 extern "C" int mgdt_spr_attn_scale_fwd(const float* pooled, int nsplit, int tiles_x, int tiles_y, const float* fc1_w, const float* fc1_b, const float* fc2_w, const float* fc2_b, int groups,
                                        const mgdt_view* x, const mgdt_view* y, const mgdt_view* pool_a, const mgdt_view* pool_b, int dtype, mgdt_stream s) {
   if (nsplit <= 0) nsplit = SPR_SPLITS;
@@ -604,11 +622,9 @@
   if (groups < 1 || c % groups || (c / groups) % 4 || c > 4096) MGDT_FAIL(MGDT_BAD_SHAPE, "spr_attn_scale: c=%d groups=%d", c, groups);
   if (!vec4_ok(x, dtype) || !vec4_ok(y, dtype) || x->n != y->n || x->h != y->h || x->w != y->w || y->c != c)
     MGDT_FAIL(MGDT_BAD_SHAPE, "spr_attn_scale: views must be matching NHWC, c%%4==0");
-  const int cw = c / groups, hid = cw / 4;
-  size_t lds = (size_t)(c * 5 + groups * hid + 2 * c) * sizeof(float);
-  const size_t wbytes = ((size_t)hid * (5 * cw + 4) + (size_t)cw * (hid + 1) + hid + cw + 4) * sizeof(float);
-  const int fast = tiles_x > 0 && c <= 256 && lds + wbytes <= 48 * 1024 && ((uintptr_t)fc1_w & 15) == 0;
-  if (fast) lds += wbytes;
+  const int cw = c / groups;
+  int fast;
+  const size_t lds = spr_prologue_lds(c, groups, tiles_x, fc1_w, &fast);
   SprPool pl[2] = {{nullptr, 0, 0, 0, 0}, {nullptr, 0, 0, 0, 0}};
   bool pool8 = true;
   const mgdt_view* pv[2] = {pool_a, pool_b};
@@ -647,6 +663,34 @@
     for (int k = 0; k + 1 < ns; ++k) fprintf(stderr, " %.2f", ph[k] * 0.01 / (gK * x->n));
     fprintf(stderr, fast ? "  (issue | loads land | sums | fc1 | fc2 | softmax | scale)\n" : "  (prologue | scale)\n");
   }
+  return MGDT_OK;
+}
+
+__global__ __launch_bounds__(256) void spr_attn_tiles_kernel(const float* __restrict__ partial, const float* __restrict__ w1, const float* __restrict__ b1,
+                                                             const float* __restrict__ w2, const float* __restrict__ b2, int C, int G, int H, int W, int nsplit,
+                                                             int tiles_x, int tiles_y, FastDiv fd_gst, FastDiv fd_tx, FastDiv fd_l4, int fast, float* __restrict__ attn) {
+  extern __shared__ float sm[];
+  int nt = 0;
+  const int n = blockIdx.x;
+  spr_attention_lds(partial, w1, b1, w2, b2, C, G, H, W, n, nsplit, tiles_x, tiles_y, fd_gst, fd_tx, fd_l4, fast, sm, nullptr, nt);
+  const float* att = sm + C * 5 + G * (C / G / 4) + C;
+  for (int c = threadIdx.x; c < C; c += 256) attn[(long)n * C + c] = att[c];
+}
+
+extern "C" int mgdt_spr_attn_tiles_fwd(const float* pooled, int nsplit, int tiles_x, int tiles_y, const float* fc1_w, const float* fc1_b, const float* fc2_w, const float* fc2_b, int groups,
+                                       int n, int c, int h, int w, float* attn, mgdt_stream s) {
+  if (nsplit <= 0) nsplit = SPR_SPLITS;
+  if (tiles_x > 0 && (tiles_y <= 0 || nsplit % (tiles_x * tiles_y) || tiles_x % 2 || tiles_y % 2 || h % 2 || w % 2))
+    MGDT_FAIL(MGDT_BAD_SHAPE, "spr_attn_tiles: per-tile sums need an even tile grid over an even map (nsplit=%d tiles %dx%d)", nsplit, tiles_y, tiles_x);
+  if (!pooled || !fc1_w || !fc1_b || !fc2_w || !fc2_b || !attn || n < 1 || h < 1 || w < 1) MGDT_FAIL(MGDT_BAD_ARG, "spr_attn_tiles: null/empty argument");
+  if (groups < 1 || c % groups || (c / groups) % 4 || c > 4096) MGDT_FAIL(MGDT_BAD_SHAPE, "spr_attn_tiles: c=%d groups=%d", c, groups);
+  const int cw = c / groups;
+  int fast;
+  const size_t lds = spr_prologue_lds(c, groups, tiles_x, fc1_w, &fast);
+  spr_attn_tiles_kernel<<<n, 256, lds, (hipStream_t)s>>>(pooled, fc1_w, fc1_b, fc2_w, fc2_b, c, groups, h, w, nsplit, tiles_x, tiles_y,
+                                                         make_fastdiv((uint32_t)(tiles_x > 0 ? nsplit / (tiles_x * tiles_y) : 1)), make_fastdiv((uint32_t)std::max(tiles_x, 1)),
+                                                         make_fastdiv((uint32_t)(5 * cw / 4)), fast, attn);
+  MGDT_CHECK_LAUNCH("spr_attn_tiles_fwd");
   return MGDT_OK;
 }
 
diff --git a/mgdt_yolo_amd/nn/modules/block.py b/mgdt_yolo_amd/nn/modules/block.py
--- a/mgdt_yolo_amd/nn/modules/block.py
+++ b/mgdt_yolo_amd/nn/modules/block.py
@@ -147,6 +147,9 @@
             mids = [pk for m in self.bottleneck for pk in (m.cv1.packed(dt, False), m.cv2.packed(dt, False))]
             out, pool, slots, tiles = ops.csp_block(ops.CSP_MSPA, x, self._packed_chain(dt).blob, None, mids, self.bottleneck[0].add,
                                                     self.convs[3].packed(dt, False), wd, act_code(self.convs[0].act), self.convs[3].conv.out_channels, True)
+            if deliver and deliver.get('defer') and d_out is None:
+                deliver['attn'] = ops.spr_attention_tiles(pool, slots, tiles, at.fc1.weight, at.fc1.bias, at.fc2.weight, at.fc2.bias, s, *out.shape)
+                return out
             return ops.spr_attention_scale(out, at.fc1.weight, at.fc1.bias, at.fc2.weight, at.fc2.bias, s, out=d_out, part=pool, nsplit=slots, tiles=tiles, pools=d_pools)
         cat = ops.new_act(b, (s - 1 + n) * wd, h, w, dt, x.device)
         if not train and s == 4 and ops.pw_chain_supported(wd, cat.dtype) and x.dtype == cat.dtype and self._chain_ok():
@@ -266,7 +269,7 @@
 
 class SimFusion_4in(nn.Module):
 
-    def forward(self, x, pre=None):
+    def forward(self, x, pre=None, scales=None):
         x_l, x_m, x_s, x_n = x
         b, c, h, w = x_s.shape
         cs = [x_l.shape[1], x_m.shape[1], c, x_n.shape[1]]
@@ -276,6 +279,8 @@
             out, done = pre['out'], pre['done']
         if out is None:
             out = ops.new_act(b, sum(cs), h, w, x_s.dtype, x_s.device)
+        if scales and any(slot not in done for slot in scales):
+            raise RuntimeError('SimFusion_4in: an unscaled (deferred) input needs its pooled copy delivered by the producer side')
         o = 0
         if 0 not in done:
             ops.adaptive_avgpool(x_l, out[:, o:o + cs[0]])
@@ -306,7 +311,8 @@
         self.cv3 = Conv(in_channel_list[2], out_channels, act=nn.ReLU()) if in_channel_list[2] != out_channels else nn.Identity()
         self.cv_fuse = Conv(out_channels * 3, out_channels, act=nn.ReLU())
 
-    def forward(self, x, pre=None):
+    def forward(self, x, pre=None, scales=None):
+        scales = scales or {}
         b, _, h, w = x[1].shape
         oc = self.cv_fuse.conv.out_channels
         dt, dev = x[1].dtype, x[1].device
@@ -314,6 +320,9 @@
         cat, done, pooled0 = None, (), None
         if pre is not None and pre.get('out') is not None and tuple(pre['out'].shape) == (b, 3 * oc, h, w) and pre['out'].dtype == dt:
             cat, done, pooled0 = pre['out'], pre['done'], pre.get('pooled0')
+        if 1 in scales or 2 in scales or (
+                0 in scales and not (0 in done if isinstance(self.cv1, nn.Identity) else (pooled0 is not None and tuple(pooled0.shape) == (b, x[0].shape[1], h, w)))):
+            raise RuntimeError('SimFusion_3in: an unscaled (deferred) input needs its pooled copy delivered by the producer side')
         if cat is None:
             cat = ops.new_act(b, 3 * oc, h, w, dt, dev)
         if isinstance(self.cv1, nn.Identity):
diff --git a/mgdt_yolo_amd/nn/tasks.py b/mgdt_yolo_amd/nn/tasks.py
--- a/mgdt_yolo_amd/nn/tasks.py
+++ b/mgdt_yolo_amd/nn/tasks.py
@@ -10,6 +10,7 @@
 
 from .. import ops
 from ..yolo.utils.torch_utils import fuse_conv_and_bn, initialize_weights, intersect_dicts, make_divisible
+from .modules.conv import act_code
 from .modules import (C2f, IFM, MSPA_C2f, SPPF, Bottleneck, Concat, Conv, Detect, DWConv, InjectionMultiSum_Auto_pool,
                       SimFusion_3in, SimFusion_4in, TOODHead, Upsample)
 
@@ -75,6 +76,7 @@
             layers = list(self.model)[2:]
         plan = self._neck_plan(x) if not self.training else None
         bufs = {}
+        deferred = {}
         head = None
         side = self._side_branch() if not self.training else None
         first = layers[0].i
@@ -90,9 +92,18 @@
             elif self._injection_feeds_next(m):
                 head, out = (m, xin), None
             elif plan is not None and m.i in plan['producers']:
-                out = m(xin, deliver=self._neck_deliveries(plan, m, xin, bufs))
+                dl = self._neck_deliveries(plan, m, xin, bufs)
+                if dl is not None and self._spr_deferrable(plan, m, xin, dl, bufs):
+                    dl['defer'] = True
+                out = m(xin, deliver=dl)
+                if dl is not None and dl.get('attn') is not None:
+                    deferred[m.i] = (dl['attn'], dl['pools'])
+            elif m.i - 1 in deferred and m.f == -1:
+                attn, pools = deferred[m.i - 1]
+                out = ops.conv3x3_s2_scaled(xin, attn, m.packed(torch.bfloat16, direct=False), act_code(m.act), pools=pools)
             elif plan is not None and m.i in plan['consumers']:
-                out = m(xin, pre=bufs.get(m.i))
+                scales = {slot: deferred[j][0] for slot, j in enumerate(self._absf(m)) if j in deferred}
+                out = m(xin, pre=bufs.get(m.i), scales=scales) if scales else m(xin, pre=bufs.get(m.i))
             else:
                 out = m(xin)
             prev.pop(m.i - 1, None)
@@ -184,6 +195,35 @@
             return None
         return plan
 
+    @staticmethod
+    def _absf(m):
+        return [m.i + f if f < 0 else f for f in ([m.f] if isinstance(m.f, int) else m.f)]
+
+    def _spr_deferrable(self, plan, m, x, dl, bufs):
+        if not ops.DEFER_SPR or ops.Q8_CALIB is not None or type(self.model[-1]) is not Detect or dl.get('out') is not None:
+            return False
+        want = plan['producers'][m.i]
+        pools = dl['pools']
+        if len(pools) != len(want) or not pools or sorted(x.shape[2] // p.shape[2] for p in pools) not in ([2], [4], [2, 4]):
+            return False
+        if m.i + 1 >= len(self.model):
+            return False
+        cv = self.model[m.i + 1]
+        if not (type(cv) is Conv and cv.f == -1 and not cv._forward_hooks and not cv.__dict__.get('_q8') and cv.plain_affine() and cv.conv.kernel_size == (3, 3)
+                and cv.conv.stride == (2, 2) and cv.conv.padding == (1, 1) and cv.conv.groups == 1 and cv.conv.in_channels == x.shape[1]
+                and ops.conv3x3_s2_scaled_supported(x, cv.conv.out_channels, act_code(cv.act))):
+            return False
+        for j in range(m.i + 2, len(self.model)):
+            cm = self.model[j]
+            for slot, src in enumerate(self._absf(cm)):
+                if src != m.i:
+                    continue
+                if j not in plan['consumers'] or cm._forward_hooks:
+                    return False
+                if ('pool', j, slot) not in want:
+                    return False
+        return True
+
     def _neck_deliveries(self, plan, m, x, bufs):
         b, c, h, w = x.shape
         out, pools = None, []
@@ -210,6 +250,8 @@
                 st['out'] = ops.new_act(b, total, th, tw, x.dtype, x.device)
             if tuple(st['out'].shape) != (b, total, th, tw):
                 continue
+            if kind == 'pool' and len(pools) == 2:
+                continue
             if isinstance(cm, SimFusion_3in) and slot == 0 and not isinstance(cm.cv1, nn.Identity):
                 st['pooled0'] = ops.new_act(b, c, th, tw, x.dtype, x.device)
                 pools.append(st['pooled0'])
@@ -220,7 +262,7 @@
             else:
                 out = view
             st['done'].add(slot)
-        return {'out': out, 'pools': pools[:2]} if (out is not None or pools) else None
+        return {'out': out, 'pools': pools} if (out is not None or pools) else None
 
     def _stem_fusable(self, x):
         if not ops.FUSED_STEM or getattr(self, 'compute_dtype', None) != torch.bfloat16 or len(self.model) < 3 or 0 in self.save:
diff --git a/mgdt_yolo_amd/ops.py b/mgdt_yolo_amd/ops.py
--- a/mgdt_yolo_amd/ops.py
+++ b/mgdt_yolo_amd/ops.py
@@ -303,6 +303,37 @@
     return out
 
 
+def spr_attention_tiles(part, nsplit, tiles, fc1_w, fc1_b, fc2_w, fc2_b, groups, b, c, h, w):
+    attn = torch.empty(b, c, dtype=torch.float32, device=part.device)
+    _launch('spr_attn_tiles_fwd', 'mgdt_spr_attn_tiles_fwd', ptr(part), int(nsplit), int(tiles[0]), int(tiles[1]), ptr(fc1_w), ptr(fc1_b), ptr(fc2_w), ptr(fc2_b), groups,
+            b, c, h, w, ptr(attn), stream())
+    return attn
+
+
+def conv3x3_s2_scaled_supported(x, cout, act):
+    b, c, h, w = x.shape
+    return bool(x.dtype == torch.bfloat16 and is_nhwc(x) and L.lib().mgdt_conv3x3_s2_scaled_supported(b, h, w, c, cout, act))
+
+
+def conv3x3_s2_scaled(x, in_scale, pk, act, out=None, pools=()):
+    _need_gpu(x)
+    b, _, h, w = x.shape
+    if pk.direct or pk.k != 3 or pk.dtype != torch.bfloat16 or in_scale.dtype != torch.float32 or tuple(in_scale.shape) != (b, pk.cin) or not in_scale.is_contiguous():
+        raise RuntimeError('conv3x3_s2_scaled: bf16 3x3 MFMA panel and a contiguous fp32 [b, cin] factor')
+    if out is None:
+        out = new_act(b, pk.cout, h // 2, w // 2, pk.dtype, x.device)
+    pools = list(pools)
+    if len(pools) > 2:
+        raise RuntimeError('conv3x3_s2_scaled: at most two pooled outputs')
+    _same(x, out, *pools)
+    if x.dtype != pk.dtype:
+        raise RuntimeError(f'conv3x3_s2_scaled: the weights are packed for {pk.dtype}, the input is {x.dtype}')
+    pa, pb = (pools + [None, None])[:2]
+    _launch('conv3x3_s2_scaled_fwd', 'mgdt_conv3x3_s2_scaled_fwd', vp(x), ptr(in_scale), ptr(pk.w), ptr(pk.bias), act, vp(out), vp(pa), vp(pb), stream())
+    return out
+
+
+DEFER_SPR = os.environ.get('MGDT_DEFER_SPR', '1') != '0'
 FUSED_NECK = True
 
 
```
